# HTDerekLiu/surface_multigrid_code

Measured on AMD Instinct MI355X. Metric: V-cycles/sec + fine-level SpMV GB/s (% HBM peak), 1M-vert mesh fp64, higher is better.
Workload: dtype f64; 1 GPU; C3: bunny_15K_init x3 midpoint subdivision, 1011330 verts, 5 levels, M_bary+0.01(-L), fp64; n_verts=1011330, nnz=7079298, levels=5, smoother=gs, rhs_columns_per_gpu=1, parallelism=single GPU

## Files before the change

include/smg.h:

```cpp
#ifndef SMG_H
#define SMG_H

#ifdef __cplusplus
extern "C" {
#endif

#define SMG_VERSION 507

enum {
    SMG_OK = 0,
    SMG_ERR_INVALID = -1,
    SMG_ERR_NO_DEVICE = -2,
    SMG_ERR_HIP = -3,
    SMG_ERR_NONFINITE = -4,
    SMG_ERR_ALLOC = -5,
    SMG_ERR_IO = -6,
    SMG_ERR_REDUCE = -7
};

enum { SMG_HOST = 0, SMG_DEVICE = 1 };

enum { SMG_DEC_QSLIM = 0, SMG_DEC_MIDPOINT = 1, SMG_DEC_VERTEX_REMOVAL = 2 };

enum { SMG_SMOOTH_GS = 0, SMG_SMOOTH_JACOBI = 1, SMG_SMOOTH_HYBRID = 2, SMG_SMOOTH_CHEBYSHEV = 3, SMG_SMOOTH_HYBRID_CHEBYSHEV = 4 };
// ... 93 lines not shown
int smg_eigs(smg_hierarchy *h, const double *mass_diag, int nev, int block, const double *X0, int ld_x0, int memspace,
             const smg_solve_opts *opts, unsigned long long seed, double *evals, double *X, int ld_x, double *res_his, int *n_iter,
             int *n_converged);

typedef struct smg_geodesics smg_geodesics;
int smg_geodesics_create(const smg_hierarchy *h, const double *V, int nV, const int *F, int nF, double t, int voronoi, smg_geodesics **out);
void smg_geodesics_destroy(smg_geodesics *g);
double smg_geodesics_time(const smg_geodesics *g);
int smg_geodesics_set_solver(smg_geodesics *g, int heat_pcg, int poisson_pcg);
long long smg_geodesics_device_bytes(const smg_geodesics *g);
int smg_geodesics_solve(smg_geodesics *g, int k, const int *src_ptr, const int *src, int memspace, const smg_solve_opts *heat_opts,
                        const smg_solve_opts *poisson_opts, double *D, int ld_d, int *cycles);

typedef struct smg_arap smg_arap;
int smg_arap_create(const smg_hierarchy *h, const double *V, int nV, const int *F, int nF, const int *handles, int n_handles, smg_arap **out);
void smg_arap_destroy(smg_arap *a);
int smg_arap_set_solver(smg_arap *a, int pcg);
long long smg_arap_device_bytes(const smg_arap *a);
int smg_arap_solve(smg_arap *a, const double *handle_pos, int ld_hp, const double *U0, int ld_u0, int memspace, int max_iter, double rel_tol,
                   const smg_solve_opts *opts, double *U, int ld_u, double *energy_his, int *cycles, int *n_iter);

typedef struct {
    double young, poisson, thickness, mass_scale, dt, pressure;
    int newton_iters;
    double ls_c, ls_shrink, ls_min_alpha, eig_floor, eig_value;
} smg_membrane_params;
void smg_membrane_params_default(smg_membrane_params *p);
typedef struct smg_membrane smg_membrane;
int smg_membrane_create(const smg_hierarchy *h, const double *V, int nV, const int *F, int nF, const smg_membrane_params *p, smg_membrane **out);
void smg_membrane_destroy(smg_membrane *m);
long long smg_membrane_device_bytes(const smg_membrane *m);
int smg_membrane_set_state(smg_membrane *m, const double *pos, const double *qdot, int memspace);
int smg_membrane_get_state(smg_membrane *m, double *pos, double *qdot, int memspace);
int smg_membrane_set_solver(smg_membrane *m, int pcg);
int smg_membrane_step(smg_membrane *m, const smg_solve_opts *opts, double *objective_his, double *alpha, int *cycles, int *n_newton);
int smg_membrane_lists(const int *F, int nF, int nV, int *n_blocks, int *n_contrib, int *bptr, int *bcol, int *c_ptr, int *c_src);
int smg_membrane_faces_host(const double *V0, const double *P, int nV, const int *F, int nF, const smg_membrane_params *p, int fix, double *W,
                            double *G, double *H);

int smg_solve_begin(smg_hierarchy *h, const double *RHS, int ld_rhs, const double *known_val, int ld_kv,
                    const double *z0, int ld_z0, int k, int memspace, const smg_solve_opts *opts);
int smg_solve_iter_residual(smg_hierarchy *h, double *d_sumsq);
int smg_solve_iter_cycle(smg_hierarchy *h, const double *d_sumsq);
int smg_solve_iter_cycle_speculative(smg_hierarchy *h);
int smg_solve_iter_commit(smg_hierarchy *h, const double *d_sumsq);
int smg_solve_poll(smg_hierarchy *h, int *done, int *n_his);
int smg_solve_end(smg_hierarchy *h, double *z, int ld_z, int memspace, double *r_his, int *n_his, int *converged);

typedef int (*smg_reduce_fn)(double *d_sumsq, int count, void *hip_stream, void *ctx);
int smg_solve_sharded(smg_hierarchy *h, const double *RHS, int ld_rhs, const double *known_val, int ld_kv, const double *z0,
                      int ld_z0, int k_local, int memspace, const smg_solve_opts *opts, smg_reduce_fn reduce, void *ctx,
                      double *z, int ld_z, double *r_his, int *n_his, int *converged);

int smg_level_rows(const smg_hierarchy *h, int lv);
int smg_vcycle(smg_hierarchy *h, const double *B, int pre, int post, int lv, double *u, int k);
int smg_apply_A(smg_hierarchy *h, int lv, const double *u, int k, double *Au);
int smg_restrict(smg_hierarchy *h, int lv, const double *x, int k, double *Rx);
int smg_prolong(smg_hierarchy *h, int lv, const double *x, int k, double *Px);
int smg_relax(smg_hierarchy *h, int lv, const double *B, int k, int iters, double *u);
int smg_coarse_solve(smg_hierarchy *h, const double *B, int k, double *u);
int smg_residual_norm(smg_hierarchy *h, int lv, const double *B, const double *u, int k, double *norm);

int smg_raw_spmv(smg_hierarchy *h, int lv, int mode, const double *x, const double *b, double *y, int k);
int smg_raw_relax(smg_hierarchy *h, int lv, const double *b, double *u, int k, int iters);
int smg_raw_spmv_f32(smg_hierarchy *h, int lv, const float *x, float *y, int k);
int smg_raw_outer_iteration(smg_hierarchy *h, int n_iter);
int smg_synchronize(smg_hierarchy *h);
int smg_bench_vcycle(smg_hierarchy *h, int lv, int k, int pre, int post, int reps, double *us_per_cycle);
int smg_bench_relax(smg_hierarchy *h, int lv, int k, int sweeps, int reps, double *us_per_call);

int smg_level_get_matrix(const smg_hierarchy *h, int lv, int which, int internal, int *n_rows, int *n_cols, int *nnz,
                         int *rowptr, int *col, double *val);
int smg_level_get_perm(const smg_hierarchy *h, int lv, int *perm);
int smg_level_get_colors(const smg_hierarchy *h, int lv, int *n_colors, int *color_ptr );
int smg_level_get_Adiag(const smg_hierarchy *h, int lv, double *diag);
int smg_get_unknown(const smg_hierarchy *h, int *n_unknown, int *unknown );
int smg_level_sell_stats(const smg_hierarchy *h, int lv, int which, long *stored, long *padded, int *n_slices);
int smg_level_first_colour_rows(const smg_hierarchy *h, int lv);
long smg_level_spmv_bytes(const smg_hierarchy *h, int lv, int k);
long smg_vcycle_bytes(const smg_hierarchy *h, int k, int pre, int post);

int smg_debug_check_tiling_plan(smg_hierarchy *h, int lv, int sweeps, int tile_rows, int *n_tiles, int *max_ext_rows, double *redundancy,
                                double *max_abs_diff);
int smg_debug_check_block_gs_plan(smg_hierarchy *h, int lv, int block_rows, int *n_blocks, int *n_colors, double *rim, double *fill, double *max_abs_diff);
int smg_debug_check_wave_gs_plan(smg_hierarchy *h, int lv, int piece_rows, int pieces_mode, int *n_pieces, int *n_colors, double *stats, double *max_abs_diff);
int smg_debug_raise_coarse_stall(smg_hierarchy *h);
int smg_debug_schur_solve_host(int n, const int *ptr, const int *col, const double *val, const double *b, double *x, int *n_blocks, int *n_sep);
int smg_debug_check_sparse_cholesky(int n, const int *rowptr, const int *col, const double *val, long *factor_entries, int *dependency_depth,
                                    double *rel_residual);

int smg_debug_dense_geneig_host(int n, const double *A, const double *B, double *evals, double *V);

int smg_debug_eig_gram(int n, int m, int nb_a, const double *Sa, int nb_b, const double *Sb, const double *w, int sym, int done, double *G,
                       int *groups, int *guard_bad);
int smg_debug_eig_combine(int n, int m, int nb, const double *S, const double *AS, const double *C, int make_p, int done, double *X, double *AX,
                          double *P, double *AP, int *guard_bad);
int smg_debug_eig_residual(int n, int m, const double *X, const double *AX, const double *mass, const double *lam, int f32, int done, double *b0,
                           double *u0, float *b32, float *u32, double *res, int *groups, int *guard_bad);
enum { SMG_KRY_DOTS_ZR_ZQ = 0, SMG_KRY_DIRECTION = 1, SMG_KRY_DOTS_PQ = 2, SMG_KRY_STEP_DECIDE = 3, SMG_KRY_PRECOND_IN = 4, SMG_KRY_WIDEN = 5 };
int smg_debug_krylov(int op, int n, int k, double *v0, double *v1, double *v2, double *v3, float *e, double *s, int *restart, double tol, int done,
                     double *ctrl_d, int *ctrl_i, int *groups, int *guard_bad);
enum { SMG_GEO_BASIS = 0, SMG_GEO_SCATTER = 1, SMG_GEO_DIVERGENCE = 2, SMG_GEO_SHIFT = 3 };
int smg_debug_geodesics(int op, int n, int nF, int k, const int *F, const int *m_ptr, const int *m_idx, const int *src_ptr, const int *src,
                        const double *in, double *W, double *Af, double *out, int ld_out, int *guard_bad);
enum { SMG_ARAP_COVARIANCE = 0, SMG_ARAP_ROTATIONS = 1, SMG_ARAP_RHS = 2, SMG_ARAP_VERTEX_ENERGY = 3, SMG_ARAP_ENERGY = 4 };
int smg_debug_arap(int op, int n, const int *rowptr, const int *col, const double *w, const double *P0, const double *P, const double *R_in,
                   double *out, int *guard_hits);

enum { SMG_MEM_REST = 0, SMG_MEM_FACES_RAW = 1, SMG_MEM_FACES = 2, SMG_MEM_ENERGY = 3, SMG_MEM_PRESSURE = 4, SMG_MEM_MATRIX = 5,
       SMG_MEM_GRADIENT = 6, SMG_MEM_OBJECTIVE = 7 };
int smg_debug_membrane(int op, int nV, int nF, const int *F, const double *V0, const double *P, const double *in, const smg_membrane_params *p,
                       double *out, int *guard_hits);

int smg_prof_enable(smg_hierarchy *h, int on);
int smg_prof_reset(smg_hierarchy *h);
int smg_prof_count(smg_hierarchy *h);
int smg_prof_get(smg_hierarchy *h, int idx, char *name, int name_cap, long *count, double *total_ms);

int smg_mesh_read(const char *path, double **V, int *nV, int **F, int *nF);
void smg_free(void *p);
int smg_mesh_normalize_unit_area(double *V, int nV, const int *F, int nF);
int smg_mesh_cotmatrix(const double *V, int nV, const int *F, int nF, int *nnz, int *rowptr, int *col, double *val);
int smg_mesh_massmatrix(const double *V, int nV, const int *F, int nF, int voronoi, double *diag);
int smg_mesh_boundary_loop(const int *F, int nF, int nV, int *loop, int *n_loop);
int smg_mesh_midpoint_upsample(int nV, const int *F, int nF, int *nE, int *S_rowptr, int *S_col, double *S_val,
                               int *NF);
int smg_mesh_torus(int nu, int nv, double R, double r, double *V, int *F);

#ifdef __cplusplus
}
#endif
#endif
```

surface_multigrid_code_amd/_lib.py:

```python
import ctypes as C
import os

HERE = os.path.dirname(os.path.abspath(__file__))
LIB_PATH = os.environ.get("SMG_LIB") or os.path.join(HERE, "lib", "libsmg.so")

SMG_HOST, SMG_DEVICE = 0, 1


class SolveOptsC(C.Structure):
    _fields_ = [("tol", C.c_double), ("max_iter", C.c_int), ("pre", C.c_int), ("post", C.c_int),
                ("verbosity", C.c_int), ("check_every", C.c_int), ("use_graph", C.c_int), ("precision", C.c_int),
                ("smoother", C.c_int), ("omega", C.c_double), ("jacobi_max_rows", C.c_int), ("cheby_fraction", C.c_double)]


class MembraneParamsC(C.Structure):
    _fields_ = [("young", C.c_double), ("poisson", C.c_double), ("thickness", C.c_double), ("mass_scale", C.c_double), ("dt", C.c_double),
                ("pressure", C.c_double), ("newton_iters", C.c_int), ("ls_c", C.c_double), ("ls_shrink", C.c_double),
                ("ls_min_alpha", C.c_double), ("eig_floor", C.c_double), ("eig_value", C.c_double)]


_lib = None


REDUCE_FN = C.CFUNCTYPE(C.c_int, C.c_void_p, C.c_int, C.c_void_p, C.c_void_p)
# ... 24 lines not shown
        "smg_level_spectral_bound": (d, [vp, i]),
        "smg_level_set_prolong": (i, [vp, i, i, i, ip, ip, dp]),
        "smg_level_set_prolong_csc": (i, [vp, i, i, i, ip, ip, dp]),
        "smg_level_set_mesh": (i, [vp, i, dp, i, ip, i]),
        "smg_level_get_mesh": (i, [vp, i, ip, ip, dp, ip]),
        "smg_mg_precompute": (i, [dp, i, ip, i, f, i, i, C.POINTER(vp)]),
        "smg_mg_precompute_capped": (i, [dp, i, ip, i, f, i, i, f, C.POINTER(vp)]),
        "smg_mg_precompute_logged": (i, [dp, i, ip, i, f, i, i, f, i, C.POINTER(vp)]),
        "smg_query_coarse_to_fine": (i, [vp, i, i, ip, dp, ip, dp]),
        "smg_query_fine_to_coarse": (i, [vp, i, i, ip, dp, ip, dp]),
        "smg_mg_precompute_block": (i, [dp, i, ip, i, f, i, i, C.POINTER(vp)]),
        "smg_hierarchy_save": (i, [vp, C.c_char_p]),
        "smg_hierarchy_load": (i, [C.c_char_p, C.POINTER(vp)]),
        "smg_mg_precompute_subdiv": (i, [dp, i, ip, i, i, f, i, i, C.POINTER(vp), dp, ip]),
        "smg_precompute": (i, [vp, i, ip, ip, dp, ip, i]),
        "smg_precompute_values_device": (i, [vp, vp]),
        "smg_assembler_create": (i, [ip, i, i, C.POINTER(vp)]),
        "smg_assembler_destroy": (None, [vp]),
        "smg_assembler_pattern": (i, [vp, ip, ip, ip]),
        "smg_assemble": (i, [vp, vp, i, d, d, vp, vp, vp, vp]),
        "smg_solve": (i, [vp, vp, i, vp, i, vp, i, i, i, C.POINTER(SolveOptsC), vp, i, dp, ip, ip]),
        "smg_solve_pcg": (i, [vp, vp, i, vp, i, vp, i, i, i, C.POINTER(SolveOptsC), vp, i, dp, ip, ip]),
        "smg_eigs": (i, [vp, vp, i, i, vp, i, i, C.POINTER(SolveOptsC), C.c_ulonglong, dp, vp, i, dp, ip, ip]),
        "smg_debug_dense_geneig_host": (i, [i, dp, dp, dp, dp]),
        "smg_debug_eig_gram": (i, [i, i, i, dp, i, dp, dp, i, i, dp, ip, ip]),
        "smg_debug_eig_combine": (i, [i, i, i, dp, dp, dp, i, i, dp, dp, dp, dp, ip]),
        "smg_debug_eig_residual": (i, [i, i, dp, dp, dp, dp, i, i, dp, dp, fp, fp, dp, ip, ip]),
        "smg_debug_krylov": (i, [i, i, i, dp, dp, dp, dp, fp, dp, ip, d, i, dp, ip, ip, ip]),
        "smg_debug_geodesics": (i, [i, i, i, i, ip, ip, ip, ip, ip, dp, dp, dp, dp, i, ip]),
        "smg_geodesics_create": (i, [vp, dp, i, ip, i, d, i, C.POINTER(vp)]),
        "smg_geodesics_destroy": (None, [vp]),
        "smg_geodesics_time": (d, [vp]),
        "smg_geodesics_set_solver": (i, [vp, i, i]),
        "smg_geodesics_device_bytes": (C.c_longlong, [vp]),
        "smg_geodesics_solve": (i, [vp, i, ip, ip, i, C.POINTER(SolveOptsC), C.POINTER(SolveOptsC), vp, i, ip]),
        "smg_debug_arap": (i, [i, i, ip, ip, dp, dp, dp, dp, dp, ip]),
        "smg_arap_create": (i, [vp, dp, i, ip, i, ip, i, C.POINTER(vp)]),
        "smg_arap_destroy": (None, [vp]),
        "smg_arap_set_solver": (i, [vp, i]),
        "smg_arap_device_bytes": (C.c_longlong, [vp]),
        "smg_arap_solve": (i, [vp, vp, i, vp, i, i, i, d, C.POINTER(SolveOptsC), vp, i, dp, ip, ip]),
        "smg_debug_membrane": (i, [i, i, i, ip, dp, dp, dp, C.POINTER(MembraneParamsC), dp, ip]),
        "smg_membrane_params_default": (None, [C.POINTER(MembraneParamsC)]),
        "smg_membrane_create": (i, [vp, dp, i, ip, i, C.POINTER(MembraneParamsC), C.POINTER(vp)]),
        "smg_membrane_destroy": (None, [vp]),
        "smg_membrane_device_bytes": (C.c_longlong, [vp]),
        "smg_membrane_set_state": (i, [vp, vp, vp, i]),
        "smg_membrane_get_state": (i, [vp, vp, vp, i]),
        "smg_membrane_set_solver": (i, [vp, i]),
        "smg_membrane_step": (i, [vp, C.POINTER(SolveOptsC), dp, dp, ip, ip]),
        "smg_membrane_lists": (i, [ip, i, i, ip, ip, ip, ip, ip, ip]),
        "smg_membrane_faces_host": (i, [dp, dp, i, ip, i, C.POINTER(MembraneParamsC), i, dp, dp, dp]),
        "smg_solve_sharded": (i, [vp, vp, i, vp, i, vp, i, i, i, C.POINTER(SolveOptsC), REDUCE_FN, vp, vp, i, dp, ip, ip]),
        "smg_solve_begin": (i, [vp, vp, i, vp, i, vp, i, i, i, C.POINTER(SolveOptsC)]),
        "smg_solve_iter_residual": (i, [vp, vp]),
        "smg_solve_iter_cycle": (i, [vp, vp]),
        "smg_solve_iter_cycle_speculative": (i, [vp]),
        "smg_solve_iter_commit": (i, [vp, vp]),
        "smg_solve_poll": (i, [vp, ip, ip]),
        "smg_solve_end": (i, [vp, vp, i, i, dp, ip, ip]),
        "smg_level_rows": (i, [vp, i]),
        "smg_vcycle": (i, [vp, dp, i, i, i, dp, i]),
        "smg_apply_A": (i, [vp, i, dp, i, dp]),
        "smg_restrict": (i, [vp, i, dp, i, dp]),
        "smg_prolong": (i, [vp, i, dp, i, dp]),
        "smg_relax": (i, [vp, i, dp, i, i, dp]),
        "smg_coarse_solve": (i, [vp, dp, i, dp]),
        "smg_residual_norm": (i, [vp, i, dp, dp, i, dp]),
        "smg_raw_spmv": (i, [vp, i, i, vp, vp, vp, i]),
        "smg_raw_relax": (i, [vp, i, vp, vp, i, i]),
        "smg_raw_spmv_f32": (i, [vp, i, vp, vp, i]),
        "smg_raw_outer_iteration": (i, [vp, i]),
        "smg_synchronize": (i, [vp]),
        "smg_bench_vcycle": (i, [vp, i, i, i, i, i, dp]),
        "smg_bench_relax": (i, [vp, i, i, i, i, dp]),
        "smg_level_get_matrix": (i, [vp, i, i, i, ip, ip, ip, ip, ip, dp]),
        "smg_level_get_perm": (i, [vp, i, ip]),
        "smg_level_get_colors": (i, [vp, i, ip, ip]),
        "smg_level_get_Adiag": (i, [vp, i, dp]),
        "smg_get_unknown": (i, [vp, ip, ip]),
        "smg_level_sell_stats": (i, [vp, i, i, lp, lp, ip]),
        "smg_level_first_colour_rows": (i, [vp, i]),
        "smg_debug_check_tiling_plan": (i, [vp, i, i, i, ip, ip, dp, dp]),
        "smg_debug_check_sparse_cholesky": (i, [i, ip, ip, dp, lp, ip, dp]),
        "smg_hierarchy_set_coarse_dense_max": (i, [vp, i]),
        "smg_hierarchy_set_coarse_schur": (i, [vp, i, i]),
        "smg_debug_schur_solve_host": (i, [i, ip, ip, dp, dp, dp, ip, ip]),
        "smg_hierarchy_set_block_gs": (i, [vp, i]),
        "smg_hierarchy_set_wave_gs": (i, [vp, i]),
        "smg_hierarchy_set_memory_lean": (i, [vp, i]),
        "smg_hierarchy_create_union": (i, [C.POINTER(vp), i, C.POINTER(vp)]),
        "smg_union_members": (i, [vp]),
        "smg_union_member_rows": (i, [vp, i, ip, ip]),
        "smg_union_get_history": (i, [vp, i, dp, i, ip, ip]),
        "smg_debug_device_bytes": (i, [vp, C.c_char_p, i]),
        "smg_level_get_wave_gs_order": (i, [vp, i, i, ip, ip, ip, ip, ip, dp]),
        "smg_debug_check_wave_gs_plan": (i, [vp, i, i, i, ip, ip, dp, dp]),
        "smg_debug_raise_coarse_stall": (i, [vp]),
        "smg_debug_check_block_gs_plan": (i, [vp, i, i, ip, ip, dp, dp, dp]),
        "smg_level_get_block_gs_order": (i, [vp, i, i, ip, ip, ip, ip, ip, dp]),
        "smg_hierarchy_coarse_solver": (i, [vp, lp]),
        "smg_hierarchy_set_block_mode": (i, [vp, i]),
        "smg_hierarchy_block_size": (i, [vp]),
        "smg_level_block_stats": (i, [vp, i, lp, lp, ip]),
        "smg_level_get_block_image": (i, [vp, i, ip, ip, ip, ip, ip, ip, dp]),
        "smg_level_spmv_bytes": (C.c_long, [vp, i, i]),
        "smg_vcycle_bytes": (C.c_long, [vp, i, i, i]),
        "smg_prof_enable": (i, [vp, i]),
        "smg_prof_reset": (i, [vp]),
        "smg_prof_count": (i, [vp]),
        "smg_prof_get": (i, [vp, i, C.c_char_p, i, lp, dp]),
        "smg_mesh_read": (i, [C.c_char_p, C.POINTER(dp), ip, C.POINTER(ip), ip]),
        "smg_free": (None, [vp]),
        "smg_mesh_normalize_unit_area": (i, [dp, i, ip, i]),
        "smg_mesh_cotmatrix": (i, [dp, i, ip, i, ip, ip, ip, dp]),
        "smg_mesh_massmatrix": (i, [dp, i, ip, i, i, dp]),
        "smg_mesh_boundary_loop": (i, [ip, i, i, ip, ip]),
        "smg_mesh_midpoint_upsample": (i, [i, ip, i, ip, ip, ip, dp, ip]),
        "smg_mesh_torus": (i, [i, i, d, d, dp, ip]),
    }
    for name, (res, args) in sig.items():
        fn = getattr(L, name)
        fn.restype = res
        fn.argtypes = args
    L._smg_signatures = sig
    _lib = L
    return L


def exported_symbols():
    return sorted(load()._smg_signatures.keys())
```

surface_multigrid_code_amd/api.py:

```python
import ctypes as C

import numpy as np
import scipy.sparse as sp

from . import _lib
from ._lib import SMG_DEVICE, SMG_HOST, SolveOptsC


class SmgError(RuntimeError):
    def __init__(self, code, where):
        msg = _lib.load().smg_last_error()
        super().__init__("%s failed (%d): %s" % (where, code, msg.decode() if msg else ""))
        self.code = code


def _chk(rc, where):
    if rc != 0:
        raise SmgError(rc, where)


def _ip(a):
    return a.ctypes.data_as(C.POINTER(C.c_int))


# ... 216 lines not shown
        y = np.zeros((nout, x.shape[1]), order="F")
        _chk(fn(self.h, lv, _dp(x), x.shape[1], _dp(y)), name)
        return y

    def A(self, lv, u):
        return self._piece(self.L.smg_apply_A, "smg_apply_A", lv, u, self.rows(lv), self.rows(lv))

    def restrict(self, lv, x):
        return self._piece(self.L.smg_restrict, "smg_restrict", lv, x, self.rows(lv + 1), self.rows(lv))

    def prolong(self, lv, x):
        return self._piece(self.L.smg_prolong, "smg_prolong", lv, x, self.rows(lv), self.rows(lv + 1))

    def relax(self, lv, B, u, iters):
        B, u = _colmajor(B), _colmajor(u).copy(order="F")
        self._rows_checked(lv, "smg_relax", B, u)
        _chk(self.L.smg_relax(self.h, lv, _dp(B), B.shape[1], iters, _dp(u)), "smg_relax")
        return u

    def coarse_solve(self, B, u):
        B, u = _colmajor(B), _colmajor(u).copy(order="F")
        self._rows_checked(self.n_levels - 1, "smg_coarse_solve", B, u)
        _chk(self.L.smg_coarse_solve(self.h, _dp(B), B.shape[1], _dp(u)), "smg_coarse_solve")
        return u

    def vcycle(self, B, u, lv=0, pre=2, post=2):
        B, u = _colmajor(B), _colmajor(u).copy(order="F")
        self._rows_checked(lv, "smg_vcycle", B, u)
        _chk(self.L.smg_vcycle(self.h, _dp(B), pre, post, lv, _dp(u), B.shape[1]), "smg_vcycle")
        return u

    def residual_norm(self, lv, B, u):
        B, u = _colmajor(B), _colmajor(u)
        self._rows_checked(lv, "smg_residual_norm", B, u)
        out = C.c_double(0)
        _chk(self.L.smg_residual_norm(self.h, lv, _dp(B), _dp(u), B.shape[1], C.byref(out)), "smg_residual_norm")
        return out.value

    def matrix(self, lv, which="A", internal=False):
        w = {"A": 0, "P": 1, "PT": 2, "P_full": 3, "Auk": 4}[which]
        nr, nc, nnz = C.c_int(), C.c_int(), C.c_int()
        _chk(self.L.smg_level_get_matrix(self.h, lv, w, int(internal), C.byref(nr), C.byref(nc), C.byref(nnz),
                                         None, None, None), "smg_level_get_matrix")
        ptr = np.zeros(nr.value + 1, np.int32)
        col = np.zeros(max(nnz.value, 1), np.int32)
        val = np.zeros(max(nnz.value, 1))
        _chk(self.L.smg_level_get_matrix(self.h, lv, w, int(internal), None, None, None, _ip(ptr), _ip(col), _dp(val)),
             "smg_level_get_matrix")
        return sp.csr_matrix((val[: nnz.value], col[: nnz.value], ptr), shape=(nr.value, nc.value))

    def perm(self, lv):
        p = np.zeros(self.rows(lv), np.int32)
        _chk(self.L.smg_level_get_perm(self.h, lv, _ip(p)), "smg_level_get_perm")
        return p

    def colors(self, lv):
        nc = C.c_int()
        _chk(self.L.smg_level_get_colors(self.h, lv, C.byref(nc), None), "smg_level_get_colors")
        cp = np.zeros(nc.value + 1, np.int32)
        _chk(self.L.smg_level_get_colors(self.h, lv, None, _ip(cp)), "smg_level_get_colors")
        return cp

    def Adiag(self, lv):
        d = np.zeros(self.rows(lv))
        _chk(self.L.smg_level_get_Adiag(self.h, lv, _dp(d)), "smg_level_get_Adiag")
        return d

    def unknown(self):
        n = C.c_int()
        _chk(self.L.smg_get_unknown(self.h, C.byref(n), None), "smg_get_unknown")
        u = np.zeros(n.value, np.int32)
        _chk(self.L.smg_get_unknown(self.h, None, _ip(u)), "smg_get_unknown")
        return u

    def sell_stats(self, lv, which="A"):
        st, pd, ns = C.c_long(), C.c_long(), C.c_int()
        _chk(self.L.smg_level_sell_stats(self.h, lv, {"A": 0, "P": 1, "PT": 2}[which], C.byref(st), C.byref(pd),
                                         C.byref(ns)), "smg_level_sell_stats")
        return {"stored": st.value, "padded": pd.value, "n_slices": ns.value}

    def first_colour_rows(self, lv):
        return self.L.smg_level_first_colour_rows(self.h, lv)

    def set_block_gs(self, min_rows):
        _chk(self.L.smg_hierarchy_set_block_gs(self.h, int(min_rows)), "smg_hierarchy_set_block_gs")

    def block_gs_order(self, lv, k):
        nb, nc = C.c_int(), C.c_int()
        rc = self.L.smg_level_get_block_gs_order(self.h, lv, int(k), C.byref(nb), C.byref(nc), None, None, None, None)
        if rc < 0:
            _chk(rc, "smg_level_get_block_gs_order")
        if rc == 0:
            return None
        cp, bp, rows, st = np.zeros(nc.value + 1, np.int32), np.zeros(nb.value + 1, np.int32), np.zeros(self.rows(lv), np.int32), np.zeros(2)
        _chk(min(self.L.smg_level_get_block_gs_order(self.h, lv, int(k), None, None, _ip(cp), _ip(bp), _ip(rows), _dp(st)), 0), "smg_level_get_block_gs_order")
        return {"rows": rows, "blk_ptr": bp, "color_ptr": cp, "rim": st[0], "fill": st[1]}

    def set_wave_gs(self, mode="auto"):
        _chk(self.L.smg_hierarchy_set_wave_gs(self.h, {"auto": -1, "never": 0, "all": 1}[mode]), "smg_hierarchy_set_wave_gs")

    def wave_gs_order(self, lv, k=1):
        nb, nc = C.c_int(), C.c_int()
        rc = self.L.smg_level_get_wave_gs_order(self.h, lv, int(k), C.byref(nb), C.byref(nc), None, None, None, None)
        if rc < 0:
            _chk(rc, "smg_level_get_wave_gs_order")
        if rc == 0:
            return None
        cp, bp, rows, st = np.zeros(nc.value + 1, np.int32), np.zeros(nb.value + 1, np.int32), np.zeros(self.rows(lv), np.int32), np.zeros(3)
        _chk(min(self.L.smg_level_get_wave_gs_order(self.h, lv, int(k), None, None, _ip(cp), _ip(bp), _ip(rows), _dp(st)), 0), "smg_level_get_wave_gs_order")
        return {"rows": rows, "piece_ptr": bp, "color_ptr": cp, "rim": st[0], "phases_mean": st[1], "phases_max": int(st[2])}

    def gs_order(self, lv, k=1):
        w = self.wave_gs_order(lv, k)
        if w is not None:
            return w["rows"]
        b = self.block_gs_order(lv, k)
        if b is not None:
            return b["rows"]
        return np.arange(self.rows(lv), dtype=np.int32)

    @classmethod
    def union(cls, members):
        L = _lib.load()
        arr = (C.c_void_p * len(members))(*[m.h for m in members])
        out = C.c_void_p()
        _chk(L.smg_hierarchy_create_union(arr, len(members), C.byref(out)), "smg_hierarchy_create_union")
        return cls(handle=out.value)

    def union_members(self):
        return self.L.smg_union_members(self.h)

    def union_member_rows(self, member):
        a, b = C.c_int(), C.c_int()
        _chk(self.L.smg_union_member_rows(self.h, member, C.byref(a), C.byref(b)), "smg_union_member_rows")
        return a.value, b.value

    def union_history(self, member, cap=4096):
        rh, n, cv = np.zeros(cap), C.c_int(), C.c_int()
        _chk(self.L.smg_union_get_history(self.h, member, _dp(rh), cap, C.byref(n), C.byref(cv)), "smg_union_get_history")
        return bool(cv.value), rh[:min(n.value, cap)].copy()

    def set_coarse_dense_max(self, n_max):
        _chk(self.L.smg_hierarchy_set_coarse_dense_max(self.h, int(n_max)), "smg_hierarchy_set_coarse_dense_max")

    def set_coarse_schur(self, when="refactor", n_min=-1):
        _chk(self.L.smg_hierarchy_set_coarse_schur(self.h, {"never": 0, "always": 1, "refactor": 2}[when], int(n_min)), "smg_hierarchy_set_coarse_schur")

    def set_memory_lean(self, on=True):
        _chk(self.L.smg_hierarchy_set_memory_lean(self.h, 1 if on else 0), "smg_hierarchy_set_memory_lean")

    def coarse_solver(self):
        ne = C.c_long()
        kind = self.L.smg_hierarchy_coarse_solver(self.h, C.byref(ne))
        return {"kind": {1: "sparse_cholesky", 2: "schur_complement"}.get(kind, "dense_inverse"), "factor_entries": ne.value}

    def set_block_mode(self, mode="auto"):
        _chk(self.L.smg_hierarchy_set_block_mode(self.h, {"auto": -1, "scalar": 0, "block": 3}.get(mode, mode)), "smg_hierarchy_set_block_mode")

    def block_size(self):
        return self.L.smg_hierarchy_block_size(self.h)

    def block_stats(self, lv=0):
        nb, ns, nc = C.c_long(), C.c_long(), C.c_int()
        _chk(self.L.smg_level_block_stats(self.h, lv, C.byref(nb), C.byref(ns), C.byref(nc)), "smg_level_block_stats")
        return {"blocks": nb.value, "block_slots": ns.value, "vertex_colors": nc.value}

# ... 346 lines not shown
```

surface_multigrid_code_amd/csrc/smg_capi.cpp:

```cpp
#include <hip/hip_runtime.h>

#include <algorithm>
#include <atomic>
#include <chrono>
#include <cmath>
#include <cstdarg>
#include <cstdio>
#include <cstdlib>
#include <cstring>
#include <functional>
#include <memory>
#include <numeric>
#include <string>
#include <thread>
#include <vector>

#include "smg_internal.hpp"

using namespace smg;

static thread_local std::string g_err;
int smg::fail(int code, const char* fmt, ...)
{
    char buf[512];
    va_list ap;
    va_start(ap, fmt);
    std::vsnprintf(buf, sizeof(buf), fmt, ap);
    va_end(ap);
    g_err = buf;
    return code;
}

extern "C" const char* smg_last_error(void) { return g_err.c_str(); }
extern "C" int smg_version(void) { return SMG_VERSION; }
extern "C" long long smg_device_bytes_live(void) { return (long long)smg::devbuf_live_bytes().load(); }
extern "C" int smg_debug_device_bytes(const smg_hierarchy* h, char* buf, int cap)
{
    if (!h || !buf || cap < 1) return SMG_ERR_INVALID;
    std::string out;
    auto B = [](const auto& d) { return (long long)(d.n * sizeof(*d.p)); };
    auto sell = [&](const smg::SellBuf& S) { return B(S.slice_row) + B(S.slice_off) + B(S.slice_w) + B(S.col) + B(S.order) + B(S.val) + B(S.diag_slot) + B(S.long_row) + B(S.long_ptr) + B(S.long_col) + B(S.long_val) + B(S.long_valf); };
    long long tot = 0;
    auto line = [&](const std::string& nm, long long v) { if (v) { out += nm + " " + std::to_string(v) + "\n"; tot += v; } };
    for (int lv = 0; lv < h->n_levels; lv++) {
        const smg::Level& L = h->lv[lv];
        const std::string p = "level" + std::to_string(lv) + ".";
        line(p + "A_sell", sell(L.dA)); line(p + "AT_sell", sell(L.dAT)); line(p + "P_sell", sell(L.dP)); line(p + "PT_sell", sell(L.dPT));
        line(p + "A_block3", B(L.bA.slice_row) + B(L.bA.slice_off) + B(L.bA.slice_w) + B(L.bA.col) + B(L.bA.order) + B(L.bA.val) + B(L.bA.valf) + B(L.bAT.slice_row) + B(L.bAT.slice_off) + B(L.bAT.slice_w) + B(L.bAT.col) + B(L.bAT.order) + B(L.bAT.val) + B(L.bAT.valf) + B(L.mapB) + B(L.mapBT));
        line(p + "values_caller_order", B(L.d_Aval) + B(L.d_Tval));
        line(p + "refresh_maps", B(L.mapA) + B(L.mapAT));
        line(p + "galerkin_recipes", B(L.r1_ptr) + B(L.r1_idx) + B(L.r2_ptr) + B(L.r2_idx) + B(L.r1_coef) + B(L.r2_coef));
        long long t = 0;
        for (const auto& T : L.tiled) t += T.bytes();
        line(p + "tiled_plans", t);
        line(p + "bgs_plan", L.bgs.bytes());
        line(p + "wgs_plan", L.wgs.bytes());
        line(p + "fp32_images", B(L.a32) + B(L.at32) + B(L.p32) + B(L.pt32) + B(L.b32) + B(L.u32) + B(L.r32) + B(L.t32) + B(L.d32));
        line(p + "vectors", B(L.b) + B(L.u) + B(L.r) + B(L.t) + B(L.d));
    }
    line("coarse.dense_inverse", B(h->d_Ainv) + B(h->d_Ainv32));
    line("coarse.sym_partials", B(h->d_sympart));
    line("coarse.sparse_factor", B(h->c_perm) + B(h->c_rptr) + B(h->c_rcol) + B(h->c_cptr) + B(h->c_crow) + B(h->c_err) + B(h->c_rval) + B(h->c_cval) + B(h->c_diag) + B(h->c_work));
    line("coarse.schur", B(h->sch.irow) + B(h->sch.bsize) + B(h->sch.srow) + B(h->sch.sptr) + B(h->sch.sidx) + B(h->sch.aptr) + B(h->sch.ablk) + B(h->sch.acol) + B(h->sch.rptr) + B(h->sch.coff) + B(h->sch.pos) +
                         B(h->sch.pos2) + B(h->sch.ones) + B(h->sch.rdst) + B(h->sch.rdst2) + B(h->sch.rsrc) + B(h->sch.arena) + B(h->sch.g) + B(h->sch.xs) + B(h->sch.sym) + B(h->sch.gj) + B(h->sch.arena32) + B(h->sch.g32) + B(h->sch.xs32));
    line("maps_level0", B(h->d_map0) + B(h->d_perm0) + B(h->d_unknown) + B(h->d_known) + B(h->d_auk_ptr) + B(h->d_auk_col) + B(h->d_auk_val));
    line("reprecompute_bookkeeping", B(h->d_lhs_src) + B(h->d_auk_src) + B(h->d_diag_idx) + B(h->d_dense_pos) + B(h->d_Afull));
    line("early_upload", B(h->early0.ptr) + B(h->early0.col) + B(h->early0.val));
    line("krylov", B(h->kry_x) + B(h->kry_r) + B(h->kry_p) + B(h->kry_q) + B(h->kry_b) + B(h->kry_part) + B(h->kry_s) + B(h->kry_restart));
    line("eigs", B(h->eig_x[0]) + B(h->eig_x[1]) + B(h->eig_ax[0]) + B(h->eig_ax[1]) + B(h->eig_p[0]) + B(h->eig_p[1]) + B(h->eig_ap[0]) + B(h->eig_ap[1]) +
                 B(h->eig_w) + B(h->eig_aw) + B(h->eig_mass) + B(h->eig_part) + B(h->eig_small) + B(h->eig_stage));
    line("solve_state", B(h->d_ctrl) + B(h->d_rhis) + B(h->d_partials) + B(h->d_lam) + B(h->d_stage_rhs) + B(h->d_stage_z) + B(h->d_stage_kv) + B(h->d_tmp_cm) + B(h->d_zsave));
    out += "total " + std::to_string(tot) + "\n";
    std::snprintf(buf, (size_t)cap, "%s", out.c_str());
    return SMG_OK;
}
extern "C" int smg_device_count(void)
{
    int n = 0;
    if (hipGetDeviceCount(&n) != hipSuccess) return 0;
    return n;
}
extern "C" void smg_solve_opts_default(smg_solve_opts* o)
{
    if (!o) return;
    o->tol = 1e-3;
    o->max_iter = 20;
    o->pre = 2;
    o->post = 2;
    o->verbosity = 0;
    o->check_every = 0;
    o->use_graph = 1;
    o->precision = 0;
    o->smoother = SMG_SMOOTH_GS;
    o->omega = 0.8;
    o->jacobi_max_rows = 100000;
    o->cheby_fraction = 0.1;
}

int smg::ensure_device(smg_hierarchy* h)
{
    if (h->device >= 0) return SMG_OK;
    int n = 0;
    if (hipGetDeviceCount(&n) != hipSuccess || n <= 0)
        return fail(SMG_ERR_NO_DEVICE, "no HIP device: libsmg has no CPU fallback (the CPU oracle lives in oracle/)");
    int dev = 0;
    HIPCHK(hipGetDevice(&dev));
    h->device = dev;
    if (!h->stream && !h->user_stream) {
        HIPCHK(hipStreamCreateWithFlags(&h->stream, hipStreamNonBlocking));
        h->own_stream = true;
    }
    HIPCHK(h->d_ctrl.alloc(1));
    HIPCHK(hipMemset(h->d_ctrl.p, 0, sizeof(Ctrl)));
    HIPCHK(h->d_rhis.alloc(1));
    return SMG_OK;
}

void smg::drop_graphs(smg_hierarchy* h) { h->graphs.drop(); }

hipError_t SellBuf::upload(const Sell& S)
{
    hipError_t e;
    if ((e = slice_row.upload(S.slice_row)) != hipSuccess) return e;
    if ((e = slice_off.upload(S.slice_off)) != hipSuccess) return e;
    if ((e = slice_w.upload(S.slice_w)) != hipSuccess) return e;
    const bool layout_only = S.col.empty() && S.padded() > 0;
    if (layout_only) {
        if ((e = col.alloc((size_t)S.padded())) != hipSuccess) return e;
        if ((e = val.alloc((size_t)S.padded())) != hipSuccess) return e;
    } else {
        if ((e = col.upload(S.col)) != hipSuccess) return e;
        if ((e = val.upload(S.val)) != hipSuccess) return e;
    }
    if ((e = order.upload(S.region_order)) != hipSuccess) return e;
    view.n_rows = S.n_rows; view.n_cols = S.n_cols; view.n_slices = S.n_slices; view.C = S.C;
    view.order = S.region_order.empty() ? nullptr : order.p;
// ... 710 lines not shown
```

surface_multigrid_code_amd/csrc/smg_cycle.cpp:

```cpp
#include <hip/hip_runtime.h>

#include <algorithm>
#include <chrono>
#include <cmath>
#include <cstdarg>
#include <cstdio>
#include <cstdlib>
#include <cstring>
#include <functional>
#include <memory>
#include <numeric>
#include <string>
#include <thread>
#include <vector>

#include "smg_internal.hpp"

using namespace smg;


int smg::ensure_work(smg_hierarchy* h, int k)
{
    const int L = h->n_levels;
    if (k > h->kcap) {
// ... 198 lines not shown
    static hipError_t coarse(smg_hierarchy* h, Level& L, int k, const Ctrl* ctrl)
    {
        if (h->union_m > 0) return launch_blockdiag_gemv_add(h->un.view, h->d_Ainv.p, h->nc, L.b.p, L.u.p, k, ctrl, h->stream);
        if (h->coarse_sparse) return launch_sparse_coarse_solve(h->c_view, L.b.p, L.u.p, k, ctrl, h->stream);
        if (h->coarse_schur) return launch_schur_solve(h->sch.view, L.b.p, L.u.p, k, ctrl, h->stream);
        return launch_dense_gemv_add(h->d_Ainv.p, h->nc, h->nc_pad, L.b.p, L.u.p, coarse_cols(h, k), k, ctrl, h->stream, h->d_sympart.p);
    }
    static hipError_t opA(smg_hierarchy* h, Level& L, bool smoother_image, SellMode m, int s0, int s1, const double* x, const double* bb, double* y, int k,
                          const Ctrl* ctrl, const FirstColour* fc = nullptr, double omega = 1.0)
    {
        if (h->bs == 3) {
            const Bsr3Dev& V = (smoother_image && L.gs_on_transpose) ? L.bAT.view : L.bA.view;
            return launch_bsr3(m, V, s0, s1 < 0 ? V.n_slices : s1, x, bb, y, k, ctrl, nullptr, nullptr, h->stream, omega, fc ? fc->c1 : 0.0, fc ? fc->d : nullptr);
        }
        const SellDev& V = smoother_image ? G(L) : A(L);
        return sell(m, V, s0, s1 < 0 ? V.n_slices : s1, x, bb, y, k, ctrl, h->stream, nullptr, fc, omega);
    }
};
template <> struct Prec<float> {
    static float* b(Level& L) { return L.b32.p; }
    static float* u(Level& L) { return L.u32.p; }
    static float* r(Level& L) { return L.r32.p; }
    static float* t(Level& L) { return L.t32.p; }
    static float* d(Level& L) { return L.d32.p; }
    static void set_d(FirstColour& fc, Level& L) { fc.df = L.d32.p; }
    static const SellDev& A(Level& L) { return L.dA32; }
    static const SellDev& G(Level& L) { return L.gs_on_transpose ? L.dAT32 : L.dA32; }
    static const SellDev& P(Level& L) { return L.dP32; }
    static const SellDev& PT(Level& L) { return L.dPT32; }
    static bool has_vals(const SellDev& V) { return V.valf != nullptr; }
    static hipError_t sell(SellMode m, const SellDev& V, int s0, int s1, const float* x, const float* bb, float* y, int k, const Ctrl* ctrl,
                           hipStream_t st, float* zero_rows = nullptr, const FirstColour* first = nullptr, double omega = 1.0)
    { return launch_sell_f32(m, V, s0, s1, x, bb, y, k, ctrl, st, zero_rows, first, omega); }
    static hipError_t coarse(smg_hierarchy* h, Level& L, int k, const Ctrl* ctrl)
    {
        if (h->coarse_schur) return launch_schur_solve_f32(h->sch.view, L.b32.p, L.u32.p, k, ctrl, h->stream);
        return launch_dense_gemv_add_f32(h->d_Ainv32.p, h->nc, h->nc_pad, L.b32.p, L.u32.p, coarse_cols(h, k), k, ctrl, h->stream, (float*)h->d_sympart.p);
    }
    static hipError_t opA(smg_hierarchy* h, Level& L, bool smoother_image, SellMode m, int s0, int s1, const float* x, const float* bb, float* y, int k,
                          const Ctrl* ctrl, const FirstColour* fc = nullptr, double omega = 1.0)
    {
        if (h->bs == 3) {
            const Bsr3Dev& V = (smoother_image && L.gs_on_transpose) ? L.bAT.view : L.bA.view;
            return launch_bsr3_f32(m, V, s0, s1 < 0 ? V.n_slices : s1, x, bb, y, k, ctrl, h->stream, omega, fc ? fc->c1 : 0.0, fc ? fc->df : nullptr);
        }
        const SellDev& V = smoother_image ? G(L) : A(L);
        return sell(m, V, s0, s1 < 0 ? V.n_slices : s1, x, bb, y, k, ctrl, h->stream, nullptr, fc, omega);
    }
};

static const std::vector<int>& colour_slices(const smg_hierarchy* h, const Level& Lv)
{
    if (h->bs == 3) return (Lv.gs_on_transpose ? Lv.bAT : Lv.bA).color_slice_ptr;
    return (Lv.gs_on_transpose ? Lv.dAT : Lv.dA).color_slice_ptr;
}

template <typename T>
static int enqueue_gs(smg_hierarchy* h, int lv, const SweepPlan& sp, const T* b, T* u, int k, int iters, const Ctrl* ctrl, int first = FIRST_NONE, T* t = nullptr)
{
    Level& Lv = h->lv[lv];
    ProfGuard pg(h, "MG: relaxation");
    if (const WgsBuf* W = sp.wave) {
        for (int it = 0; it < iters; it++)
            for (size_t c = 0; c + 1 < W->color_ptr.size(); c++)
                HIPCHK(launch_wgs(W->view, W->color_ptr[c], W->color_ptr[c + 1], (const double*)b, (double*)u, k, ctrl, h->stream));
        return SMG_OK;
    }
    if (const BgsBuf* Q = sp.block) {
        for (int it = 0; it < iters; it++)
            for (size_t c = 0; c + 1 < Q->color_ptr.size(); c++)
                HIPCHK(launch_bgs(Q->view, Q->color_ptr[c], Q->color_ptr[c + 1], (const double*)b, (double*)u, k, ctrl, h->stream));
        return SMG_OK;
    }
    const std::vector<int>& cs = colour_slices(h, Lv);
    for (int it = first == FIRST_SWEEP ? 1 : 0; it < iters; it++)
        for (size_t c = (it == 0 && first == FIRST_LAUNCH) ? 1 : 0; c + 1 < cs.size(); c++) {
            if (it == 1 && first == FIRST_SWEEP) HIPCHK(Prec<T>::sell(SELL_GS_OOP, Prec<T>::G(Lv), cs[c], cs[c + 1], t, b, u, k, ctrl, h->stream));
            else HIPCHK(Prec<T>::opA(h, Lv, true, SELL_GS, cs[c], cs[c + 1], u, b, u, k, ctrl));
        }
    return SMG_OK;
}

template <typename T>
static int enqueue_gs_tiled(smg_hierarchy* h, const TiledDev& plan, const T* b, T* const buf[2], int* cur, int k, const Ctrl* ctrl)
{
    ProfGuard pg(h, "MG: relaxation");
    HIPCHK(launch_tiled_gs(plan, (const double*)buf[*cur], (const double*)b, (double*)buf[1 - *cur], k, ctrl, h->stream));
    *cur ^= 1;
    return SMG_OK;
}

template <typename T>
static int enqueue_jacobi(smg_hierarchy* h, int lv, const T* b, T* const buf[2], int* cur, int k, int iters, const Ctrl* ctrl)
{
    Level& Lv = h->lv[lv];
    ProfGuard pg(h, "MG: relaxation");
    for (int it = 0; it < iters; it++) {
        HIPCHK(Prec<T>::opA(h, Lv, true, SELL_JACOBI, 0, -1, buf[*cur], b, buf[1 - *cur], k, ctrl, nullptr, h->omega));
        *cur ^= 1;
    }
    return SMG_OK;
}

template <typename T>
static int enqueue_cheby(smg_hierarchy* h, int lv, const T* b, T* const buf[2], int* cur, int k, int iters, const Ctrl* ctrl, bool first_done = false)
{
    if (iters <= 0) return SMG_OK;
    Level& Lv = h->lv[lv];
    ProfGuard pg(h, "MG: relaxation");
    std::vector<ChebyCoef> cf;
    cheby_coefs(Lv.lam, h->cheby_fraction, iters + 1, cf);
    for (int s = first_done ? 1 : 0; s <= iters; s++) {
        FirstColour fc;
        Prec<T>::set_d(fc, Lv);
        fc.c1 = cf[s].c1;
        HIPCHK(Prec<T>::opA(h, Lv, true, SELL_CHEBY, 0, -1, buf[*cur], b, buf[1 - *cur], k, ctrl, &fc, cf[s].c2));
        *cur ^= 1;
    }
    return SMG_OK;
}

static bool fuse_first_colour() { static const int on = env_int("SMG_FUSE_FIRST", 1); return on != 0; }

template <typename T>
static int enqueue_vcycle_t(smg_hierarchy* h, int lv, int k, int pre, int post, const Ctrl* ctrl, int first = FIRST_NONE)
{
    const bool first_done = first != FIRST_NONE;
    const int L = h->n_levels;
    Level& Lv = h->lv[lv];
    if (lv == L - 1) {
        ProfGuard pg(h, "MG: coarse solve");
        HIPCHK(Prec<T>::coarse(h, Lv, k, ctrl));
        return SMG_OK;
    }
    Level& Lc = h->lv[lv + 1];
    const int kind = level_kind(h, lv);
    const bool jac = kind != LV_GS;
    T* const buf[2] = {Prec<T>::u(Lv), Prec<T>::t(Lv)};
    int cur = 0;
    const bool fp64 = std::is_same<T, double>::value;
    const SweepPlan sp_pre = sweep_plan(h, lv, k, pre, fp64, first), sp_post = sweep_plan(h, lv, k, post, fp64, FIRST_NONE);
    int rc;
    if (kind == LV_JACOBI) {
        if (first_done) cur = 1;
        rc = enqueue_jacobi<T>(h, lv, Prec<T>::b(Lv), buf, &cur, k, pre - (first_done ? 1 : 0), ctrl);
    } else if (kind == LV_CHEBY) {
        if (first_done) cur = 1;
        rc = enqueue_cheby<T>(h, lv, Prec<T>::b(Lv), buf, &cur, k, pre, ctrl, first_done);
    } else if (sp_pre.tiled) rc = enqueue_gs_tiled<T>(h, *sp_pre.tiled, Prec<T>::b(Lv), buf, &cur, k, ctrl);
    else rc = enqueue_gs<T>(h, lv, sp_pre, Prec<T>::b(Lv), buf[0], k, pre, ctrl, first, buf[1]);
    if (rc) return rc;
    {
        ProfGuard pg(h, "MG: residual");
        HIPCHK(Prec<T>::opA(h, Lv, false, SELL_RESID, 0, -1, buf[cur], Prec<T>::b(Lv), Prec<T>::r(Lv), k, ctrl));
    }
    const SellBuf& Gc = Lc.gs_on_transpose ? Lc.dAT : Lc.dA;
    const int kind_c = level_kind(h, lv + 1);
    const bool jac_c = kind_c != LV_GS;
    const bool fuse = h->bs == 1 && sweep_plan(h, lv + 1, k, pre, fp64, FIRST_NONE).colours() && fuse_first_colour() && lv + 1 < L - 1 && pre > 0 && Prec<T>::has_vals(Prec<T>::G(Lc)) && (jac_c ? Gc.n_all > 0 : Gc.n_first > 0);
    const int kt = k * h->bs;
    {
        ProfGuard pg(h, "MG: restrict");
        FirstColour fc;
        if (fuse) {
            fc.diag_slot = Gc.diag_slot.p; fc.n_first = jac_c ? Gc.n_all : Gc.n_first;
            fc.val = Prec<T>::G(Lc).val; fc.valf = Prec<T>::G(Lc).valf;
            fc.jacobi = kind_c == LV_CHEBY ? 2 : (jac_c ? 1 : 0); fc.omega = h->omega;
            if (kind_c == LV_CHEBY) {
                std::vector<ChebyCoef> cf;
                cheby_coefs(Lc.lam, h->cheby_fraction, 1, cf);
                fc.omega = cf[0].c2;
                Prec<T>::set_d(fc, Lc);
            }
        }
        T* init = (fuse && jac_c) ? Prec<T>::t(Lc) : Prec<T>::u(Lc);
        HIPCHK(Prec<T>::sell(SELL_AX, Prec<T>::PT(Lc), 0, Prec<T>::PT(Lc).n_slices, Prec<T>::r(Lv), nullptr, Prec<T>::b(Lc), kt, ctrl, h->stream, init,
                             fuse ? &fc : nullptr));
    }
    rc = enqueue_vcycle_t<T>(h, lv + 1, k, pre, post, ctrl, fuse ? FIRST_LAUNCH : FIRST_NONE);
    if (rc) return rc;
    {
        ProfGuard pg(h, "MG: prolong");
        int dst = cur;
        const int flips = sp_post.tiled ? 1 : kind == LV_CHEBY ? (post > 0 ? post + 1 : 0) : post;
        if ((jac || sp_post.tiled) && ((cur + flips) & 1)) dst = 1 - cur;
        if (!jac && !sp_post.tiled && cur == 1) dst = 0;
        HIPCHK(Prec<T>::sell(SELL_ADD, Prec<T>::P(Lc), 0, Prec<T>::P(Lc).n_slices, Prec<T>::u(Lc), buf[cur], buf[dst], kt, ctrl, h->stream));
        cur = dst;
    }
    if (kind == LV_CHEBY) return enqueue_cheby<T>(h, lv, Prec<T>::b(Lv), buf, &cur, k, post, ctrl);
    if (jac) return enqueue_jacobi<T>(h, lv, Prec<T>::b(Lv), buf, &cur, k, post, ctrl);
    if (sp_post.tiled) return enqueue_gs_tiled<T>(h, *sp_post.tiled, Prec<T>::b(Lv), buf, &cur, k, ctrl);
    return enqueue_gs<T>(h, lv, sp_post, Prec<T>::b(Lv), buf[0], k, post, ctrl);
}

int smg::enqueue_vcycle(smg_hierarchy* h, int k, const Ctrl* ctrl, int first)
{
    if (h->precision == 1) return enqueue_vcycle_t<float>(h, 0, k, h->pre, h->post, ctrl);
    return enqueue_vcycle_t<double>(h, 0, k, h->pre, h->post, ctrl, first);
}

int smg::apply_A(smg_hierarchy* h, int lv, SellMode mode, const double* x, const double* b, double* y, int k, const Ctrl* ctrl)
{
    HIPCHK(Prec<double>::opA(h, h->lv[lv], false, mode, 0, -1, x, b, y, k, ctrl));
    return SMG_OK;
}


static int enqueue_relax(smg_hierarchy* h, int lv, const double* b, double* u, int k, int iters, const Ctrl* ctrl)
{
    Level& Lv = h->lv[lv];
    const int kind = level_kind(h, lv);
    const SweepPlan sp = sweep_plan(h, lv, k, iters, true, FIRST_NONE);
    if (kind == LV_GS && !sp.tiled) return enqueue_gs<double>(h, lv, sp, b, u, k, iters, ctrl);
    double* const buf[2] = {u, Lv.t.p};
    int cur = 0;
    int rc = kind == LV_GS ? enqueue_gs_tiled<double>(h, *sp.tiled, b, buf, &cur, k, ctrl)
             : kind == LV_CHEBY ? enqueue_cheby<double>(h, lv, b, buf, &cur, k, iters, ctrl) : enqueue_jacobi<double>(h, lv, b, buf, &cur, k, iters, ctrl);
    if (rc) return rc;
    if (cur == 1) HIPCHK(hipMemcpyAsync(u, Lv.t.p, (size_t)Lv.n * k * sizeof(double), hipMemcpyDeviceToDevice, h->stream));
    return SMG_OK;
}

bool smg::head_fusable(smg_hierarchy* h, int k)
{
    static const int on = env_int("SMG_FUSE_HEAD", 1);
    if (!on || h->precision != 0 || h->n_levels < 2 || h->prof_on || h->bs != 1 || h->union_m > 0) return false;
    Level& L0 = h->lv[0];
    if (L0.gs_on_transpose) return false;
    if (!sweep_plan(h, 0, k, h->pre, true, FIRST_NONE).colours()) return false;
    const int kind = level_kind(h, 0);
    return kind == LV_GS ? h->pre >= 2 : h->pre >= 1;
}

int smg::enqueue_residual_ss(smg_hierarchy* h, int k, bool fuse_decide, double* sumsq_out)
// ... 47 lines not shown

int smg::enqueue_cycle_part(smg_hierarchy* h, int k, const double* d_sumsq)
{
    if (d_sumsq) HIPCHK(launch_decide(h->d_ctrl.p, d_sumsq, h->stream));
    {
        ProfGuard pg(h, "MG: total VCycle");
        if (h->precision == 1) {
            Level& L0 = h->lv[0];
            const size_t cnt = (size_t)L0.n * k;
            HIPCHK(launch_residual_to_f32(L0.b32.p, L0.u32.p, L0.r.p, cnt, h->d_ctrl.p, h->stream));
            int rc = enqueue_vcycle(h, k, h->d_ctrl.p, FIRST_NONE);
            if (rc) return rc;
            HIPCHK(launch_add_correction(L0.u.p, L0.u32.p, cnt, h->d_ctrl.p, h->stream));
        } else {
            int rc = enqueue_vcycle(h, k, h->d_ctrl.p, h->head_fuse ? FIRST_SWEEP : FIRST_NONE);
            if (rc) return rc;
            if (h->union_m > 0) HIPCHK(launch_union_restore(h->un.view, h->lv[0].u.p, k, h->d_ctrl.p, h->stream));
        }
    }
    return SMG_OK;
}

int smg::coarse_stall_check(smg_hierarchy* h)
{
    if (!h->coarse_sparse || !h->c_err.p) return SMG_OK;
    int cerr = 0;
    HIPCHK(hipMemcpy(&cerr, h->c_err.p, sizeof(int), hipMemcpyDeviceToHost));
    if (!cerr) return SMG_OK;
    (void)hipMemset(h->c_err.p, 0, sizeof(int));
    return fail(SMG_ERR_HIP, "the triangular solves of the sparse coarse factorisation stalled (results are NaN)");
}

int smg::check_ready(const smg_hierarchy* h, const char* who)
{
    if (!h) return fail(SMG_ERR_INVALID, "%s: null handle", who);
    if (!h->precomputed) return fail(SMG_ERR_INVALID, "%s: call smg_precompute first", who);
    if (h->device < 0) return fail(SMG_ERR_NO_DEVICE, "%s: no HIP device", who);
    return SMG_OK;
}

int smg::internal_cols(const smg_hierarchy* h, int k)
{
    static const int on = env_int("SMG_PAD_COLS", 1);
    if (!on || k <= 4 || k > 64 || h->union_m > 0) return k;
    if (k > 32) return k > 40 ? 64 : k;
    int p = 8;
    while (p < k) p *= 2;
    return p;
}

static int piece_prolog(smg_hierarchy* h, int lv, int k, const char* who, bool need_coarser);

static int time_graph(smg_hierarchy* h, hipGraphExec_t g, int reps, double* us)
{
    hipEvent_t e0, e1;
    HIPCHK(hipEventCreate(&e0));
    HIPCHK(hipEventCreate(&e1));
    for (int i = 0; i < 3; i++) HIPCHK(hipGraphLaunch(g, h->stream));
    HIPCHK(hipEventRecord(e0, h->stream));
    for (int i = 0; i < reps; i++) HIPCHK(hipGraphLaunch(g, h->stream));
    HIPCHK(hipEventRecord(e1, h->stream));
    HIPCHK(hipStreamSynchronize(h->stream));
    float ms = 0.f;
    HIPCHK(hipEventElapsedTime(&ms, e0, e1));
    *us = 1e3 * ms / reps;
    (void)hipEventDestroy(e0); (void)hipEventDestroy(e1); (void)hipGraphExecDestroy(g);
    return SMG_OK;
}

extern "C" int smg_bench_vcycle(smg_hierarchy* h, int lv, int k, int pre, int post, int reps, double* us_per_cycle)
{
    int rc = piece_prolog(h, lv, k, "smg_bench_vcycle", false);
    if (rc) return rc;
    DeviceScope dsc(h->device);
    if (reps < 1 || !us_per_cycle) return fail(SMG_ERR_INVALID, "smg_bench_vcycle: bad arguments");
    if ((rc = prepare_sweep_plans(h, k, pre, post))) return rc;
    hipGraphExec_t g = nullptr;
    rc = capture_graph(h, &g, [&]() { return enqueue_vcycle_t<double>(h, lv, k, pre, post, nullptr); });
    if (rc) return rc;
    if ((rc = time_graph(h, g, reps, us_per_cycle))) return rc;
    return coarse_stall_check(h);
}

extern "C" int smg_bench_relax(smg_hierarchy* h, int lv, int k, int sweeps, int reps, double* us_per_call)
{
    int rc = piece_prolog(h, lv, k, "smg_bench_relax", true);
    if (rc) return rc;
    DeviceScope dsc(h->device);
    if (reps < 1 || sweeps < 1 || !us_per_call) return fail(SMG_ERR_INVALID, "smg_bench_relax: bad arguments");
    if ((rc = prepare_sweep_plans(h, k, sweeps, sweeps))) return rc;
    Level& Lv = h->lv[lv];
    hipGraphExec_t g = nullptr;
    rc = capture_graph(h, &g, [&]() { return enqueue_relax(h, lv, Lv.b.p, Lv.u.p, k, sweeps, nullptr); });
    if (rc) return rc;
    return time_graph(h, g, reps, us_per_call);
}

extern "C" int smg_synchronize(smg_hierarchy* h)
{
    if (!h || h->device < 0) return fail(SMG_ERR_INVALID, "smg_synchronize: no device");
    DeviceScope dsc(h->device);
    HIPCHK(hipStreamSynchronize(h->stream));
    return coarse_stall_check(h);
}

extern "C" int smg_level_rows(const smg_hierarchy* h, int lv)
{
    if (!h || lv < 0 || lv >= h->n_levels) return SMG_ERR_INVALID;
    return h->lv[lv].n;
}

static int put_block(smg_hierarchy* h, int lv, const double* src, int k, double* dst)
{
    const Level& Lv = h->lv[lv];
    std::vector<double> tmp((size_t)Lv.n * k);
    for (int i = 0; i < Lv.n; i++)
        for (int c = 0; c < k; c++) tmp[(size_t)i * k + c] = src[(size_t)Lv.ord.perm[i] + (size_t)c * Lv.n];
    HIPCHK(hipMemcpyAsync(dst, tmp.data(), tmp.size() * sizeof(double), hipMemcpyHostToDevice, h->stream));
    HIPCHK(hipStreamSynchronize(h->stream));
    return SMG_OK;
}
static int get_block(smg_hierarchy* h, int lv, const double* src, int k, double* dst)
{
    const Level& Lv = h->lv[lv];
    std::vector<double> tmp((size_t)Lv.n * k);
    HIPCHK(hipMemcpyAsync(tmp.data(), src, tmp.size() * sizeof(double), hipMemcpyDeviceToHost, h->stream));
    HIPCHK(hipStreamSynchronize(h->stream));
    for (int i = 0; i < Lv.n; i++)
        for (int c = 0; c < k; c++) dst[(size_t)Lv.ord.perm[i] + (size_t)c * Lv.n] = tmp[(size_t)i * k + c];
    return coarse_stall_check(h);
}

static int piece_prolog(smg_hierarchy* h, int lv, int k, const char* who, bool need_coarser)
{
    int rc = check_ready(h, who);
    if (rc) return rc;
    if (h->in_solve) return fail(SMG_ERR_INVALID, "%s: a split-phase solve is in progress", who);
    if (lv < 0 || lv >= h->n_levels || (need_coarser && lv >= h->n_levels - 1) || k < 1)
        return fail(SMG_ERR_INVALID, "%s: bad level %d or k %d", who, lv, k);
    DeviceScope dsc(h->device);
    return ensure_work(h, k);
}

extern "C" int smg_apply_A(smg_hierarchy* h, int lv, const double* u, int k, double* Au)
{
    int rc = piece_prolog(h, lv, k, "smg_apply_A", true);
    if (rc) return rc;
    DeviceScope dsc(h->device);
    Level& Lv = h->lv[lv];
    if ((rc = put_block(h, lv, u, k, Lv.u.p))) return rc;
    HIPCHK(Prec<double>::opA(h, Lv, false, SELL_AX, 0, -1, Lv.u.p, nullptr, Lv.r.p, k, nullptr));
    return get_block(h, lv, Lv.r.p, k, Au);
}

extern "C" int smg_restrict(smg_hierarchy* h, int lv, const double* x, int k, double* Rx)
{
    int rc = piece_prolog(h, lv, k, "smg_restrict", true);
    if (rc) return rc;
    DeviceScope dsc(h->device);
    Level &Lv = h->lv[lv], &Lc = h->lv[lv + 1];
    if ((rc = put_block(h, lv, x, k, Lv.r.p))) return rc;
    HIPCHK(launch_sell(SELL_AX, Lc.dPT.view, 0, Lc.dPT.view.n_slices, Lv.r.p, nullptr, Lc.b.p, k * h->bs, nullptr, nullptr, nullptr, h->stream));
    return get_block(h, lv + 1, Lc.b.p, k, Rx);
}

extern "C" int smg_prolong(smg_hierarchy* h, int lv, const double* x, int k, double* Px)
// ... 139 lines not shown
```

surface_multigrid_code_amd/csrc/smg_device.hip:

```cpp
#include <hip/hip_runtime.h>

#include <cstdlib>
#include <type_traits>

#include "smg_device.hpp"
#include "smg_device_inl.hpp"
#include "smg_gj_inl.hpp"

namespace smg {


__device__ int g_never_done = 0;
const int* never_done()
{
    static const int* p = nullptr;
    if (!p) { void* q = nullptr; if (hipGetSymbolAddress(&q, HIP_SYMBOL(g_never_done)) == hipSuccess) p = (const int*)q; }
    return p;
}


template <typename T> struct CoarseInit { T* u; const T* gs_val; const int* diag_slot; int n_first; int jacobi; T omega; T* d; T c1; int codes; T tab[4]; };
template <typename T> __device__ __forceinline__ T code_val(const CoarseInit<T>& z, int cw)
{
    const T lo = (cw & 1) ? z.tab[1] : z.tab[0], hi = (cw & 1) ? z.tab[3] : z.tab[2];
// ... 982 lines not shown
        for (int t = 0; t < DEPTH; t++) { av[t] = an[t]; bv[t] = bn[t]; }
    }
    __shared__ double red[4][4][64];
#pragma unroll
    for (int r = 0; r < 4; r++) red[w][r][lane] = acc[r];
    __syncthreads();
    if (w == 0 && !stop) {
#pragma unroll
        for (int r = 0; r < 4; r++) {
            const int row = row0 + lr + 4 * r;
            if (row < n && colok) {
                const size_t o = (size_t)row * ld + col0 + lc;
                u[o] = u[o] + ((red[0][r][lane] + red[1][r][lane]) + (red[2][r][lane] + red[3][r][lane]));
            }
        }
    }
}

template <int KC, int CPW>
__global__ __launch_bounds__(256) void k_dense_gemm_mfma_multi(const double* __restrict__ Ainv, int n, int lda, const double* __restrict__ b,
                                                               double* u, int ld, const int* done, int kvalid)
{
    const int stop = load_flag(done);
    constexpr int CB = KC / 16 / CPW, DEPTH = 6;
    const int lane = threadIdx.x & 63, w = threadIdx.x >> 6;
    const int rb = blockIdx.x / CB, cb = blockIdx.x % CB;
    const int row0 = rb * 16, col0 = cb * 16 * CPW;
    const int lc = lane & 15, lr = lane >> 4;
    const int per = lda / 16;
    const int s0 = per * w;
    const double* pa = Ainv + (size_t)(4 * s0 + lr) * lda + row0 + lc;
    const double* pb = b + (size_t)(4 * s0 + lr) * ld + col0 + lc;
    const size_t sa = (size_t)4 * lda, sb = (size_t)4 * ld;
    v4f64_t acc[CPW];
#pragma unroll
    for (int c = 0; c < CPW; c++) acc[c] = (v4f64_t){0.0, 0.0, 0.0, 0.0};
    double av[DEPTH], bv[CPW][DEPTH];
#pragma unroll
    for (int t = 0; t < DEPTH; t++) {
        av[t] = t < per ? pa[t * sa] : 0.0;
#pragma unroll
        for (int c = 0; c < CPW; c++) bv[c][t] = (t < per && col0 + 16 * c + lc < kvalid) ? pb[t * sb + 16 * c] : 0.0;
    }
    for (int s = 0; s < per; s += DEPTH) {
        double an[DEPTH], bn[CPW][DEPTH];
#pragma unroll
        for (int t = 0; t < DEPTH; t++) {
            const int q = s + DEPTH + t;
            an[t] = q < per ? pa[q * sa] : 0.0;
#pragma unroll
            for (int c = 0; c < CPW; c++) bn[c][t] = (q < per && col0 + 16 * c + lc < kvalid) ? pb[q * sb + 16 * c] : 0.0;
        }
#pragma unroll
        for (int t = 0; t < DEPTH; t++)
#pragma unroll
            for (int c = 0; c < CPW; c++) acc[c] = __builtin_amdgcn_mfma_f64_16x16x4f64(av[t], bv[c][t], acc[c], 0, 0, 0);
#pragma unroll
        for (int t = 0; t < DEPTH; t++) {
            av[t] = an[t];
#pragma unroll
            for (int c = 0; c < CPW; c++) bv[c][t] = bn[c][t];
        }
    }
    __shared__ double red[CPW][4][4][64];
#pragma unroll
    for (int c = 0; c < CPW; c++)
#pragma unroll
        for (int r = 0; r < 4; r++) red[c][w][r][lane] = acc[c][r];
    __syncthreads();
    if (!stop) {
        for (int c = w; c < CPW; c += 4) {
#pragma unroll
            for (int r = 0; r < 4; r++) {
                const int row = row0 + lr + 4 * r;
                if (row < n && col0 + 16 * c + lc < kvalid) {
                    const size_t o = (size_t)row * ld + col0 + 16 * c + lc;
                    u[o] = u[o] + ((red[c][0][r][lane] + red[c][1][r][lane]) + (red[c][2][r][lane] + red[c][3][r][lane]));
                }
            }
        }
    }
}

template <typename T>
__global__ __launch_bounds__(256) void k_sym_gemv_tiles(const T* __restrict__ Ainv, int lda, const T* __restrict__ b, T* __restrict__ part, int nb)
{
    const int idx = blockIdx.x;
    int I = (int)((sqrtf(8.0f * (float)idx + 1.0f) - 1.0f) * 0.5f);
    I -= (I * (I + 1) / 2 > idx);
    I += ((I + 1) * (I + 2) / 2 <= idx);
    const int J = idx - I * (I + 1) / 2;
    __shared__ T tile[64][65];
    __shared__ T bI[64], bJ[64];
    const int t = threadIdx.x;
#pragma unroll
    for (int e = 0; e < 16; e++) {
        const int idx = e * 256 + t, r = idx >> 6, c = idx & 63;
        tile[r][c] = Ainv[(size_t)(I * 64 + r) * lda + J * 64 + c];
    }
    if (t < 64) bJ[t] = b[J * 64 + t];
    else if (t < 128) bI[t - 64] = b[I * 64 + t - 64];
    __syncthreads();
    __shared__ T red[4][64];
    const int g = t >> 6, l = t & 63, h0 = (g & 1) * 32;
    T s = (T)0;
    if (g < 2) {
#pragma unroll 8
        for (int c = h0; c < h0 + 32; c++) s += tile[l][c] * bJ[c];
    } else {
#pragma unroll 8
        for (int r = h0; r < h0 + 32; r++) s += tile[r][l] * bI[r];
    }
    red[g][l] = s;
    __syncthreads();
    if (t < 64) part[((size_t)I * nb + J) * 64 + t] = red[0][t] + red[1][t];
    else if (t < 128 && I != J) part[((size_t)J * nb + I) * 64 + (t - 64)] = red[2][t - 64] + red[3][t - 64];
}
template <typename T>
__global__ __launch_bounds__(256) void k_sym_gemv_sum(const T* __restrict__ part, int nb, int n, T* u, const int* done)
{
    const int stop = load_flag(done);
    __shared__ T red[4][64];
    const int a = blockIdx.x, g = threadIdx.x >> 6, l = threadIdx.x & 63;
    const int q = (nb + 3) / 4, b0 = g * q, b1 = min(nb, b0 + q);
    T s = (T)0;
#pragma unroll 8
    for (int bidx = b0; bidx < b1; bidx++) s += part[((size_t)a * nb + bidx) * 64 + l];
    red[g][l] = s;
    __syncthreads();
    const int i = a * 64 + l;
    if (g == 0 && i < n && !stop) u[i] = u[i] + ((red[0][l] + red[1][l]) + (red[2][l] + red[3][l]));
}

template <typename T>
static hipError_t launch_dense_T(const T* Ainv, int n, int lda, const T* b, T* u, int k, int ld, const Ctrl* ctrl, hipStream_t st, void* sym_work)
{
    const int* done = ctrl ? &ctrl->done : never_done();
    const int nb = (n + 3) / 4;
    if (n <= 0) return hipSuccess;
    if (k == 1 && ld == 1 && sym_work && lda % 64 == 0 && lda >= 512) {
        const int nt = lda / 64;
        hipLaunchKernelGGL((k_sym_gemv_tiles<T>), dim3(nt * (nt + 1) / 2), dim3(256), 0, st, Ainv, lda, b, (T*)sym_work, nt);
        hipLaunchKernelGGL((k_sym_gemv_sum<T>), dim3(nt), dim3(256), 0, st, (const T*)sym_work, nt, n, u, done);
        return hipGetLastError();
    }
    int c0 = 0;
    static const int use_mfma8 = getenv("SMG_COARSE_MFMA") ? atoi(getenv("SMG_COARSE_MFMA")) : 1;
    const int mfma_min = (std::is_same<T, double>::value && use_mfma8 && lda % 64 == 0) ? 8 : 16;
    while (k - c0 >= mfma_min) {
        int kc = 64;
        while (kc > k - c0 && kc > 16) kc >>= 1;
        const int kv = kc < k - c0 ? kc : k - c0;
        const int tb = (n + 15) / 16;
        static const int use_mfma = getenv("SMG_COARSE_MFMA") ? atoi(getenv("SMG_COARSE_MFMA")) : 1;
        if constexpr (std::is_same<T, double>::value) {
            if (use_mfma && lda % 64 == 0) {
                static const int cpw = getenv("SMG_COARSE_CPW") ? atoi(getenv("SMG_COARSE_CPW")) : 2;
                if (kc == 64 && cpw == 2) { hipLaunchKernelGGL((k_dense_gemm_mfma_multi<64, 2>), dim3(tb * 2), dim3(256), 0, st, Ainv, n, lda, b + c0, u + c0, ld, done, kv); c0 += kv; continue; }
                switch (kc) {
                    case 64: hipLaunchKernelGGL((k_dense_gemm_mfma<64>), dim3(tb * 4), dim3(256), 0, st, Ainv, n, lda, b + c0, u + c0, ld, done, kv); break;
                    case 32: hipLaunchKernelGGL((k_dense_gemm_mfma<32>), dim3(tb * 2), dim3(256), 0, st, Ainv, n, lda, b + c0, u + c0, ld, done, kv); break;
                    default: hipLaunchKernelGGL((k_dense_gemm_mfma<16>), dim3(tb), dim3(256), 0, st, Ainv, n, lda, b + c0, u + c0, ld, done, kv); break;
                }
                c0 += kv;
                continue;
            }
        }
        switch (kc) {
            case 64: hipLaunchKernelGGL((k_dense_gemm_tile<64, T>), dim3(tb), dim3(256), 0, st, Ainv, n, lda, b + c0, u + c0, ld, done); break;
            case 32: hipLaunchKernelGGL((k_dense_gemm_tile<32, T>), dim3(tb), dim3(256), 0, st, Ainv, n, lda, b + c0, u + c0, ld, done); break;
            default: hipLaunchKernelGGL((k_dense_gemm_tile<16, T>), dim3(tb), dim3(256), 0, st, Ainv, n, lda, b + c0, u + c0, ld, done); break;
        }
        c0 += kc;
    }
    for (; c0 < k; c0 += 4) {
        const int kb = (k - c0) < 4 ? (k - c0) : 4;
        switch (kb) {
            case 1: hipLaunchKernelGGL((k_dense_gemv_add<1, T>), dim3(nb), dim3(256), 0, st, Ainv, n, lda, b + c0, u + c0, ld, done); break;
            case 2: hipLaunchKernelGGL((k_dense_gemv_add<2, T>), dim3(nb), dim3(256), 0, st, Ainv, n, lda, b + c0, u + c0, ld, done); break;
            case 3: hipLaunchKernelGGL((k_dense_gemv_add<3, T>), dim3(nb), dim3(256), 0, st, Ainv, n, lda, b + c0, u + c0, ld, done); break;
            default: hipLaunchKernelGGL((k_dense_gemv_add<4, T>), dim3(nb), dim3(256), 0, st, Ainv, n, lda, b + c0, u + c0, ld, done); break;
        }
    }
    return hipGetLastError();
}
hipError_t launch_sym_gemv_tiles(const double* Ainv, int lda, const double* b, double* part, hipStream_t st)
{
    if (lda <= 0 || lda % 64) return hipErrorInvalidValue;
    const int nt = lda / 64;
    hipLaunchKernelGGL((k_sym_gemv_tiles<double>), dim3(nt * (nt + 1) / 2), dim3(256), 0, st, Ainv, lda, b, part, nt);
    return hipGetLastError();
}
hipError_t launch_sym_gemv_tiles_f32(const float* Ainv, int lda, const float* b, float* part, hipStream_t st)
{
    if (lda <= 0 || lda % 64) return hipErrorInvalidValue;
    const int nt = lda / 64;
    hipLaunchKernelGGL((k_sym_gemv_tiles<float>), dim3(nt * (nt + 1) / 2), dim3(256), 0, st, Ainv, lda, b, part, nt);
    return hipGetLastError();
}
hipError_t launch_dense_gemv_add(const double* Ainv, int n, int lda, const double* b, double* u, int k, int ld,
                                 const Ctrl* ctrl, hipStream_t st, double* sym_work)
{
    return launch_dense_T<double>(Ainv, n, lda, b, u, k, ld, ctrl, st, sym_work);
}
hipError_t launch_dense_gemv_add_f32(const float* Ainv, int n, int lda, const float* b, float* u, int k, int ld,
                                     const Ctrl* ctrl, hipStream_t st, float* sym_work)
{
    return launch_dense_T<float>(Ainv, n, lda, b, u, k, ld, ctrl, st, sym_work);
}

__global__ void k_cvt_f64_f32(float* dst, const double* src, size_t n)
{
    const size_t i = (size_t)blockIdx.x * blockDim.x + threadIdx.x;
    if (i < n) dst[i] = (float)src[i];
}
__global__ void k_residual_to_f32(float* b32, float* u32, const double* r64, size_t n, const int* done)
{
    if (done && *done) return;
    const size_t i = (size_t)blockIdx.x * blockDim.x + threadIdx.x;
    if (i < n) { b32[i] = (float)r64[i]; u32[i] = 0.0f; }
}
__global__ void k_add_correction(double* z, const float* e, size_t n, const int* done)
{
    if (done && *done) return;
    const size_t i = (size_t)blockIdx.x * blockDim.x + threadIdx.x;
    if (i < n) z[i] = z[i] + (double)e[i];
}
hipError_t launch_cvt_f64_f32(float* dst, const double* src, size_t n, hipStream_t st)
{
    if (n == 0) return hipSuccess;
    hipLaunchKernelGGL(k_cvt_f64_f32, dim3((unsigned)((n + 255) / 256)), dim3(256), 0, st, dst, src, n);
    return hipGetLastError();
}
hipError_t launch_residual_to_f32(float* b32, float* u32, const double* r64, size_t n, const Ctrl* ctrl, hipStream_t st)
{
    if (n == 0) return hipSuccess;
    hipLaunchKernelGGL(k_residual_to_f32, dim3((unsigned)((n + 255) / 256)), dim3(256), 0, st, b32, u32, r64, n, ctrl ? &ctrl->done : nullptr);
    return hipGetLastError();
}
hipError_t launch_add_correction(double* z, const float* e, size_t n, const Ctrl* ctrl, hipStream_t st)
{
    if (n == 0) return hipSuccess;
    hipLaunchKernelGGL(k_add_correction, dim3((unsigned)((n + 255) / 256)), dim3(256), 0, st, z, e, n, ctrl ? &ctrl->done : nullptr);
    return hipGetLastError();
}

constexpr int GJ_H = 32;

__global__ __launch_bounds__(256) void k_gj_diag(const double* M, int n, int kb, double* dinv)
{
    __shared__ double a[GJ_NB][GJ_NB + 1];
    __shared__ double Rb[16][GJ_NB + 1];
    __shared__ double Cb[GJ_NB][17];
    const int K = kb * GJ_NB;
    for (int e = threadIdx.x; e < GJ_NB * GJ_NB; e += 256) a[e / GJ_NB][e % GJ_NB] = M[(size_t)(K + e / GJ_NB) * n + K + e % GJ_NB];
    __syncthreads();
    gj_invert64(a, Rb, Cb);
    for (int e = threadIdx.x; e < GJ_NB * GJ_NB; e += 256) dinv[e] = a[e / GJ_NB][e % GJ_NB];
}

__global__ __launch_bounds__(256) void k_gj_panels(const double* M, int n, int kb, const double* dinv, double* rowp,
                                                   double* colp)
{
    __shared__ double m_s[GJ_NB][GJ_H + 1];
    const int K = kb * GJ_NB;
    const int j0 = blockIdx.x * GJ_H;
    const int J = j0 / GJ_NB;
    const int t = threadIdx.x;
    if (J == kb) {
        for (int e = t; e < GJ_NB * GJ_H; e += 256) {
            const int r = e / GJ_H, c = e % GJ_H;
            rowp[(size_t)r * n + j0 + c] = dinv[r * GJ_NB + j0 + c - K];
        }
        return;
    }
    const int lane = t & 63, w = t >> 6, lr = lane >> 4, lc = lane & 15;
    double av[GJ_NB / 4], mr[8];
#pragma unroll
    for (int q = 0; q < GJ_NB / 4; q++) av[q] = dinv[(16 * w + lc) * GJ_NB + 4 * q + lr];
    if (J < kb) {
// ... 618 lines not shown
```

surface_multigrid_code_amd/csrc/smg_device.hpp:

```cpp
#pragma once
#include <hip/hip_runtime_api.h>

#include <cstdint>

namespace smg {

struct Ctrl {
    int done;
    int n_his;
    int status;
    int just_done;
    double sumsq;
    double tol;
    double* r_his;
    int his_cap;
    int pad_;
    double r_last, r_prev;
};

struct SellDev {
    int n_rows = 0, n_cols = 0, n_slices = 0;
    int C = 64;
    const int* slice_row = nullptr;
    const int* slice_off = nullptr;
// ... 40 lines not shown
struct FirstColour {
    const int* diag_slot = nullptr;
    int n_first = 0;
    const double* val = nullptr;
    const float* valf = nullptr;
    int jacobi = 0;
    double omega = 1.0;
    double* d = nullptr;
    float* df = nullptr;
    double c1 = 0.0;
};
hipError_t launch_sell(SellMode mode, const SellDev& A, int s_begin, int s_end, const double* x, const double* b,
                       double* y, int k, const Ctrl* ctrl, double* partials, int* n_blocks, hipStream_t st,
                       double* zero_rows = nullptr, const FirstColour* first = nullptr, double omega = 1.0);
hipError_t launch_sell_f32(SellMode mode, const SellDev& A, int s_begin, int s_end, const float* x, const float* b,
                           float* y, int k, const Ctrl* ctrl, hipStream_t st, float* zero_rows = nullptr,
                           const FirstColour* first = nullptr, double omega = 1.0);
hipError_t launch_gershgorin(const SellDev& A, double* out, hipStream_t st);
struct Bsr3Dev {
    int n_vert = 0, n_slices = 0, w_max = 0;
    const int* slice_row = nullptr;
    const int* slice_off = nullptr;
    const int* slice_w = nullptr;
    const int* order = nullptr;
    const int* col = nullptr;
    const double* val = nullptr;
    const float* valf = nullptr;
};
hipError_t launch_bsr3(SellMode mode, const Bsr3Dev& A, int s_begin, int s_end, const double* x, const double* b, double* y, int k, const Ctrl* ctrl,
                       double* partials, int* n_blocks, hipStream_t st, double omega = 1.0, double c1 = 0.0, double* dvec = nullptr);
hipError_t launch_bsr3_f32(SellMode mode, const Bsr3Dev& A, int s_begin, int s_end, const float* x, const float* b, float* y, int k, const Ctrl* ctrl, hipStream_t st,
                           double omega = 1.0, double c1 = 0.0, float* dvec = nullptr);
hipError_t launch_bsr3_gershgorin(const Bsr3Dev& A, double* out, hipStream_t st);
int bsr3_blocks(int n_slices);
hipError_t launch_bsr3_fill(const int* ptr, const int* col, const double* val, const int* gptr, const int* gcol, const int* perm, const int* iperm, const Bsr3Dev& B,
                            size_t panel_cols, bool transposed, hipStream_t st);

struct BgsDev {
    int n_blocks = 0, n_colors = 0, xrows = 0;
    const int* hdr = nullptr;
    const int* xrow = nullptr;
    const int* ugrow = nullptr;
    const int* ulrow = nullptr;
    const double* udiag = nullptr;
    const int* eidx = nullptr;
    const double* eval = nullptr;
};
hipError_t launch_bgs(const BgsDev& P, int b_begin, int b_end, const double* b, double* u, int k, const Ctrl* ctrl, hipStream_t st);

struct WgsDev {
    int n_pieces = 0, n_colors = 0, rim_pitch = 0, nb_max = 0;
    const int* hdr = nullptr;
    const int* grow = nullptr;
    const int* meta = nullptr;
    const double* diag = nullptr;
    const int* rim = nullptr;
    const unsigned* eoff = nullptr;
    const double* eval = nullptr;
};
hipError_t launch_wgs(const WgsDev& P, int q_begin, int q_end, const double* b, double* u, int k, const Ctrl* ctrl, hipStream_t st);

struct UnionDev {
    int m = 0, his_cap = 0, max_rows = 0;
    const int* rows = nullptr;
    const int* rptr = nullptr;
    const int* crow_member = nullptr;
    const long long* moff = nullptr;
    const int* mlda = nullptr;
    const int* mrow0 = nullptr;
    double* ss = nullptr;
    double* his = nullptr;
    int* nhis = nullptr;
    int* done = nullptr;
    double* zsave = nullptr;
};
hipError_t launch_blockdiag_gemv_add(const UnionDev& U, const double* Ainv, int n, const double* b, double* u, int k, const Ctrl* ctrl, hipStream_t st);
hipError_t launch_union_sumsq_decide(const UnionDev& U, const double* r, const double* u, int k, Ctrl* ctrl, hipStream_t st);
hipError_t launch_union_restore(const UnionDev& U, double* u, int k, const Ctrl* ctrl, hipStream_t st);
hipError_t launch_scatter_dense(double* dense, const double* src, const long long* pos, int nnz, hipStream_t st);
hipError_t launch_dense_identity(double* dense, int np, int n, hipStream_t st);

struct TiledDev {
    int n_tiles = 0, nc = 0, P = 0, sweeps = 0, max_ext = 0, w_max = 0, threads = 512;
    const int* hdr = nullptr;
    const int* ext_rows = nullptr;
    const int* pcol = nullptr;
    const double* pval = nullptr;
    const int* prow = nullptr;
    const double* pdiag = nullptr;
};
hipError_t launch_tiled_gs(const TiledDev& T, const double* x, const double* b, double* y, int k, const Ctrl* ctrl, hipStream_t st);
hipError_t tiled_gs_prepare(int max_ext);

struct SparseCholDev {
    int n = 0;
    const int* perm = nullptr;
    const int *rptr = nullptr, *rcol = nullptr;
    const int *cptr = nullptr, *crow = nullptr;
    const double *rval = nullptr, *cval = nullptr, *diag = nullptr;
    double* work = nullptr;
    int* err = nullptr;
};
hipError_t launch_sparse_coarse_solve(const SparseCholDev& F, const double* b, double* u, int k, const Ctrl* ctrl, hipStream_t st);
int sparse_coarse_work_cols(int k);

constexpr int SCHUR_M_MAX_DEV = 128;
struct SchurDev {
    int n = 0, nb = 0, ns = 0, ns_pad = 0;
    const int *irow = nullptr, *bsize = nullptr, *srow = nullptr, *sptr = nullptr, *sidx = nullptr, *aptr = nullptr, *ablk = nullptr, *apan = nullptr;
    double* arena = nullptr;
    float* arena32 = nullptr;
    long long off_D = 0, off_P = 0, off_W = 0, off_S = 0, off_C = 0;
    const long long *coff = nullptr, *pos = nullptr, *pos2 = nullptr, *ones = nullptr, *rdst = nullptr, *rdst2 = nullptr, *rsrc = nullptr;
    const int* rptr = nullptr;
    int nnz = 0, n_ones = 0, n_red = 0;
    double *g = nullptr, *xs = nullptr;
    float *g32 = nullptr, *xs32 = nullptr;
    double* sym_work = nullptr;
    double* gj_work = nullptr;
};
hipError_t launch_schur_factor(const SchurDev& F, const double* vals, hipStream_t st);
hipError_t launch_schur_check(const SchurDev& F, int* d_flag, hipStream_t st);
hipError_t launch_schur_solve(const SchurDev& F, const double* b, double* u, int k, const Ctrl* ctrl, hipStream_t st);
hipError_t launch_schur_solve_f32(const SchurDev& F, const float* b, float* u, int k, const Ctrl* ctrl, hipStream_t st);

int sell_blocks(int n_slices);
int sell_wide_blocks(int n_slices, int k);

int ss_partials_room();
hipError_t launch_ss_finalize(const double* partials, int n, Ctrl* ctrl, hipStream_t st, double* out = nullptr);
hipError_t launch_decide(Ctrl* ctrl, const double* sumsq, hipStream_t st);
hipError_t launch_decide_spec(Ctrl* ctrl, const double* sumsq, hipStream_t st);
hipError_t launch_copy_unless_done(double* dst, const double* src, size_t n, const Ctrl* ctrl, hipStream_t st);
hipError_t launch_restore_if_just_done(double* dst, const double* src, size_t n, const Ctrl* ctrl, hipStream_t st);
hipError_t launch_ss_finalize_decide(const double* partials, int n, Ctrl* ctrl, hipStream_t st);

enum { KS_RZ = 0, KS_RZ_PREV = 1, KS_ALPHA = 2, KS_BETA = 3, KS_SLOTS = 4 };
constexpr int KRY_MAX_GROUPS = 512;
struct KryDev {
    int n = 0, k = 0;
    int groups = 0;
    double* part = nullptr;
    double* s = nullptr;
    int* restart = nullptr;
};
int kry_groups(int n, int k);
hipError_t launch_kry_dots_zr_zq(const KryDev& K, const double* z, const double* r, const double* q, const Ctrl* ctrl, hipStream_t st);
hipError_t launch_kry_direction(const KryDev& K, const double* z, double* p, const Ctrl* ctrl, hipStream_t st);
hipError_t launch_kry_dots_pq(const KryDev& K, const double* p, const double* q, const Ctrl* ctrl, hipStream_t st);
hipError_t launch_kry_step_decide(const KryDev& K, double* x, double* r, const double* p, const double* q, Ctrl* ctrl, hipStream_t st);
hipError_t launch_kry_precond_in(const double* r, double* b0, double* u0, size_t cnt, const Ctrl* ctrl, hipStream_t st);
hipError_t launch_kry_widen(const float* e, double* z, size_t cnt, const Ctrl* ctrl, hipStream_t st);
hipError_t launch_kry_arm(const KryDev& K, Ctrl* ctrl, bool reopen, hipStream_t st);

struct EigBlocks {
    const double* p[3] = {nullptr, nullptr, nullptr};
    int nb = 0;
};
constexpr int EIG_TILE = 64;
constexpr int EIG_MAX_GROUPS = 256;
int eig_groups(int n);
size_t eig_gram_part_size(int a, int b, int groups);
hipError_t launch_eig_gram(const EigBlocks& Sa, const EigBlocks& Sb, int n, int m, const double* w, bool sym, double* part, int groups,
                           double* G, const Ctrl* ctrl, hipStream_t st);
hipError_t launch_eig_combine(const EigBlocks& S, const EigBlocks& AS, int n, int m, const double* C, double* X, double* AX, double* P,
                              double* AP, const Ctrl* ctrl, hipStream_t st);
hipError_t launch_eig_residual(const double* X, const double* AX, const double* mass, const double* lam, int n, int m, double* b0, double* u0,
                               float* b32, float* u32, double* part, int groups, double* res, const Ctrl* ctrl, hipStream_t st);

hipError_t launch_dense_gemv_add(const double* Ainv, int n, int lda, const double* b, double* u, int k, int ld,
                                 const Ctrl* ctrl, hipStream_t st, double* sym_work = nullptr);
hipError_t launch_dense_gemv_add_f32(const float* Ainv, int n, int lda, const float* b, float* u, int k, int ld,
                                     const Ctrl* ctrl, hipStream_t st, float* sym_work = nullptr);
hipError_t launch_sym_gemv_tiles(const double* Ainv, int lda, const double* b, double* part, hipStream_t st);
hipError_t launch_sym_gemv_tiles_f32(const float* Ainv, int lda, const float* b, float* part, hipStream_t st);
hipError_t launch_cvt_f64_f32(float* dst, const double* src, size_t n, hipStream_t st);
hipError_t launch_residual_to_f32(float* b32, float* u32, const double* r64, size_t n, const Ctrl* ctrl, hipStream_t st);
hipError_t launch_add_correction(double* z, const float* e, size_t n, const Ctrl* ctrl, hipStream_t st);
hipError_t launch_spd_inverse(double* M, int n, double* work, hipStream_t st);

hipError_t launch_recipe(int n_out, const int* ptr, const int* idx, const double* coef, const double* src, double* out, hipStream_t st);
hipError_t launch_sell_fill(const int* ptr, const int* col, const double* val, const int* perm, const int* iperm, const SellDev& S, size_t padded, hipStream_t st,
                            bool transposed = false);
hipError_t launch_sell_encode(const SellDev& S, size_t padded, const double* tab, int n_tab, int* out_col, int* bad, hipStream_t st);
hipError_t launch_sell_diag_slots(const SellDev& S, int* slot, int* first_missing, hipStream_t st);
hipError_t warm_device_code(hipStream_t st);
hipError_t launch_sell_fill_map(const int* ptr, const int* col, const int* perm, const int* iperm, const SellDev& S, size_t padded, bool transposed, int* map, hipStream_t st);
hipError_t launch_bit_symmetric(int n, const int* ptr, const int* col, const double* val, int* differs, hipStream_t st);
hipError_t launch_gather_vals(double* dst, const double* src, const int* map, size_t n, hipStream_t st);
hipError_t launch_dense_from_csr(double* dense, int np, int n, const double* src, const long long* pos, int nnz, hipStream_t st);
hipError_t launch_add_at(double* v, const int* where, int n, double c, hipStream_t st);

hipError_t launch_assemble(int nV, int nF, int nnz, const double* V, const int* F, int voronoi, const int* l_ptr, const int* l_idx,
                           const signed char* l_sgn, const int* m_ptr, const int* m_idx, const int* diag_of, double* Qc, double* Qm,
                           double* Md, double mass_coef, double lap_coef, double* val, double* Lval, hipStream_t st);

hipError_t launch_gather_in(double* dst, const double* src, const int* map, int n, int k, int kin, int ld_src,
                            hipStream_t st);
hipError_t launch_scatter_out(double* dst, const double* src, const int* map, int n, int k, int kin, int ld_dst,
                              hipStream_t st);
hipError_t launch_scatter_cm(double* dst, const double* src, const int* idx, int n, int k, int ld_src, int ld_dst,
                             hipStream_t st);
hipError_t launch_gather_cm(double* dst, const double* src, const int* idx, int n, int k, int ld_src, int ld_dst,
                            hipStream_t st);
hipError_t launch_csr_sub(int n_rows, const int* ptr, const int* col, const double* val, const double* x, int ldx,
                          double* y, int ld, int k, hipStream_t st);

hipError_t launch_geo_basis(const double* V, const int* F, int nF, double* W, double* Af, hipStream_t st);
hipError_t launch_geo_scatter(int n, int k, const int* src_ptr, const int* src, double* B, int ldb, hipStream_t st);
hipError_t launch_geo_divergence(int n, int k, const int* F, const double* W, const double* Af, const int* m_ptr, const int* m_idx,
                                 const double* U, int ldu, double* out, int ldo, hipStream_t st);
hipError_t launch_geo_shift(int n, int k, const int* src_ptr, const int* src, const double* phi, int ldp, double* mean, double* D, int ldd,
                            hipStream_t st);

hipError_t launch_arap_covariance(int n, const int* rowptr, const int* col, const double* w, const double* P0, const double* P, double* S, hipStream_t st);
hipError_t launch_arap_rotations(int n, const int* rowptr, const int* col, const double* w, const double* P0, const double* P, double* R, double* eterm,
                                 hipStream_t st);
hipError_t launch_arap_vertex_energy(int n, const int* rowptr, const int* col, const double* w, const double* P0, const double* P, const double* R,
                                     double* eterm, hipStream_t st);
hipError_t launch_arap_rhs(int n, const int* rowptr, const int* col, const double* w, const double* P0, const double* R, double* B, int ldb, hipStream_t st);
int arap_groups(int n);
hipError_t launch_arap_energy(const double* eterm, int n, double* part, double* E, hipStream_t st);
hipError_t launch_arap_rows(int n, const double* U, int ldu, double* P, hipStream_t st);
hipError_t launch_arap_columns(int n, const double* P, double* U, int ldu, hipStream_t st);
hipError_t launch_arap_set_handles(int nh, const int* handles, const double* hp, int ldh, double* U, int ldu, hipStream_t st);

hipError_t launch_membrane_rest(int nF, const int* F, const double* V0, double thickness, double* rest, hipStream_t st);
hipError_t launch_membrane_faces(int mode, int nF, const int* F, const double* P, const double* rest, double alpha, double beta, double floor,
                                 double value, double* W, double* G, double* H, hipStream_t st);
hipError_t launch_membrane_matrix(int nB, const int* brow, const int* bcol, const int* bptr, const int* c_ptr, const int* c_src, const double* H,
                                  int nF, double dt2, const double* mass0, double mass_scale, double* val, hipStream_t st);
hipError_t launch_membrane_pressure(int nV, int nF, const int* F, const double* P, const int* m_ptr, const int* m_idx, double pressure, double* Qn,
                                    double* mass, double* fext, hipStream_t st);
hipError_t launch_membrane_gradient(int nV, const int* m_ptr, const int* m_idx, const double* G, int nF, const double* mass0, double mass_scale,
                                    double dt, const double* qdot, const double* qdot0, const double* fext, double* g, double* b, hipStream_t st);
hipError_t launch_membrane_trial(int nV, const double* qdot, const double* dx, double step, const double* qdot0, const double* pos0,
                                 const double* fext, const double* mass0, double mass_scale, double dt, double* t_out, double* p_out, double* term,
                                 hipStream_t st);
hipError_t launch_membrane_dot3(int nV, const double* a, const double* b, double* term, hipStream_t st);

}
```

surface_multigrid_code_amd/csrc/smg_hier.hpp:

```cpp
#pragma once
#include <memory>
#include <hip/hip_runtime_api.h>

#include <atomic>
#include <cstdint>
#include <string>
#include <vector>

#include "smg_bsr3.hpp"
#include "smg_coarse.hpp"
#include "smg_device.hpp"
#include "smg_mesh.hpp"
#include "smg_order.hpp"
#include "smg_sparse.hpp"
#include "smg_tiled.hpp"
#include "smg_bgs.hpp"
#include "smg_wgs.hpp"
#include "smg_schur.hpp"

namespace smg {

inline std::atomic<long long>& devbuf_live_bytes() { static std::atomic<long long> v{0}; return v; }

template <typename T>
// ... 7 lines not shown
    void release() { if (p) (void)hipHostFree(p); p = nullptr; n = 0; }
    hipError_t ensure(size_t count)
    {
        if (count <= n) return hipSuccess;
        release();
        hipError_t e = hipHostMalloc((void**)&p, count * sizeof(T), hipHostMallocDefault);
        if (e == hipSuccess) n = count; else p = nullptr;
        return e;
    }
};

template <typename T>
struct DevBuf {
    T* p = nullptr;
    size_t n = 0;
    DevBuf() = default;
    DevBuf(const DevBuf&) = delete;
    DevBuf& operator=(const DevBuf&) = delete;
    DevBuf(DevBuf&& o) noexcept : p(o.p), n(o.n) { o.p = nullptr; o.n = 0; }
    DevBuf& operator=(DevBuf&& o) noexcept { if (this != &o) { release(); p = o.p; n = o.n; o.p = nullptr; o.n = 0; } return *this; }
    ~DevBuf() { release(); }
    void release() { if (p) { (void)hipFree(p); devbuf_live_bytes() -= (long long)(n * sizeof(T)); } p = nullptr; n = 0; }
    hipError_t alloc(size_t count)
    {
        release();
        if (count == 0) return hipSuccess;
        hipError_t e = hipMalloc((void**)&p, count * sizeof(T));
        if (e == hipSuccess) { n = count; devbuf_live_bytes() += (long long)(count * sizeof(T)); } else p = nullptr;
        return e;
    }
    hipError_t ensure(size_t count) { return count <= n ? hipSuccess : alloc(count); }
    long long bytes() const { return (long long)(n * sizeof(T)); }
    template <class Alloc>
    hipError_t upload(const std::vector<T, Alloc>& v)
    {
        hipError_t e = alloc(v.size());
        if (e != hipSuccess || v.empty()) return e;
        return hipMemcpy(p, v.data(), v.size() * sizeof(T), hipMemcpyHostToDevice);
    }
    template <class Alloc>
    hipError_t upload_in_place(const std::vector<T, Alloc>& v, bool* moved)
    {
        if (p && v.size() == n) return v.empty() ? hipSuccess : hipMemcpy(p, v.data(), v.size() * sizeof(T), hipMemcpyHostToDevice);
        *moved = true;
        return upload(v);
    }
};

struct SellBuf {
    DevBuf<int> slice_row, slice_off, slice_w, col, order;
    DevBuf<double> val;
    SellDev view;
    std::vector<int> color_slice_ptr;
    DevBuf<int> diag_slot;
    int n_first = 0;
    int n_all = 0;
    long stored = 0, padded = 0, used = 0;
    hipError_t upload(const Sell& S);
    DevBuf<int> long_row, long_ptr, long_col;
    DevBuf<double> long_val;
    DevBuf<float> long_valf;
    hipError_t upload_long(const std::vector<int>& rows, const std::vector<int>& ptr, const std::vector<int>& col, const std::vector<double>& val);
    hipError_t encode_codes(const double* vals, size_t n_vals, hipStream_t st);
};

struct Bsr3Buf {
    DevBuf<int> slice_row, slice_off, slice_w, col, order;
    DevBuf<double> val;
    DevBuf<float> valf;
    Bsr3Dev view;
    std::vector<int> color_slice_ptr;
    long stored = 0, blocks = 0, padded = 0;
    hipError_t upload(const Bsr3Sell& S);
};

struct PlanValues {
    DevBuf<double> val, diag;
    DevBuf<int> map, mapd;
    std::vector<int> host_map, host_mapd;
    long long bytes() const { return val.bytes() + diag.bytes() + map.bytes() + mapd.bytes(); }
};

struct TiledBuf {
    DevBuf<int> hdr, ext_rows, pcol, prow;
    PlanValues v;
    TiledDev view;
    bool tried = false;
    long long bytes() const { return hdr.bytes() + ext_rows.bytes() + pcol.bytes() + prow.bytes() + v.bytes(); }
};

struct BgsBuf {
    DevBuf<int> hdr, xrow, ugrow, ulrow, eidx;
    PlanValues v;
    BgsDev view;
    std::vector<int> color_ptr;
    std::vector<int> host_rows, host_blk_ptr;
    double rim = 0.0, fill = 0.0;
    bool tried = false;
    long long bytes() const { return hdr.bytes() + xrow.bytes() + ugrow.bytes() + ulrow.bytes() + eidx.bytes() + v.bytes(); }
};

struct WgsBuf {
    DevBuf<int> hdr, grow, meta, rim;
    DevBuf<unsigned> eoff;
    PlanValues v;
    WgsDev view;
    std::vector<int> color_ptr;
    std::vector<int> host_rows, host_piece_ptr;
    double rim_ratio = 0.0, phases_mean = 0.0;
    int phases_max = 0;
    bool tried = false;
    long long bytes() const { return hdr.bytes() + grow.bytes() + meta.bytes() + rim.bytes() + eoff.bytes() + v.bytes(); }
};

struct Level {
    std::vector<double> V;
    std::vector<int> F;
    Csr P_full;
    std::shared_ptr<DecimationLog> dec_log;
    Csr A;
    std::vector<double> A_diag;
    Csr P, PT;
    Ordering ord;
    uint64_t ord_key = 0;
    Csr A_int, P_int, PT_int;
    Ordering vord;
    Csr Pv, PTv;
    Bsr3Buf bA, bAT;
    DevBuf<int> mapB, mapBT;
    SellBuf dA, dP, dPT;
    SellBuf dAT;
    bool gs_on_transpose = false;
    bool P_device_filled = false, PT_device_filled = false;
    bool device_filled = false;
    Csr vpat;
    bool A_bit_symmetric = false;
    TiledBuf tiled[4];
    WgsBuf wgs;
    BgsBuf bgs;
    std::vector<int> A_int_src;
    DevBuf<double> d_Aval;
    DevBuf<double> d_Tval;
    DevBuf<int> mapA, mapAT;
    DevBuf<int> r1_ptr, r1_idx, r2_ptr, r2_idx;
    DevBuf<double> r1_coef, r2_coef;
    int nnzT = 0;
    DevBuf<float> a32, at32, p32, pt32;
    SellDev dA32, dAT32, dP32, dPT32;
    DevBuf<float> b32, u32, r32;
    DevBuf<double> b, u, r;
    DevBuf<double> t;
    DevBuf<float> t32;
    DevBuf<double> d;
    DevBuf<float> d32;
    double lam = 0.0;
    int n = 0;
};

struct GraphKey {
    int k = 0, k_user = 0, pre = 0, post = 0, precision = 0, smoother = 0, jacobi_max_rows = 0;
    double omega = 0.0, cheby_fraction = 0.0;
    bool head_fuse = false;
    bool operator==(const GraphKey& o) const
    {
        return k == o.k && k_user == o.k_user && pre == o.pre && post == o.post && precision == o.precision && smoother == o.smoother &&
               jacobi_max_rows == o.jacobi_max_rows && omega == o.omega && cheby_fraction == o.cheby_fraction && head_fuse == o.head_fuse;
    }
    bool operator!=(const GraphKey& o) const { return !(*this == o); }
};

enum Step { STEP_ITER,
            STEP_ITER_N,
            STEP_HEAD,
            STEP_TAIL,
            STEP_SPLIT_RESID,
            STEP_SPLIT_CYCLE,
            STEP_SPEC,
            STEP_PCG,
            STEP_PCG_N,
            STEP_COUNT };

struct GraphCache {
    hipGraphExec_t exec[STEP_COUNT] = {};
    GraphKey mg_key, pcg_key;
    double* sumsq = nullptr;
    void drop(int s0 = 0, int s1 = STEP_COUNT)
    {
        for (int s = s0; s < s1; s++) if (exec[s]) { (void)hipGraphExecDestroy(exec[s]); exec[s] = nullptr; }
        if (s0 <= STEP_ITER && s1 > STEP_ITER) mg_key = GraphKey();
        if (s0 <= STEP_PCG && s1 > STEP_PCG) pcg_key = GraphKey();
    }
};

struct ProfScope { std::string name; long count = 0; double ms = 0.0; };
struct ProfRec { int scope; hipEvent_t e0, e1; };

}

struct smg_hierarchy {
    int n_levels = 0;
    std::vector<smg::Level> lv;
    int n_full = 0;
    bool has_known = false, precomputed = false;
    std::vector<int> known, unknown;
    smg::Csr LHS_unused;
    smg::Csr Auk;
    smg::DevBuf<int> d_map0;
    smg::DevBuf<int> d_perm0;
    smg::DevBuf<int> d_unknown, d_known;
    smg::DevBuf<int> d_auk_ptr, d_auk_col;
    smg::DevBuf<double> d_auk_val;
    uint64_t pre_key = 0;
    int p_version = 0;
    bool input_canonical = false;
    bool recipes_built = false, host_stale = false;
    int nnz_input = 0;
    std::vector<int> lhs_src, auk_src;
    smg::DevBuf<int> d_lhs_src, d_auk_src, d_diag_idx;
    smg::DevBuf<long long> d_dense_pos;
    smg::DevBuf<double> d_Afull;
// ... 92 lines not shown
```

surface_multigrid_code_amd/csrc/smg_internal.hpp:

```cpp
#pragma once
#include <hip/hip_runtime_api.h>

#include <chrono>
#include <cstdio>
#include <cstdlib>
#include <exception>
#include <new>
#include <string>

#include "../../include/smg.h"
#include "smg_hier.hpp"
#include "smg_mesh.hpp"

namespace smg {

int fail(int code, const char* fmt, ...) __attribute__((format(printf, 2, 3)));

#define HIPCHK(expr)                                                                                          \
    do {                                                                                                      \
        hipError_t e__ = (expr);                                                                              \
        if (e__ != hipSuccess) return ::smg::fail(SMG_ERR_HIP, "%s failed: %s", #expr, hipGetErrorString(e__)); \
    } while (0)

template <typename Fn>
// ... 51 lines not shown

int prof_scope_id(smg_hierarchy* h, const char* name);
hipEvent_t prof_event(smg_hierarchy* h);
void prof_collect(smg_hierarchy* h);
struct ProfGuard {
    smg_hierarchy* h; int idx = -1;
    ProfGuard(smg_hierarchy* hh, const char* name) : h(hh)
    {
        if (!h->prof_on) return;
        ProfRec r; r.scope = prof_scope_id(h, name); r.e0 = prof_event(h); r.e1 = prof_event(h);
        (void)hipEventRecord(r.e0, h->stream);
        h->recs.push_back(r);
        idx = (int)h->recs.size() - 1;
    }
    ~ProfGuard() { if (idx >= 0) (void)hipEventRecord(h->recs[idx].e1, h->stream); }
};

const char* check_compressed(int n_major, int n_minor, const int* ptr, const int* idx);
int set_prolong(smg_hierarchy* h, int lv, Csr&& P);
Mesh wrap_mesh(const double* V, int nV, const int* F, int nF);

double double_area(const double* V, const int* F, int f);
int components(const int* F, int nF, int nV);
int level0_rows(const smg_hierarchy* h);
long long handle_bytes(const smg_hierarchy* h);
int copy_prolongations(const smg_hierarchy* src, smg_hierarchy* dst);

struct MembraneLists { std::vector<int> bptr, bcol, brow, c_ptr, c_src; };
void membrane_lists(const int* F, int nF, int nV, MembraneLists& L);

int spectral_bounds(smg_hierarchy* h);
int ensure_spectral_bounds(smg_hierarchy* h);
int refresh_host_values(smg_hierarchy* h);
int ensure_P_int(smg_hierarchy* h, int lv);
int ensure_A_int(smg_hierarchy* h, int lv);

int union_coarse_factor(smg_hierarchy* h, const double* d_vals, bool first);
int union_begin_solve(smg_hierarchy* h, int k);

enum { LV_GS = 0, LV_JACOBI = 1, LV_CHEBY = 2 };
int level_kind(const smg_hierarchy* h, int lv);
inline bool level_is_jacobi(const smg_hierarchy* h, int lv) { return level_kind(h, lv) != LV_GS; }

enum { FIRST_NONE = 0,
       FIRST_LAUNCH = 1,
       FIRST_SWEEP = 2 };

int ensure_work(smg_hierarchy* h, int k);
int ensure_fp32(smg_hierarchy* h, int k);
int enqueue_vcycle(smg_hierarchy* h, int k, const Ctrl* ctrl, int first);
int enqueue_residual_ss(smg_hierarchy* h, int k, bool fuse_decide = false, double* sumsq_out = nullptr);
int enqueue_cycle_part(smg_hierarchy* h, int k, const double* d_sumsq);
int apply_A(smg_hierarchy* h, int lv, SellMode mode, const double* x, const double* b, double* y, int k, const Ctrl* ctrl);
bool head_fusable(smg_hierarchy* h, int k);
int internal_cols(const smg_hierarchy* h, int k);
int coarse_stall_check(smg_hierarchy* h);

template <typename Fn>
static int capture_graph(smg_hierarchy* h, hipGraphExec_t* out, Fn&& body)
{
    hipGraph_t g = nullptr;
    HIPCHK(hipStreamBeginCapture(h->stream, hipStreamCaptureModeThreadLocal));
    int rc = body();
    hipError_t e = hipStreamEndCapture(h->stream, &g);
    if (rc) { if (g) (void)hipGraphDestroy(g); return rc; }
    if (e != hipSuccess) return fail(SMG_ERR_HIP, "hipStreamEndCapture: %s", hipGetErrorString(e));
    e = hipGraphInstantiate(out, g, nullptr, nullptr, 0);
    (void)hipGraphDestroy(g);
    if (e != hipSuccess) return fail(SMG_ERR_HIP, "hipGraphInstantiate: %s", hipGetErrorString(e));
    return SMG_OK;
}

int latch_solve_opts(smg_hierarchy* h, const smg_solve_opts& o);
int reset_ctrl(smg_hierarchy* h, int cap);

struct SweepPlan {
    const TiledDev* tiled = nullptr;
    const WgsBuf* wave = nullptr;
    const BgsBuf* block = nullptr;
    bool colours() const { return !tiled && !wave && !block; }
};
SweepPlan sweep_plan(const smg_hierarchy* h, int lv, int k, int sweeps, bool fp64, int first);
int prepare_sweep_plans(smg_hierarchy* h, int k, int sa, int sb);
int prepare_level_plans(smg_hierarchy* h, int lv);
int refresh_plan_values(smg_hierarchy* h);
void drop_sweep_plans(smg_hierarchy* h);

}
```

surface_multigrid_code_amd/csrc/smg_precompute.cpp:

```cpp
#include <hip/hip_runtime.h>

#include <algorithm>
#include <atomic>
#include <chrono>
#include <condition_variable>
#include <mutex>
#include <cmath>
#include <cstdarg>
#include <cstdio>
#include <cstdlib>
#include <cstring>
#include <exception>
#include <functional>
#include <memory>
#include <numeric>
#include <string>
#include <thread>
#include <vector>

#include "smg_internal.hpp"

using namespace smg;

static bool bit_symmetric(const Csr& A)
// ... 609 lines not shown
        Lv.b32.release(); Lv.u32.release(); Lv.r32.release(); Lv.t32.release(); Lv.d32.release();
    }
    h->kcap = 0; h->kcap32 = 0; h->f32_valid = false;
    return SMG_OK;
}

static void run_image_tasks(const char* what, int lv, std::vector<std::function<void()>>& tasks)
{
    static const bool on = env_int("SMG_TIMING", 0) != 0;
    if (!on) { parallel_tasks(tasks); return; }
    std::vector<double> ms(tasks.size(), 0.0);
    std::vector<std::function<void()>> timed;
    for (size_t i = 0; i < tasks.size(); i++)
        timed.push_back([&, i] {
            const auto t0 = std::chrono::steady_clock::now();
            tasks[i]();
            ms[i] = 1e3 * std::chrono::duration<double>(std::chrono::steady_clock::now() - t0).count();
        });
    const auto t0 = std::chrono::steady_clock::now();
    parallel_tasks(timed);
    std::fprintf(stderr, "[smg timing] device:   level %d %s: %.1f ms, tasks", lv, what, 1e3 * std::chrono::duration<double>(std::chrono::steady_clock::now() - t0).count());
    for (double v : ms) std::fprintf(stderr, " %.1f", v);
    std::fprintf(stderr, "\n");
}

static int coarse_images(smg_hierarchy* h)
{
    const int L = h->n_levels;
    Level& Lc = h->lv[L - 1];
    Lc.device_filled = false;
    Lc.A_int = Lc.A;
    Lc.A_int_src.resize((size_t)Lc.A.nnz());
    std::iota(Lc.A_int_src.begin(), Lc.A_int_src.end(), 0);
    if (L == 1) {
        Sell S = build_sell(Lc.A_int, nullptr, SELL_C, false, h->mem_lean ? 0 : -1);
        HIPCHK(Lc.dA.upload(S));
    }
    const int nc = Lc.n;
    const int np = ((nc + 63) / 64) * 64;
    h->coarse_schur = false;
    h->schur_declined = false;
    if (h->union_m > 0) {
        if (h->bs != 1) return fail(SMG_ERR_INVALID, "a union handle needs scalar hierarchies (no 3-DOF block structure)");
        h->sch.release(); h->schur = SchurPlan();
        DevBuf<double> d_val;
        HIPCHK(d_val.upload(Lc.A.val));
        return union_coarse_factor(h, d_val.p, true);
    }
    if (schur_wanted(h, nc, 1)) {
        bool planned = false;
        const int rc = coarse_plan_schur(h, Lc.A, &planned);
        if (rc) return rc;
        if (planned) {
            DevBuf<double> d_val;
            HIPCHK(d_val.upload(Lc.A.val));
            HIPCHK(launch_schur_factor(h->sch.view, d_val.p, h->stream));
            { int rc2 = schur_check_spd(h, nc); if (rc2) return rc2; }
            h->nc = nc; h->nc_pad = np;
            h->coarse_schur = true;
            if (h->coarse_sparse) {
                h->coarse_sparse = false;
                h->c_perm.release(); h->c_rptr.release(); h->c_rcol.release(); h->c_cptr.release(); h->c_crow.release(); h->c_rval.release(); h->c_cval.release(); h->c_diag.release(); h->c_work.release();
            }
            h->d_Ainv.release(); h->d_Ainv32.release(); h->d_sympart.release();
            return SMG_OK;
        }
    }
    h->sch.release(); h->schur = SchurPlan();
    if (Lc.n > h->coarse_dense_max) {
        h->nc = Lc.n; h->nc_pad = Lc.n;
        return coarse_factor_sparse(h, Lc.A, false);
    }
    h->coarse_sparse = false;
    h->nc = nc; h->nc_pad = np;
    std::vector<long long> pos((size_t)Lc.A.nnz());
    for (int i = 0; i < nc; i++)
        for (int p = Lc.A.ptr[i]; p < Lc.A.ptr[i + 1]; p++) pos[(size_t)p] = (long long)i * np + Lc.A.col[p];
    DevBuf<long long> d_pos;
    DevBuf<double> d_val;
    HIPCHK(d_pos.upload(pos));
    HIPCHK(d_val.upload(Lc.A.val));
    HIPCHK(h->d_Ainv.ensure((size_t)np * np));
    HIPCHK(launch_dense_from_csr(h->d_Ainv.p, np, nc, d_val.p, d_pos.p, (int)Lc.A.nnz(), h->stream));
    if (env_int("SMG_SYM_COARSE", 1)) HIPCHK(h->d_sympart.ensure((size_t)(np / 64) * (np / 64) * 64)); else h->d_sympart.release();
    DevBuf<double> work;
    HIPCHK(work.alloc((size_t)2 * np * 64 + 2 * 64 * 64));
    HIPCHK(launch_spd_inverse(h->d_Ainv.p, np, work.p, h->stream));
    HIPCHK(hipStreamSynchronize(h->stream));
    return SMG_OK;
}

static int level_images(smg_hierarchy* h, int lv, int sym0)
{
    const int L = h->n_levels;
    const int sellC = SELL_C;
    const bool region = env_int("SMG_REGION_ORDER", 1) != 0;
    const bool blk = h->bs == 3;
    const int lp = lv + 1;
    Level& Lw = h->lv[lv];
    Level& Lp = h->lv[lp];
    {
        std::vector<std::function<void()>> tasks;
        tasks.push_back([h, lv, &Lw] {
            Lw.device_filled = false;
            if (device_fill_candidate(h, lv)) {
                Lw.A_int = Csr(); Lw.A_int_src.clear();
                Lw.device_filled = true;
            } else Lw.A_int = permute(Lw.A, Lw.ord.perm, Lw.ord.perm, &Lw.A_int_src);
        });
        tasks.push_back([h, &Lw, &Lp] {
            Lp.P_device_filled = device_fill_rows(h, Lp.P.nr);
            if (Lp.P_device_filled) Lp.P_int = Csr(); else Lp.P_int = permute(Lp.P, Lw.ord.perm, Lp.ord.perm);
        });
        tasks.push_back([h, &Lw, &Lp] {
            static const int long_min = env_int("SMG_LONG_ROW_MIN", 65);
            bool ok = device_fill_rows(h, Lp.PT.nr);
            if (ok && long_min > 0) for (int r = 0; r < Lp.PT.nr && ok; r++) if (Lp.PT.ptr[(size_t)r + 1] - Lp.PT.ptr[(size_t)r] >= long_min) ok = false;
            Lp.PT_device_filled = ok;
            if (ok) Lp.PT_int = Csr(); else Lp.PT_int = permute(Lp.PT, Lp.ord.perm, Lw.ord.perm);
        });
        run_image_tasks("operators in the device numbering", lv, tasks);
    }
    int bad = 0;
    hipError_t eA = hipSuccess, eT = hipSuccess, eP = hipSuccess, eQ = hipSuccess;
    std::vector<std::function<void()>> tasks;
    tasks.push_back([&] {
        DeviceScope ds(h->device);
        if (blk && Lw.device_filled) {
            Lw.dA = SellBuf();
            DeviceCsr D;
            eA = D.put(Lw.A, lv == 0 && !h->has_known ? &h->early0 : nullptr);
            int differs = sym0 == 1 ? 0 : -1;
            DevBuf<int> d_differs, d_gptr, d_gcol, d_perm, d_iperm;
            if (eA == hipSuccess && differs < 0) {
                eA = d_differs.alloc(1);
                if (eA == hipSuccess) eA = launch_bit_symmetric(Lw.A.nr, D.ptr, D.col, D.val, d_differs.p, h->aux[0]);
                if (eA == hipSuccess) eA = hipMemcpyAsync(&differs, d_differs.p, sizeof(int), hipMemcpyDeviceToHost, h->aux[0]);
                if (eA == hipSuccess) eA = hipStreamSynchronize(h->aux[0]);
            }
            if (eA != hipSuccess) return;
            if (Lw.A.nr != Lw.A.nc || (differs & 2)) { bad = 1; return; }
            Lw.A_bit_symmetric = differs == 0;
            Lw.gs_on_transpose = differs != 0;
            Lw.bAT = Bsr3Buf(); Lw.dAT = SellBuf();
            const Csr& G = Lw.vpat;
            const std::vector<int>& vp = Lw.vord.perm;
            std::vector<int> row_len(vp.size());
            parallel_for((long)vp.size(), 1 << 16, [&](long r0, long r1) { for (long r = r0; r < r1; r++) row_len[(size_t)r] = G.ptr[(size_t)vp[(size_t)r] + 1] - G.ptr[(size_t)vp[(size_t)r]]; });
            if (eA == hipSuccess) eA = d_gptr.upload(G.ptr);
            if (eA == hipSuccess) eA = d_gcol.upload(G.col);
            if (eA == hipSuccess) eA = d_perm.upload(vp);
            if (eA == hipSuccess) eA = d_iperm.upload(Lw.vord.iperm);
            const Bsr3Sell S = bsr3_layout(row_len, &Lw.vord.color_ptr, region, Lw.A.nnz(), G.nnz());
            if (eA == hipSuccess) eA = Lw.bA.upload(S);
            if (eA == hipSuccess) eA = launch_bsr3_fill(D.ptr, D.col, D.val, d_gptr.p, d_gcol.p, d_perm.p, d_iperm.p, Lw.bA.view, (size_t)S.slice_off.back(), false, h->aux[0]);
            if (eA == hipSuccess && Lw.gs_on_transpose) {
                const Bsr3Sell ST = bsr3_layout(row_len, &Lw.vord.color_ptr, false, Lw.A.nnz(), G.nnz());
                eT = Lw.bAT.upload(ST);
                if (eT == hipSuccess) eT = launch_bsr3_fill(D.ptr, D.col, D.val, d_gptr.p, d_gcol.p, d_perm.p, d_iperm.p, Lw.bAT.view, (size_t)ST.slice_off.back(), true, h->aux[0]);
            }
            if (eA == hipSuccess) eA = hipStreamSynchronize(h->aux[0]);
            return;
        }
        if (blk) {
            Lw.dA = SellBuf();
            Bsr3Sell S = build_bsr3(Lw.A_int, &Lw.vord.color_ptr, region, false);
            eA = Lw.bA.upload(S);
// ... 538 lines not shown
```

surface_multigrid_code_amd/csrc/smg_sweep_plans.cpp:

```cpp
#include <algorithm>
#include <climits>
#include <cmath>
#include <vector>

#include "smg_internal.hpp"

using namespace smg;

static bool gs_plan_level(const smg_hierarchy* h, int lv)
{
    return h->bs == 1 && lv >= 0 && lv < h->n_levels - 1 && level_kind(h, lv) == LV_GS;
}

static int wgs_mode_now(const smg_hierarchy* h)
{
    static const int env = env_int("SMG_WGS", -1);
    return env >= 0 ? (env == 0 ? 0 : env == 1 ? -1 : 1) : h->wgs_mode;
}
static bool wgs_in_range(const smg_hierarchy* h, int lv)
{
    static const int max_rows = env_int("SMG_WGS_MAX_ROWS", 600000), min_rows = env_int("SMG_WGS_MIN_ROWS", 512);
    return h->precision == 0 && gs_plan_level(h, lv) && h->lv[lv].n >= min_rows && h->lv[lv].n <= max_rows;
}
static bool wgs_forced(const smg_hierarchy* h, int lv) { return wgs_mode_now(h) == 1 && wgs_in_range(h, lv); }
static bool wgs_wanted(const smg_hierarchy* h, int lv, int k)
{
    const int mode = wgs_mode_now(h);
    if (mode == 0 || k < 1 || !wgs_in_range(h, lv)) return false;
    if (mode == 1) return true;
    const Level& Lv = h->lv[lv];
    const SellBuf& Gs = Lv.gs_on_transpose ? Lv.dAT : Lv.dA;
    return Lv.ord.n_colors() > TILED_NCMAX || Gs.view.w_max > TILED_WMAX;
}
static const WgsBuf* wgs_plan(const smg_hierarchy* h, int lv, int k) { return wgs_wanted(h, lv, k) && h->lv[lv].wgs.view.n_pieces > 0 ? &h->lv[lv].wgs : nullptr; }

static bool tiled_wanted(const smg_hierarchy* h, int lv, int k, int sweeps)
{
    static const int on = env_int("SMG_TILED", 1), max_rows = env_int("SMG_TILED_MAX_ROWS", 122880), min_rows = env_int("SMG_TILED_MIN_ROWS", 512);
    if (!on || k < 1 || k > 7 || sweeps < 1 || sweeps > 3 || !gs_plan_level(h, lv) || wgs_forced(h, lv)) return false;
    return h->lv[lv].n >= min_rows && h->lv[lv].n <= max_rows;
}
static const TiledDev* tiled_plan(const smg_hierarchy* h, int lv, int k, int sweeps)
{
    if (!tiled_wanted(h, lv, k, sweeps)) return nullptr;
    const TiledBuf& B = h->lv[lv].tiled[sweeps];
    return B.view.n_tiles > 0 && (size_t)B.view.max_ext * std::min(k, 3) * sizeof(double) + TILED_LDS_STATIC <= 64 * 1024 ? &B.view : nullptr;
}
static bool tiled_either(const smg_hierarchy* h, int lv, int k, int sa, int sb) { return tiled_plan(h, lv, k, sa) || tiled_plan(h, lv, k, sb); }

static bool bgs_wanted(const smg_hierarchy* h, int lv, int k)
{
    static const int on = env_int("SMG_BGS", 1);
    if (!on || h->precision != 0 || k < BGS_COLS || k % BGS_COLS != 0 || h->bgs_min_rows < 0 || !gs_plan_level(h, lv)) return false;
    return h->lv[lv].n >= h->bgs_min_rows;
}
static const BgsBuf* bgs_plan(const smg_hierarchy* h, int lv, int k) { return bgs_wanted(h, lv, k) && h->lv[lv].bgs.view.n_blocks > 0 ? &h->lv[lv].bgs : nullptr; }

SweepPlan smg::sweep_plan(const smg_hierarchy* h, int lv, int k, int sweeps, bool fp64, int first)
{
    SweepPlan s;
    if (!fp64) return s;
    if (first != FIRST_SWEEP) {
        const TiledDev* t = tiled_plan(h, lv, k, sweeps);
        if (t && h->lv[lv].t.p) { s.tiled = t; return s; }
    }
    if (first != FIRST_NONE) return s;
    if ((s.wave = wgs_plan(h, lv, k))) return s;
    s.block = bgs_plan(h, lv, k);
    return s;
}

struct SweepMatrix {
    const Level* Lv = nullptr;
    Csr AT;
    std::vector<int> tsrc;
    const Csr* G = nullptr;
    std::vector<int> to_level_value(const std::vector<int>& entries) const
    {
        std::vector<int> m(entries.size());
        for (size_t i = 0; i < m.size(); i++) m[i] = entries[i] < 0 ? -1 : Lv->A_int_src[(size_t)(Lv->gs_on_transpose ? tsrc[(size_t)entries[i]] : entries[i])];
        return m;
    }
};
static int sweep_matrix(smg_hierarchy* h, int lv, SweepMatrix* M)
{
    int rc = ensure_A_int(h, lv);
    if (rc) return rc;
    M->Lv = &h->lv[lv];
    if (M->Lv->gs_on_transpose) M->AT = transpose(M->Lv->A_int, &M->tsrc);
    M->G = M->Lv->gs_on_transpose ? &M->AT : &M->Lv->A_int;
    return SMG_OK;
}

static int gather_plan_values(smg_hierarchy* h, const Level& Lv, PlanValues& V)
{
    auto ensure_map = [](DevBuf<int>& d, const std::vector<int>& host) { return d.n == host.size() && (d.p || host.empty()) ? hipSuccess : d.upload(host); };
    HIPCHK(ensure_map(V.map, V.host_map)); HIPCHK(ensure_map(V.mapd, V.host_mapd));
    HIPCHK(launch_gather_vals(V.val.p, Lv.d_Aval.p, V.map.p, V.val.n, h->stream));
    HIPCHK(launch_gather_vals(V.diag.p, Lv.d_Aval.p, V.mapd.p, V.diag.n, h->stream));
    return SMG_OK;
}
static int set_plan_values(smg_hierarchy* h, const Level& Lv, const SweepMatrix& M, PlanValues& V, const std::vector<double>& val, const std::vector<int>& entry,
                           const std::vector<double>& diag, const std::vector<int>& dentry)
{
    HIPCHK(V.val.upload(val)); HIPCHK(V.diag.upload(diag));
    V.host_map = M.to_level_value(entry); V.host_mapd = M.to_level_value(dentry);
    return h->host_stale && Lv.d_Aval.p ? gather_plan_values(h, Lv, V) : SMG_OK;
}

static int ensure_tiled(smg_hierarchy* h, int lv, int sweeps)
{
    Level& Lv = h->lv[lv];
    TiledBuf& B = Lv.tiled[sweeps];
    if (B.tried) return SMG_OK;
    B.tried = true;
    static const int rows_env = env_int("SMG_TILED_ROWS", 0), nt_env = env_int("SMG_TILED_NT", 0);
    const int tile_rows0 = rows_env > 0 ? rows_env : std::min(512, std::max(256, (Lv.n + 239) / 240));
    constexpr int max_ext = (64 * 1024 - TILED_LDS_STATIC) / 8;
    SweepMatrix M;
    { int rc = sweep_matrix(h, lv, &M); if (rc) return rc; }
    TiledGs P;
    int threads = 512;
    for (int tile_rows = tile_rows0, tries = 0; tries < 3 && P.empty(); tile_rows = tile_rows * 2 / 3, tries++) {
        threads = nt_env > 0 ? nt_env : 512;
        P = build_tiled_gs(*M.G, Lv.ord.color_ptr, sweeps, tile_rows, max_ext, threads);
    }
    if (P.empty()) return SMG_OK;
    HIPCHK(B.hdr.upload(P.hdr)); HIPCHK(B.ext_rows.upload(P.ext_rows)); HIPCHK(B.pcol.upload(P.pcol)); HIPCHK(B.prow.upload(P.prow));
    { int rc = set_plan_values(h, Lv, M, B.v, P.pval, P.pentry, P.pdiag, P.pdentry); if (rc) return rc; }
    HIPCHK(tiled_gs_prepare(P.max_ext));
    int wmax = 0;
    for (int t = 0; t < P.n_tiles; t++) wmax = std::max(wmax, P.hdr[(size_t)t * TILED_HDR + 2]);
    B.view.threads = threads;
    B.view.n_tiles = P.n_tiles; B.view.nc = P.nc; B.view.P = P.P; B.view.sweeps = sweeps; B.view.max_ext = P.max_ext; B.view.w_max = wmax;
    B.view.hdr = B.hdr.p; B.view.ext_rows = B.ext_rows.p; B.view.pcol = B.pcol.p; B.view.pval = B.v.val.p; B.view.prow = B.prow.p; B.view.pdiag = B.v.diag.p;
    if (env_int("SMG_DEBUG_TILED", 0))
        std::fprintf(stderr, "tiled relax(%d) level %d: %d rows, %d tiles x %d threads, %d phases, extended tile <= %d rows, %.2fx row updates, entries per row <= %d\n", sweeps, lv, Lv.n,
                     P.n_tiles, threads, P.P, P.max_ext, (double)P.updates / ((double)sweeps * Lv.n), wmax);
    return SMG_OK;
}

static int ensure_bgs(smg_hierarchy* h, int lv)
{
    Level& Lv = h->lv[lv];
    BgsBuf& B = Lv.bgs;
    if (B.tried) return SMG_OK;
    B.tried = true;
    static const int rows_env = env_int("SMG_BGS_ROWS", 64);
    SweepMatrix M;
    { int rc = sweep_matrix(h, lv, &M); if (rc) return rc; }
    const auto t_plan0 = std::chrono::steady_clock::now();
    BgsPlan P = build_bgs(*M.G, Lv.ord.color_ptr, std::min(std::max(rows_env, 8), (int)BGS_ROWS));
    const double plan_ms = 1e3 * std::chrono::duration<double>(std::chrono::steady_clock::now() - t_plan0).count();
    if (P.empty()) return SMG_OK;
    HIPCHK(B.hdr.upload(P.hdr)); HIPCHK(B.xrow.upload(P.xrow)); HIPCHK(B.ugrow.upload(P.ugrow)); HIPCHK(B.ulrow.upload(P.ulrow)); HIPCHK(B.eidx.upload(P.eidx));
    { int rc = set_plan_values(h, Lv, M, B.v, P.eval, P.eentry, P.udiag, P.dentry); if (rc) return rc; }
    B.view.n_blocks = P.n_blocks; B.view.n_colors = P.n_colors; B.view.xrows = P.xrows;
    B.view.hdr = B.hdr.p; B.view.xrow = B.xrow.p; B.view.ugrow = B.ugrow.p; B.view.ulrow = B.ulrow.p; B.view.udiag = B.v.diag.p; B.view.eidx = B.eidx.p; B.view.eval = B.v.val.p;
    B.color_ptr = P.color_ptr; B.host_rows = P.rows; B.host_blk_ptr = P.blk_ptr; B.rim = P.rim; B.fill = P.fill;
    if (env_int("SMG_DEBUG_BGS", 0))
        std::fprintf(stderr, "block Gauss-Seidel level %d: %d rows, %d blocks in %d colours, %.0f %% of the units' row slots hold a row of their own, rim %.3f rows read per row beyond the iterate, LDS image of %d rows; plan built in %.0f ms\n",
                     lv, Lv.n, P.n_blocks, P.n_colors, 100.0 * P.fill, P.rim, P.xrows, plan_ms);
    return SMG_OK;
}

static int ensure_wgs(smg_hierarchy* h, int lv)
{
    Level& Lv = h->lv[lv];
    WgsBuf& B = Lv.wgs;
    if (B.tried) return SMG_OK;
    B.tried = true;
    static const int rows_env = env_int("SMG_WGS_ROWS", WGS_ROWS), mode_env = env_int("SMG_WGS_PIECES", 1);
    SweepMatrix M;
    { int rc = sweep_matrix(h, lv, &M); if (rc) return rc; }
    const auto t_plan0 = std::chrono::steady_clock::now();
    WgsPlan P = build_wgs(*M.G, std::min(std::max(rows_env, 8), (int)WGS_ROWS), mode_env);
    const double plan_ms = 1e3 * std::chrono::duration<double>(std::chrono::steady_clock::now() - t_plan0).count();
    if (P.empty()) return SMG_OK;
    HIPCHK(B.hdr.upload(P.hdr)); HIPCHK(B.grow.upload(P.grow)); HIPCHK(B.meta.upload(P.meta)); HIPCHK(B.rim.upload(P.rim)); HIPCHK(B.eoff.upload(P.eoff));
    { int rc = set_plan_values(h, Lv, M, B.v, P.eval, P.eentry, P.diag, P.dentry); if (rc) return rc; }
    B.view.n_pieces = P.n_pieces; B.view.n_colors = P.n_colors; B.view.rim_pitch = P.rim_pitch; B.view.nb_max = P.nb_max;
    B.view.hdr = B.hdr.p; B.view.grow = B.grow.p; B.view.meta = B.meta.p; B.view.diag = B.v.diag.p; B.view.rim = B.rim.p; B.view.eoff = B.eoff.p; B.view.eval = B.v.val.p;
    B.color_ptr = P.color_ptr; B.host_rows = P.rows; B.host_piece_ptr = P.piece_ptr; B.rim_ratio = P.rim_ratio; B.phases_mean = P.phases_mean; B.phases_max = P.phases_max;
    if (env_int("SMG_DEBUG_WGS", 0))
        std::fprintf(stderr, "wave Gauss-Seidel level %d: %d rows, %d pieces in %d colours, phases per piece %.1f (max %d), rim %.2f rows read per row beyond the iterate, rim pitch %d; plan built in %.0f ms\n",
                     lv, Lv.n, P.n_pieces, P.n_colors, P.phases_mean, P.phases_max, P.rim_ratio, P.rim_pitch, plan_ms);
    return SMG_OK;
}

static int ensure_level_plans(smg_hierarchy* h, int lv, int k, int sa, int sb, bool drop)
{
    Level& Lv = h->lv[lv];
    int rc;
    for (int sw : {sa, sb}) if (tiled_wanted(h, lv, k, sw) && (rc = ensure_tiled(h, lv, sw))) return rc;
    if (bgs_wanted(h, lv, k) && !Lv.bgs.tried) { if (drop) drop_graphs(h); if ((rc = ensure_bgs(h, lv))) return rc; }
    if (wgs_wanted(h, lv, k) && !Lv.wgs.tried && !tiled_either(h, lv, k, sa, sb)) { if (drop) drop_graphs(h); if ((rc = ensure_wgs(h, lv))) return rc; }
    return SMG_OK;
}

int smg::prepare_level_plans(smg_hierarchy* h, int lv)
{
    static const int on = env_int("SMG_EARLY_PLANS", 1), max_rows = env_int("SMG_EARLY_PLANS_MAX_ROWS", 70000);
    if (!on || lv <= 0 || lv >= h->n_levels - 1 || h->precision != 0 || h->lv[lv].n > max_rows) return SMG_OK;
    return ensure_level_plans(h, lv, 1, h->pre, h->post, false);
}

int smg::prepare_sweep_plans(smg_hierarchy* h, int k, int sa, int sb)
{
    for (int lv = 0; lv < h->n_levels - 1; lv++) {
        Level& Lv = h->lv[lv];
        int rc = ensure_level_plans(h, lv, k, sa, sb, true);
        if (rc) return rc;
        if (tiled_either(h, lv, k, sa, sb) && Lv.t.n < (size_t)Lv.n * std::max(h->kcap, 1)) {
            drop_graphs(h);
            HIPCHK(Lv.t.alloc((size_t)Lv.n * std::max(h->kcap, 1)));
            HIPCHK(hipMemsetAsync(Lv.t.p, 0, Lv.t.n * sizeof(double), h->stream));
        }
    }
    return SMG_OK;
}

int smg::refresh_plan_values(smg_hierarchy* h)
{
    for (int lv = 0; lv < h->n_levels - 1; lv++) {
        Level& Lv = h->lv[lv];
        int rc;
        for (int s = 1; s <= 3; s++) if (Lv.tiled[s].view.n_tiles > 0 && (rc = gather_plan_values(h, Lv, Lv.tiled[s].v))) return rc;
        if (Lv.wgs.view.n_pieces > 0 && (rc = gather_plan_values(h, Lv, Lv.wgs.v))) return rc;
        if (Lv.bgs.view.n_blocks > 0 && (rc = gather_plan_values(h, Lv, Lv.bgs.v))) return rc;
    }
    return SMG_OK;
}
void smg::drop_sweep_plans(smg_hierarchy* h)
{
    for (auto& Lv : h->lv) { for (auto& B : Lv.tiled) B = TiledBuf(); Lv.bgs = BgsBuf(); Lv.wgs = WgsBuf(); }
}

extern "C" int smg_hierarchy_set_block_gs(smg_hierarchy* h, int min_rows)
{
    if (!h) return fail(SMG_ERR_INVALID, "smg_hierarchy_set_block_gs: null handle");
    if (h->in_solve) return fail(SMG_ERR_INVALID, "smg_hierarchy_set_block_gs called during a split-phase solve");
    if (min_rows != h->bgs_min_rows) { h->bgs_min_rows = min_rows; if (h->stream) drop_graphs(h); }
    return SMG_OK;
}
extern "C" int smg_level_get_block_gs_order(smg_hierarchy* h, int lv, int k, int* n_blocks, int* n_colors, int* color_ptr, int* blk_ptr, int* rows, double* stats)
{
    int rc = check_ready(h, "smg_level_get_block_gs_order");
    if (rc) return rc;
    if (lv < 0 || lv >= h->n_levels || k < 1) return fail(SMG_ERR_INVALID, "smg_level_get_block_gs_order: bad level / k");
    if (!bgs_wanted(h, lv, k)) return 0;
    if (!h->lv[lv].bgs.tried) { drop_graphs(h); if ((rc = ensure_bgs(h, lv))) return rc; }
    const BgsBuf* Q = bgs_plan(h, lv, k);
    if (!Q) return 0;
    if (n_blocks) *n_blocks = Q->view.n_blocks;
    if (n_colors) *n_colors = Q->view.n_colors;
    if (color_ptr) std::copy(Q->color_ptr.begin(), Q->color_ptr.end(), color_ptr);
    if (blk_ptr) std::copy(Q->host_blk_ptr.begin(), Q->host_blk_ptr.end(), blk_ptr);
    if (rows) std::copy(Q->host_rows.begin(), Q->host_rows.end(), rows);
    if (stats) { stats[0] = Q->rim; stats[1] = Q->fill; }
    return 1;
}

extern "C" int smg_hierarchy_set_wave_gs(smg_hierarchy* h, int mode)
{
    if (!h) return fail(SMG_ERR_INVALID, "smg_hierarchy_set_wave_gs: null handle");
    if (h->in_solve) return fail(SMG_ERR_INVALID, "smg_hierarchy_set_wave_gs called during a split-phase solve");
    if (mode < -1 || mode > 1) return fail(SMG_ERR_INVALID, "smg_hierarchy_set_wave_gs: mode must be -1 (automatic), 0 (never) or 1 (every Gauss-Seidel level in range)");
    if (mode != h->wgs_mode) { h->wgs_mode = mode; if (h->stream) drop_graphs(h); }
    return SMG_OK;
}
extern "C" int smg_level_get_wave_gs_order(smg_hierarchy* h, int lv, int k, int* n_pieces, int* n_colors, int* color_ptr, int* piece_ptr, int* rows, double* stats)
{
    int rc = check_ready(h, "smg_level_get_wave_gs_order");
    if (rc) return rc;
    if (lv < 0 || lv >= h->n_levels || k < 1) return fail(SMG_ERR_INVALID, "smg_level_get_wave_gs_order: bad level / k");
    if (!wgs_wanted(h, lv, k)) return 0;
    DeviceScope dsc(h->device);
    if ((rc = prepare_sweep_plans(h, k, h->pre, h->post))) return rc;
    const WgsBuf* Q = wgs_plan(h, lv, k);
    if (!Q || tiled_either(h, lv, k, h->pre, h->post)) return 0;
    if (n_pieces) *n_pieces = Q->view.n_pieces;
    if (n_colors) *n_colors = Q->view.n_colors;
    if (color_ptr) std::copy(Q->color_ptr.begin(), Q->color_ptr.end(), color_ptr);
    if (piece_ptr) std::copy(Q->host_piece_ptr.begin(), Q->host_piece_ptr.end(), piece_ptr);
    if (rows) std::copy(Q->host_rows.begin(), Q->host_rows.end(), rows);
    if (stats) { stats[0] = Q->rim_ratio; stats[1] = Q->phases_mean; stats[2] = (double)Q->phases_max; }
    return 1;
}


static int check_level(smg_hierarchy* h, int lv, bool args_ok, const char* who, const Csr** G)
{
    if (!h || lv < 0 || lv >= h->n_levels - 1 || !args_ok) return fail(SMG_ERR_INVALID, "%s: bad arguments", who);
    int rc = ensure_A_int(h, lv);
    if (rc) return rc;
    const Level& Lv = h->lv[lv];
    if (Lv.A_int.nr != Lv.n || Lv.n == 0 || h->bs != 1) return fail(SMG_ERR_INVALID, "%s: the host half of smg_precompute has not run (scalar hierarchies only)", who);
    *G = &Lv.A_int;
    return SMG_OK;
}
static std::vector<double> check_vector(int n, bool rhs)
{
    std::vector<double> v((size_t)n);
    for (int i = 0; i < n; i++) v[(size_t)i] = rhs ? std::cos(0.11 * i) - 0.5 * std::sin(2.1 * i) : std::sin(0.37 * i) + 0.25 * std::cos(1.3 * i);
    return v;
}
static double max_diff(const std::vector<double>& y, const std::vector<double>& ref)
{
    double d = 0.0;
    for (size_t i = 0; i < y.size(); i++) d = std::max(d, std::fabs(y[i] - ref[i]));
    return d;
}
static int check_partition(const Csr& G, const char* plan, const char* part, const char* parts, int n_parts, int n_colors, const std::vector<int>& color_ptr,
                           const std::vector<int>& part_ptr, const std::vector<int>& rows, int max_rows)
{
    const int n = G.nr;
    std::vector<int> part_of((size_t)n, -1), col_of_part((size_t)n_parts, -1);
    for (int c = 0; c < n_colors; c++) for (int q = color_ptr[(size_t)c]; q < color_ptr[(size_t)c + 1]; q++) col_of_part[(size_t)q] = c;
    for (int q = 0; q < n_parts; q++) {
        if (part_ptr[(size_t)q + 1] - part_ptr[(size_t)q] > max_rows) return fail(SMG_ERR_INVALID, "%s: %s %d has more than %d rows", plan, part, q, max_rows);
        for (int t = part_ptr[(size_t)q]; t < part_ptr[(size_t)q + 1]; t++) {
            const int i = rows[(size_t)t];
            if (i < 0 || i >= n || part_of[(size_t)i] >= 0) return fail(SMG_ERR_INVALID, "%s: row %d is not in exactly one %s", plan, i, part);
            part_of[(size_t)i] = q;
        }
    }
    for (int i = 0; i < n; i++) {
        if (part_of[(size_t)i] < 0) return fail(SMG_ERR_INVALID, "%s: row %d is in no %s", plan, i, part);
        for (int p = G.ptr[(size_t)i]; p < G.ptr[(size_t)i + 1]; p++) {
            const int j = G.col[(size_t)p];
            if (part_of[(size_t)j] != part_of[(size_t)i] && col_of_part[(size_t)part_of[(size_t)j]] == col_of_part[(size_t)part_of[(size_t)i]])
                return fail(SMG_ERR_INVALID, "%s: %s %d and %d share an entry and a colour", plan, parts, part_of[(size_t)i], part_of[(size_t)j]);
        }
    }
    return SMG_OK;
}
static void ordered_sweep(const Csr& G, const std::vector<int>& rows, const std::vector<double>& b, std::vector<double>& x)
{
    const int n = G.nr;
    std::vector<int> pos((size_t)n);
    for (int t = 0; t < n; t++) pos[(size_t)rows[(size_t)t]] = t;
    std::vector<std::pair<int, int>> ent;
    for (int t = 0; t < n; t++) {
        const int i = rows[(size_t)t];
        ent.clear();
        double diag = 1.0;
        for (int p = G.ptr[(size_t)i]; p < G.ptr[(size_t)i + 1]; p++) {
            if (G.col[(size_t)p] == i) diag = G.val[(size_t)p]; else ent.emplace_back(pos[(size_t)G.col[(size_t)p]], p);
        }
        std::sort(ent.begin(), ent.end());
        double acc = 0.0;
        for (const auto& e : ent) acc += G.val[(size_t)e.second] * x[(size_t)G.col[(size_t)e.second]];
        x[(size_t)i] = (b[(size_t)i] - acc) / diag;
    }
}

extern "C" int smg_debug_check_tiling_plan(smg_hierarchy* h, int lv, int sweeps, int tile_rows, int* n_tiles, int* max_ext_rows, double* redundancy,
                                           double* max_abs_diff)
{
    return guarded("smg_debug_check_tiling_plan", [&]() -> int {
        const Csr* G = nullptr;
        int rc = check_level(h, lv, !(sweeps < 1 || tile_rows < 8), "smg_debug_check_tiling_plan", &G);
        if (rc) return rc;
        const int n = G->nr;
        const TiledGs P = build_tiled_gs(*G, h->lv[lv].ord.color_ptr, sweeps, tile_rows, 1 << 20, 1 << 20);
        if (n_tiles) *n_tiles = P.n_tiles;
        if (max_ext_rows) *max_ext_rows = P.max_ext;
        if (redundancy) *redundancy = P.n_tiles ? (double)P.updates / ((double)sweeps * n) : 0.0;
        if (max_abs_diff) *max_abs_diff = 0.0;
        if (P.empty()) return SMG_OK;
        const std::vector<double> x = check_vector(n, false), b = check_vector(n, true);
        std::vector<double> ref = x, y((size_t)n, 0.0);
        const std::vector<int>& cp = h->lv[lv].ord.color_ptr;
        for (int s = 0; s < sweeps; s++)
            for (size_t c = 0; c + 1 < cp.size(); c++)
                for (int i = cp[c]; i < cp[c + 1]; i++) {
                    double acc = 0.0, diag = 1.0;
                    for (int p = G->ptr[(size_t)i]; p < G->ptr[(size_t)i + 1]; p++) {
                        if (G->col[(size_t)p] == i) diag = G->val[(size_t)p];
                        else acc += G->val[(size_t)p] * ref[(size_t)G->col[(size_t)p]];
                    }
                    ref[(size_t)i] = (b[(size_t)i] - acc) / diag;
                }
        const int bad = tiled_sweep_host(P, b.data(), x.data(), y.data());
        if (bad >= 0) return fail(SMG_ERR_INVALID, "tiling plan: tile %d holds a column outside its image", bad);
        if (max_abs_diff) *max_abs_diff = max_diff(y, ref);
        return SMG_OK;
    });
}

extern "C" int smg_debug_check_wave_gs_plan(smg_hierarchy* h, int lv, int piece_rows, int pieces_mode, int* n_pieces, int* n_colors, double* stats, double* max_abs_diff)
{
    return guarded("smg_debug_check_wave_gs_plan", [&]() -> int {
        const Csr* G = nullptr;
        int rc = check_level(h, lv, !(piece_rows < 8), "smg_debug_check_wave_gs_plan", &G);
        if (rc) return rc;
        const WgsPlan P = build_wgs(*G, std::min(piece_rows, (int)WGS_ROWS), pieces_mode);
        if (n_pieces) *n_pieces = P.n_pieces;
        if (n_colors) *n_colors = P.n_colors;
        if (stats) { stats[0] = P.rim_ratio; stats[1] = P.phases_mean; stats[2] = (double)P.phases_max; }
        if (max_abs_diff) *max_abs_diff = 0.0;
        if (P.empty()) return SMG_OK;
        if ((rc = check_partition(*G, "wave plan", "piece", "pieces", P.n_pieces, P.n_colors, P.color_ptr, P.piece_ptr, P.rows, WGS_ROWS))) return rc;
        const std::vector<double> x = check_vector(G->nr, false), b = check_vector(G->nr, true);
        std::vector<double> ref = x, y = x;
        ordered_sweep(*G, P.rows, b, ref);
        wgs_sweep_host(P, b.data(), y.data());
        if (max_abs_diff) *max_abs_diff = max_diff(y, ref);
        return SMG_OK;
    });
}

extern "C" int smg_debug_check_block_gs_plan(smg_hierarchy* h, int lv, int block_rows, int* n_blocks, int* n_colors, double* rim, double* fill, double* max_abs_diff)
{
    return guarded("smg_debug_check_block_gs_plan", [&]() -> int {
        const Csr* G = nullptr;
        int rc = check_level(h, lv, !(block_rows < 8), "smg_debug_check_block_gs_plan", &G);
        if (rc) return rc;
        const BgsPlan P = build_bgs(*G, h->lv[lv].ord.color_ptr, std::min(block_rows, (int)BGS_ROWS));
        if (n_blocks) *n_blocks = P.n_blocks;
        if (n_colors) *n_colors = P.n_colors;
        if (rim) *rim = P.rim;
        if (fill) *fill = P.fill;
        if (max_abs_diff) *max_abs_diff = 0.0;
        if (P.empty()) return SMG_OK;
        if ((rc = check_partition(*G, "block plan", "block", "blocks", P.n_blocks, P.n_colors, P.color_ptr, P.blk_ptr, P.rows, INT_MAX))) return rc;
        const std::vector<double> x = check_vector(G->nr, false), b = check_vector(G->nr, true);
        std::vector<double> ref = x, y = x;
        ordered_sweep(*G, P.rows, b, ref);
        const long bad = bgs_sweep_host(P, b.data(), y.data());
        if (bad >= 0) return fail(SMG_ERR_INVALID, "block plan: local index %d outside the image of %d rows", P.eidx[(size_t)bad], P.xrows);
        if (max_abs_diff) *max_abs_diff = max_diff(y, ref);
        return SMG_OK;
    });
}
```

surface_multigrid_code_amd/csrc/smg_tiled.cpp:

```cpp
#include "smg_tiled.hpp"
#include "smg_bgs.hpp"

#include <algorithm>
#include <array>

namespace smg {

namespace {
struct TileData {
    std::vector<int> ext;
    std::array<int, TILED_NCMAX> n_loc{}, m{};
    std::array<std::array<int, TILED_PMAX + 1>, TILED_NCMAX> cnt{};
    int W = 0;
    std::array<std::vector<int>, TILED_NCMAX> pcol, pentry, prow, pdentry;
    std::array<std::vector<double>, TILED_NCMAX> pval, pdiag;
    long updates = 0;
    bool ok = true;
};
}

std::vector<int> partition_tiles(const Csr& G, int tile_rows, int* n_tiles)
{
    const int n = G.nr;
    std::vector<int> part((size_t)n, 0), order((size_t)n), dist((size_t)n, -1);
    for (int i = 0; i < n; i++) order[(size_t)i] = i;
    struct Seg { int b, e; };
    std::vector<Seg> cur{{0, n}}, done;
    std::vector<int> stamp((size_t)n, -1);
    int id_base = 0;
    while (!cur.empty()) {
        std::vector<Seg> left(cur.size()), right(cur.size());
        std::vector<char> split(cur.size(), 0);
        parallel_for((long)cur.size(), 1, [&](long s0, long s1) {
            std::vector<int> queue;
            for (long s = s0; s < s1; s++) {
                const Seg sg = cur[(size_t)s];
                if (sg.e - sg.b <= tile_rows) continue;
                const int id = id_base + (int)s;
                for (int i = sg.b; i < sg.e; i++) { __atomic_store_n(&stamp[(size_t)order[(size_t)i]], id, __ATOMIC_RELAXED); dist[(size_t)order[(size_t)i]] = -1; }
                auto bfs = [&](int root) {
                    queue.clear();
                    for (int i = sg.b; i < sg.e; i++) dist[(size_t)order[(size_t)i]] = -1;
                    size_t head = 0;
                    int scan = sg.b;
                    int cur_root = root;
                    while ((int)queue.size() < sg.e - sg.b) {
                        if (head == queue.size()) {
                            while (cur_root < 0 || dist[(size_t)cur_root] >= 0) { cur_root = order[(size_t)scan]; scan++; }
                            dist[(size_t)cur_root] = queue.empty() ? 0 : dist[(size_t)queue.back()] + 1;
                            queue.push_back(cur_root);
                            cur_root = -1;
                        }
                        const int v = queue[head++];
                        for (int p = G.ptr[(size_t)v]; p < G.ptr[(size_t)v + 1]; p++) {
                            const int q = G.col[(size_t)p];
                            if (__atomic_load_n(&stamp[(size_t)q], __ATOMIC_RELAXED) == id && dist[(size_t)q] < 0) { dist[(size_t)q] = dist[(size_t)v] + 1; queue.push_back(q); }
                        }
                    }
                    return queue.back();
                };
                const int far1 = bfs(order[(size_t)sg.b]);
                bfs(far1);
                for (int i = 0; i < sg.e - sg.b; i++) order[(size_t)sg.b + i] = queue[(size_t)i];
                const int mid = sg.b + (sg.e - sg.b) / 2;
                left[(size_t)s] = {sg.b, mid};
                right[(size_t)s] = {mid, sg.e};
                split[(size_t)s] = 1;
            }
        });
        id_base += (int)cur.size();
        std::vector<Seg> nxt;
        for (size_t s = 0; s < cur.size(); s++) {
            if (split[s]) { nxt.push_back(left[s]); nxt.push_back(right[s]); }
            else done.push_back(cur[s]);
        }
        cur.swap(nxt);
    }
    std::sort(done.begin(), done.end(), [](const Seg& a, const Seg& c) { return a.b < c.b; });
    *n_tiles = (int)done.size();
    for (size_t t = 0; t < done.size(); t++)
        for (int i = done[t].b; i < done[t].e; i++) part[(size_t)order[(size_t)i]] = (int)t;
    return part;
}

TiledGs build_tiled_gs(const Csr& G, const std::vector<int>& cp, int sweeps, int tile_rows, int max_ext, int max_panel_rows)
{
    TiledGs R;
    const int nc = (int)cp.size() - 1, n = G.nr, P = sweeps * nc;
    if (nc < 2 || nc > TILED_NCMAX || sweeps < 1 || P > TILED_PMAX || n == 0 || tile_rows < nc) return R;
    for (int r = 0; r < n; r++) if (G.ptr[(size_t)r + 1] - G.ptr[(size_t)r] > TILED_WMAX) return R;
    std::vector<signed char> color_of((size_t)n);
    for (int c = 0; c < nc; c++) for (int r = cp[(size_t)c]; r < cp[(size_t)c + 1]; r++) color_of[(size_t)r] = (signed char)c;
    int T = 0;
    const std::vector<int> part = partition_tiles(G, tile_rows, &T);
    std::vector<int> tile_ptr((size_t)T + 1, 0), tile_rows_list((size_t)n);
    for (int r = 0; r < n; r++) tile_ptr[(size_t)part[(size_t)r] + 1]++;
    for (int t = 0; t < T; t++) tile_ptr[(size_t)t + 1] += tile_ptr[(size_t)t];
    {
        std::vector<int> fill(tile_ptr.begin(), tile_ptr.end() - 1);
        for (int r = 0; r < n; r++) tile_rows_list[(size_t)fill[(size_t)part[(size_t)r]]++] = r;
    }
    std::vector<TileData> tiles((size_t)T);
    parallel_for(T, 1, [&](long t0, long t1) {
        std::vector<int> dist((size_t)n, -1), loc((size_t)n, -1), frontier, next, touched;
        for (long t = t0; t < t1; t++) {
            TileData& D = tiles[(size_t)t];
            frontier.clear(); touched.clear();
            for (int i = tile_ptr[(size_t)t]; i < tile_ptr[(size_t)t + 1]; i++) {
                const int r = tile_rows_list[(size_t)i];
                dist[(size_t)r] = 0; frontier.push_back(r); touched.push_back(r);
            }
            std::array<std::array<std::vector<int>, TILED_PMAX + 1>, TILED_NCMAX> bucket;
            for (int r : frontier) bucket[(size_t)color_of[(size_t)r]][0].push_back(r);
            for (int d = 1; d <= P; d++) {
                next.clear();
                for (int r : frontier)
                    for (int p = G.ptr[(size_t)r]; p < G.ptr[(size_t)r + 1]; p++) {
                        const int q = G.col[(size_t)p];
                        if (dist[(size_t)q] < 0) { dist[(size_t)q] = d; next.push_back(q); touched.push_back(q); bucket[(size_t)color_of[(size_t)q]][(size_t)d].push_back(q); }
                    }
                frontier.swap(next);
            }
            if ((int)touched.size() > max_ext) D.ok = false;
            if (D.ok) {
                D.ext.reserve(touched.size());
                for (int c = 0; c < nc; c++) {
                    int run = 0;
                    for (int d = 0; d <= P; d++) {
                        std::vector<int>& bk = bucket[(size_t)c][(size_t)d];
                        std::sort(bk.begin(), bk.end());
                        for (int r : bk) { loc[(size_t)r] = (int)D.ext.size(); D.ext.push_back(r); }
                        run += (int)bk.size();
                        D.cnt[(size_t)c][(size_t)d] = run;
                    }
                    for (int d = P + 1; d <= TILED_PMAX; d++) D.cnt[(size_t)c][(size_t)d] = run;
                    D.n_loc[(size_t)c] = run;
                    D.m[(size_t)c] = D.cnt[(size_t)c][(size_t)(P - c - 1)];
                }
                for (int c = 0; c < nc; c++) if (D.m[(size_t)c] > max_panel_rows) D.ok = false;
            }
            if (D.ok) {
                int W = 0, base = 0;
                for (int c = 0; c < nc; c++) {
                    for (int i = 0; i < D.m[(size_t)c]; i++) { const int r = D.ext[(size_t)base + i]; W = std::max(W, G.ptr[(size_t)r + 1] - G.ptr[(size_t)r]); }
                    base += D.n_loc[(size_t)c];
                }
                D.W = W;
                base = 0;
                for (int c = 0; c < nc; c++) {
                    const int m = D.m[(size_t)c];
                    D.pcol[(size_t)c].assign((size_t)W * m, 0);
                    D.pentry[(size_t)c].assign((size_t)W * m, -1);
                    D.pval[(size_t)c].assign((size_t)W * m, 0.0);
                    D.prow[(size_t)c].resize((size_t)m);
                    D.pdiag[(size_t)c].assign((size_t)m, 1.0);
                    D.pdentry[(size_t)c].assign((size_t)m, -1);
                    for (int i = 0; i < m; i++) {
                        const int r = D.ext[(size_t)base + i];
                        D.prow[(size_t)c][(size_t)i] = r;
                        for (int j = 0; j < W; j++) D.pcol[(size_t)c][(size_t)j * m + i] = base + i;
                        int j = 0;
                        for (int p = G.ptr[(size_t)r]; p < G.ptr[(size_t)r + 1]; p++, j++) {
                            if (G.col[(size_t)p] == r) { D.pdiag[(size_t)c][(size_t)i] = G.val[(size_t)p]; D.pdentry[(size_t)c][(size_t)i] = p; continue; }
                            D.pcol[(size_t)c][(size_t)j * m + i] = loc[(size_t)G.col[(size_t)p]];
                            D.pval[(size_t)c][(size_t)j * m + i] = G.val[(size_t)p];
                            D.pentry[(size_t)c][(size_t)j * m + i] = p;
                        }
                    }
                    base += D.n_loc[(size_t)c];
                }
                for (int p = 1; p <= P; p++) D.updates += D.cnt[(size_t)((p - 1) % nc)][(size_t)(P - p)];
            }
            for (int r : touched) { dist[(size_t)r] = -1; loc[(size_t)r] = -1; }
        }
    });
    for (const TileData& D : tiles) if (!D.ok) return R;
    R.n_tiles = T; R.nc = nc; R.sweeps = sweeps; R.P = P;
    R.hdr.assign((size_t)T * TILED_HDR, 0);
    for (int t = 0; t < T; t++) {
        const TileData& D = tiles[(size_t)t];
        int* H = R.hdr.data() + (size_t)t * TILED_HDR;
        H[0] = (int)R.ext_rows.size(); H[1] = (int)D.ext.size(); H[2] = D.W; H[3] = 0;
        R.max_ext = std::max(R.max_ext, (int)D.ext.size());
        R.updates += D.updates;
        R.ext_rows.insert(R.ext_rows.end(), D.ext.begin(), D.ext.end());
        int lbase = 0;
        for (int c = 0; c < nc; c++) {
            int* C = H + 4 + c * TILED_CSTRIDE;
            C[0] = (int)R.pcol.size(); C[1] = D.m[(size_t)c]; C[2] = (int)R.prow.size(); C[3] = lbase;
            for (int d = 0; d <= TILED_PMAX; d++) C[4 + d] = D.cnt[(size_t)c][(size_t)d];
            R.pcol.insert(R.pcol.end(), D.pcol[(size_t)c].begin(), D.pcol[(size_t)c].end());
            R.pval.insert(R.pval.end(), D.pval[(size_t)c].begin(), D.pval[(size_t)c].end());
            R.pentry.insert(R.pentry.end(), D.pentry[(size_t)c].begin(), D.pentry[(size_t)c].end());
            R.prow.insert(R.prow.end(), D.prow[(size_t)c].begin(), D.prow[(size_t)c].end());
            R.pdiag.insert(R.pdiag.end(), D.pdiag[(size_t)c].begin(), D.pdiag[(size_t)c].end());
            R.pdentry.insert(R.pdentry.end(), D.pdentry[(size_t)c].begin(), D.pdentry[(size_t)c].end());
            lbase += D.n_loc[(size_t)c];
        }
    }
    return R;
}

int tiled_sweep_host(const TiledGs& P, const double* b, const double* x, double* y)
{
    const int nc = P.nc, PP = P.P;
    std::vector<double> xs;
    for (int t = 0; t < P.n_tiles; t++) {
        const int* H = P.hdr.data() + (size_t)t * TILED_HDR;
        const int ext_off = H[0], n_ext = H[1], w = H[2];
        xs.assign((size_t)n_ext, 0.0);
        for (int i = 0; i < n_ext; i++) xs[(size_t)i] = x[(size_t)P.ext_rows[(size_t)ext_off + i]];
        for (int p = 1; p <= PP; p++) {
            const int* C = H + 4 + ((p - 1) % nc) * TILED_CSTRIDE;
            const int pan = C[0], m = C[1], ro = C[2], lbase = C[3], cnt = C[4 + (PP - p)];
            for (int i = 0; i < cnt; i++) {
                double acc = 0.0;
                for (int j = 0; j < w; j++) {
                    const int cl = P.pcol[(size_t)pan + (size_t)j * m + i];
                    if (cl < 0 || cl >= n_ext) return t;
                    acc += P.pval[(size_t)pan + (size_t)j * m + i] * xs[(size_t)cl];
                }
                xs[(size_t)lbase + i] = (b[(size_t)P.prow[(size_t)ro + i]] - acc) / P.pdiag[(size_t)ro + i];
            }
        }
        for (int c = 0; c < nc; c++) {
            const int* C = H + 4 + c * TILED_CSTRIDE;
            for (int i = 0; i < C[4]; i++) y[(size_t)P.prow[(size_t)C[2] + i]] = xs[(size_t)C[3] + i];
        }
    }
    return -1;
}

}
```

surface_multigrid_code_amd/csrc/smg_tiled.hpp:

```cpp
#pragma once
#include <vector>

#include "smg_sparse.hpp"

namespace smg {

constexpr int TILED_NCMAX = 5;
constexpr int TILED_PMAX = 15;
constexpr int TILED_WMAX = 12;
constexpr int TILED_THREADS = 512;
constexpr int TILED_CSTRIDE = 4 + TILED_PMAX + 1;
constexpr int TILED_HDR = 4 + TILED_NCMAX * TILED_CSTRIDE;
constexpr int TILED_LDS_STATIC = 512;

struct TiledGs {
    int n_tiles = 0, nc = 0, sweeps = 0, P = 0, max_ext = 0;
    long updates = 0;
    std::vector<int> hdr;
    std::vector<int> ext_rows;
    std::vector<int> pcol;
    std::vector<double> pval;
    std::vector<int> pentry;
    std::vector<int> prow;
    std::vector<double> pdiag;
    std::vector<int> pdentry;
    bool empty() const { return n_tiles == 0; }
};

TiledGs build_tiled_gs(const Csr& G, const std::vector<int>& color_ptr, int sweeps, int tile_rows, int max_ext, int max_panel_rows = TILED_THREADS);

int tiled_sweep_host(const TiledGs& P, const double* b, const double* x, double* y);

}
```

surface_multigrid_code_amd/csrc/smg_tiled_device.hip:

```cpp
#include <hip/hip_runtime.h>

#include <cstdlib>

#include "smg_device.hpp"
#include "smg_device_inl.hpp"
#include "smg_tiled.hpp"

namespace smg {

constexpr int TILED_NT = TILED_THREADS;

template <int NC, int W, int KB>
__global__ __launch_bounds__(TILED_NT) void k_tiled_gs(const int* __restrict__ hdr, const int* __restrict__ ext_rows, const int* __restrict__ pcol,
                                                       const double* __restrict__ pval, const int* __restrict__ prow, const double* __restrict__ pdiag, const double* __restrict__ b,
                                                       const double* __restrict__ x, double* __restrict__ y, int ld, int nc, int sweeps, const int* done, int dbg_phases)
{
    extern __shared__ double xs[];
    __shared__ int Hs[TILED_HDR];
    const int tid = threadIdx.x;
    if (tid < TILED_HDR) Hs[tid] = hdr[(size_t)blockIdx.x * TILED_HDR + tid];
    const int stop = load_flag(done);
    __syncthreads();
    const int ext_off = Hs[0], n_ext = Hs[1], w = Hs[2];
    const int P = sweeps * nc;
    constexpr int U = 4;
    const int nt = (int)blockDim.x;
    int er[U];
    auto image_indices = [&](const int i0) {
#pragma unroll
        for (int t = 0; t < U; t++) { const int i = i0 + t * nt; er[t] = ext_rows[ext_off + (i < n_ext ? i : n_ext - 1)]; }
    };
    auto image_gather = [&](const int i0) {
        double g[U][KB];
#pragma unroll
        for (int t = 0; t < U; t++) gather_kb<KB, double>(x + (size_t)er[t] * ld, true, g[t]);
#pragma unroll
        for (int t = 0; t < U; t++) {
            const int i = i0 + t * nt;
            if (i < n_ext) {
#pragma unroll
                for (int q = 0; q < KB; q++) xs[i * KB + q] = g[t][q];
            }
        }
    };
    image_indices(tid);
    int cR[NC][W], gR[NC];
    double vR[NC][W], bR[NC][KB], dR[NC];
#pragma unroll
    for (int c = 0; c < NC; c++) {
        gR[c] = -1; dR[c] = 1.0;
#pragma unroll
        for (int j = 0; j < W; j++) { cR[c][j] = 0; vR[c][j] = 0.0; }
        if (c < nc) {
            const int* C = Hs + 4 + c * TILED_CSTRIDE;
            const int pan = C[0], m = C[1];
            if (tid < m) {
                gR[c] = prow[C[2] + tid];
                dR[c] = pdiag[C[2] + tid];
#pragma unroll
                for (int j = 0; j < W; j++)
                    if (j < w) { cR[c][j] = pcol[(size_t)pan + (size_t)j * m + tid]; vR[c][j] = pval[(size_t)pan + (size_t)j * m + tid]; }
            }
        }
    }
    image_gather(tid);
#pragma unroll
    for (int c = 0; c < NC; c++) gather_kb<KB, double>(b + (size_t)(gR[c] >= 0 ? gR[c] : 0) * ld, gR[c] >= 0, bR[c]);
    for (int i0 = tid + U * nt; i0 < n_ext; i0 += U * nt) { image_indices(i0); image_gather(i0); }
    if constexpr (KB > 1) {
#pragma unroll
        for (int c = 0; c < NC; c++)
#pragma unroll
            for (int j = 0; j < W; j++) { int v = cR[c][j]; asm volatile("" : "+v"(v)); cR[c][j] = v * KB; }
    }
    __syncthreads();
    for (int s = 0; s < sweeps; s++) {
#pragma unroll
        for (int c = 0; c < NC; c++) {
            if (c < nc && s * nc + c < dbg_phases) {
                const int p = s * nc + c + 1;
                const int* C = Hs + 4 + c * TILED_CSTRIDE;
                const int lrow = C[3] + tid, cnt = C[4 + (P - p)];
                if (tid < cnt) {
                    double acc[KB];
#pragma unroll
                    for (int q = 0; q < KB; q++) acc[q] = 0.0;
#pragma unroll
                    for (int j = 0; j < W; j++) {
                        const double v = vR[c][j];
                        const int at = cR[c][j];
#pragma unroll
                        for (int q = 0; q < KB; q++) acc[q] += v * xs[at + q];
                    }
#pragma unroll
                    for (int q = 0; q < KB; q++) xs[lrow * KB + q] = (bR[c][q] - acc[q]) / dR[c];
                }
                __syncthreads();
            }
        }
    }
    if (!stop) {
#pragma unroll
        for (int c = 0; c < NC; c++)
            if (c < nc) {
                const int* C = Hs + 4 + c * TILED_CSTRIDE;
                if (tid < C[4]) {
#pragma unroll
                    for (int q = 0; q < KB; q++) y[(size_t)gR[c] * ld + q] = xs[(C[3] + tid) * KB + q];
                }
            }
    }
}

template <int NC, int W>
static void launch_tiled_one(const TiledDev& Tl, const double* x, const double* b, double* y, int ld, int kb, const int* done, hipStream_t st)
{
    const size_t lds = (size_t)Tl.max_ext * kb * sizeof(double);
    static const int dbg = getenv("SMG_DEBUG_TILED_PHASES") ? atoi(getenv("SMG_DEBUG_TILED_PHASES")) : 1 << 20;
#define SMG_TILED_LAUNCH(KB) hipLaunchKernelGGL((k_tiled_gs<NC, W, KB>), dim3(Tl.n_tiles), dim3(Tl.threads), lds, st, Tl.hdr, Tl.ext_rows, Tl.pcol, Tl.pval, Tl.prow, Tl.pdiag, b, x, y, ld, Tl.nc, Tl.sweeps, done, dbg)
    if (kb == 1) SMG_TILED_LAUNCH(1);
    else if (kb == 2) SMG_TILED_LAUNCH(2);
    else SMG_TILED_LAUNCH(3);
#undef SMG_TILED_LAUNCH
}

hipError_t launch_tiled_gs(const TiledDev& Tl, const double* x, const double* b, double* y, int k, const Ctrl* ctrl, hipStream_t st)
{
    if (Tl.n_tiles <= 0 || k < 1 || (size_t)Tl.max_ext * (k < 3 ? k : 3) * sizeof(double) + TILED_LDS_STATIC > 64 * 1024) return hipErrorInvalidValue;
    const int* done = ctrl ? &ctrl->done : never_done();
    for (int c = 0; c < k; c += 3) {
        const int kb = k - c < 3 ? k - c : 3;
        const bool w8 = Tl.w_max <= 8;
        if (Tl.nc <= 3) { if (w8) launch_tiled_one<3, 8>(Tl, x + c, b + c, y + c, k, kb, done, st); else launch_tiled_one<3, 12>(Tl, x + c, b + c, y + c, k, kb, done, st); }
        else if (Tl.nc == 4) { if (w8) launch_tiled_one<4, 8>(Tl, x + c, b + c, y + c, k, kb, done, st); else launch_tiled_one<4, 12>(Tl, x + c, b + c, y + c, k, kb, done, st); }
        else { if (w8) launch_tiled_one<5, 8>(Tl, x + c, b + c, y + c, k, kb, done, st); else launch_tiled_one<5, 12>(Tl, x + c, b + c, y + c, k, kb, done, st); }
    }
    return hipGetLastError();
}

hipError_t tiled_gs_prepare(int max_ext)
{
    return (size_t)max_ext * sizeof(double) + TILED_LDS_STATIC <= 64 * 1024 ? hipSuccess : hipErrorInvalidValue;
}

}
```

Before: 3417 V-cycles/s.

## Fuse residual into tiled GS pre-smoother and single-launch symmetric coarse gemv

Tiled Gauss-Seidel plans gain one extra halo ring so the kernel can compute the residual b - A x for owned rows directly from the shared-memory iterate. This removes the separate residual SpMV pass after pre-smoothing on levels where the tiled plan is used. Separately, the symmetric dense coarse gemv folds its partial-sum reduction into the tile kernel through atomic counters and a last-block reduction, saving a launch. The costs are extra redundant halo work per tile, higher register pressure, and atomic synchronisation on the coarse level.

```diff
diff --git a/include/smg.h b/include/smg.h
--- a/include/smg.h
+++ b/include/smg.h
@@ -199,6 +199,9 @@
 
 int smg_debug_check_tiling_plan(smg_hierarchy *h, int lv, int sweeps, int tile_rows, int *n_tiles, int *max_ext_rows, double *redundancy,
                                 double *max_abs_diff);
+int smg_debug_check_tiling_resid_plan(smg_hierarchy *h, int lv, int sweeps, int tile_rows, int *n_tiles, double *redundancy, int *iterate_bits_differ,
+                                      int *residual_bits_differ);
+int smg_debug_cycle_shape(smg_hierarchy *h, int k, int *kernel_nodes, int *tiled_resid_levels, int *coarse_one_launch);
 int smg_debug_check_block_gs_plan(smg_hierarchy *h, int lv, int block_rows, int *n_blocks, int *n_colors, double *rim, double *fill, double *max_abs_diff);
 int smg_debug_check_wave_gs_plan(smg_hierarchy *h, int lv, int piece_rows, int pieces_mode, int *n_pieces, int *n_colors, double *stats, double *max_abs_diff);
 int smg_debug_raise_coarse_stall(smg_hierarchy *h);
diff --git a/surface_multigrid_code_amd/_lib.py b/surface_multigrid_code_amd/_lib.py
--- a/surface_multigrid_code_amd/_lib.py
+++ b/surface_multigrid_code_amd/_lib.py
@@ -130,6 +130,8 @@
         "smg_level_sell_stats": (i, [vp, i, i, lp, lp, ip]),
         "smg_level_first_colour_rows": (i, [vp, i]),
         "smg_debug_check_tiling_plan": (i, [vp, i, i, i, ip, ip, dp, dp]),
+        "smg_debug_check_tiling_resid_plan": (i, [vp, i, i, i, ip, dp, ip, ip]),
+        "smg_debug_cycle_shape": (i, [vp, i, ip, ip, ip]),
         "smg_debug_check_sparse_cholesky": (i, [i, ip, ip, dp, lp, ip, dp]),
         "smg_hierarchy_set_coarse_dense_max": (i, [vp, i]),
         "smg_hierarchy_set_coarse_schur": (i, [vp, i, i]),
diff --git a/surface_multigrid_code_amd/api.py b/surface_multigrid_code_amd/api.py
--- a/surface_multigrid_code_amd/api.py
+++ b/surface_multigrid_code_amd/api.py
@@ -322,6 +322,11 @@
     def first_colour_rows(self, lv):
         return self.L.smg_level_first_colour_rows(self.h, lv)
 
+    def cycle_shape(self, k=1):
+        kn, tr, co = C.c_int(), C.c_int(), C.c_int()
+        _chk(self.L.smg_debug_cycle_shape(self.h, int(k), C.byref(kn), C.byref(tr), C.byref(co)), "smg_debug_cycle_shape")
+        return kn.value, tr.value, co.value
+
     def set_block_gs(self, min_rows):
         _chk(self.L.smg_hierarchy_set_block_gs(self.h, int(min_rows)), "smg_hierarchy_set_block_gs")
 
diff --git a/surface_multigrid_code_amd/csrc/smg_capi.cpp b/surface_multigrid_code_amd/csrc/smg_capi.cpp
--- a/surface_multigrid_code_amd/csrc/smg_capi.cpp
+++ b/surface_multigrid_code_amd/csrc/smg_capi.cpp
@@ -52,6 +52,7 @@
         line(p + "galerkin_recipes", B(L.r1_ptr) + B(L.r1_idx) + B(L.r2_ptr) + B(L.r2_idx) + B(L.r1_coef) + B(L.r2_coef));
         long long t = 0;
         for (const auto& T : L.tiled) t += T.bytes();
+        for (const auto& T : L.tiled_r) t += T.bytes();
         line(p + "tiled_plans", t);
         line(p + "bgs_plan", L.bgs.bytes());
         line(p + "wgs_plan", L.wgs.bytes());
diff --git a/surface_multigrid_code_amd/csrc/smg_cycle.cpp b/surface_multigrid_code_amd/csrc/smg_cycle.cpp
--- a/surface_multigrid_code_amd/csrc/smg_cycle.cpp
+++ b/surface_multigrid_code_amd/csrc/smg_cycle.cpp
@@ -304,10 +304,11 @@
 }
 
 template <typename T>
-static int enqueue_gs_tiled(smg_hierarchy* h, const TiledDev& plan, const T* b, T* const buf[2], int* cur, int k, const Ctrl* ctrl)
+static int enqueue_gs_tiled(smg_hierarchy* h, const TiledDev& plan, const T* b, T* const buf[2], int* cur, int k, const Ctrl* ctrl, T* resid = nullptr)
 {
     ProfGuard pg(h, "MG: relaxation");
-    HIPCHK(launch_tiled_gs(plan, (const double*)buf[*cur], (const double*)b, (double*)buf[1 - *cur], k, ctrl, h->stream));
+    if (resid) HIPCHK(launch_tiled_gs_resid(plan, (const double*)buf[*cur], (const double*)b, (double*)buf[1 - *cur], (double*)resid, k, ctrl, h->stream));
+    else HIPCHK(launch_tiled_gs(plan, (const double*)buf[*cur], (const double*)b, (double*)buf[1 - *cur], k, ctrl, h->stream));
     *cur ^= 1;
     return SMG_OK;
 }
@@ -362,6 +363,7 @@
     int cur = 0;
     const bool fp64 = std::is_same<T, double>::value;
     const SweepPlan sp_pre = sweep_plan(h, lv, k, pre, fp64, first), sp_post = sweep_plan(h, lv, k, post, fp64, FIRST_NONE);
+    const TiledDev* pre_resid = (fp64 && kind == LV_GS) ? tiled_resid_plan(h, lv, k, pre, sp_pre.tiled) : nullptr;
     int rc;
     if (kind == LV_JACOBI) {
         if (first_done) cur = 1;
@@ -369,10 +371,11 @@
     } else if (kind == LV_CHEBY) {
         if (first_done) cur = 1;
         rc = enqueue_cheby<T>(h, lv, Prec<T>::b(Lv), buf, &cur, k, pre, ctrl, first_done);
-    } else if (sp_pre.tiled) rc = enqueue_gs_tiled<T>(h, *sp_pre.tiled, Prec<T>::b(Lv), buf, &cur, k, ctrl);
+    } else if (pre_resid) rc = enqueue_gs_tiled<T>(h, *pre_resid, Prec<T>::b(Lv), buf, &cur, k, ctrl, Prec<T>::r(Lv));
+    else if (sp_pre.tiled) rc = enqueue_gs_tiled<T>(h, *sp_pre.tiled, Prec<T>::b(Lv), buf, &cur, k, ctrl);
     else rc = enqueue_gs<T>(h, lv, sp_pre, Prec<T>::b(Lv), buf[0], k, pre, ctrl, first, buf[1]);
     if (rc) return rc;
-    {
+    if (!pre_resid) {
         ProfGuard pg(h, "MG: residual");
         HIPCHK(Prec<T>::opA(h, Lv, false, SELL_RESID, 0, -1, buf[cur], Prec<T>::b(Lv), Prec<T>::r(Lv), k, ctrl));
     }
@@ -586,6 +589,39 @@
     return coarse_stall_check(h);
 }
 
+extern "C" int smg_debug_cycle_shape(smg_hierarchy* h, int k, int* kernel_nodes, int* tiled_resid_levels, int* coarse_one_launch)
+{
+    int rc = piece_prolog(h, 0, k, "smg_debug_cycle_shape", false);
+    if (rc) return rc;
+    DeviceScope dsc(h->device);
+    if (h->precision != 0) return fail(SMG_ERR_INVALID, "smg_debug_cycle_shape: fp64 cycles only");
+    hipGraph_t g = nullptr;
+    HIPCHK(hipStreamBeginCapture(h->stream, hipStreamCaptureModeThreadLocal));
+    rc = enqueue_vcycle_t<double>(h, 0, k, h->pre, h->post, nullptr);
+    hipError_t e = hipStreamEndCapture(h->stream, &g);
+    if (rc) { if (g) (void)hipGraphDestroy(g); return rc; }
+    if (e != hipSuccess) return fail(SMG_ERR_HIP, "hipStreamEndCapture: %s", hipGetErrorString(e));
+    size_t nn = 0;
+    e = hipGraphGetNodes(g, nullptr, &nn);
+    std::vector<hipGraphNode_t> nodes(nn);
+    if (e == hipSuccess && nn) e = hipGraphGetNodes(g, nodes.data(), &nn);
+    int kn = 0;
+    for (size_t i = 0; e == hipSuccess && i < nn; i++) {
+        hipGraphNodeType ty;
+        if ((e = hipGraphNodeGetType(nodes[i], &ty)) == hipSuccess && ty == hipGraphNodeTypeKernel) kn++;
+    }
+    (void)hipGraphDestroy(g);
+    if (e != hipSuccess) return fail(SMG_ERR_HIP, "smg_debug_cycle_shape: %s", hipGetErrorString(e));
+    if (kernel_nodes) *kernel_nodes = kn;
+    int folded = 0;
+    for (int lv = 0; lv < h->n_levels - 1; lv++)
+        if (level_kind(h, lv) == LV_GS && tiled_resid_plan(h, lv, k, h->pre, sweep_plan(h, lv, k, h->pre, true, FIRST_NONE).tiled)) folded++;
+    if (tiled_resid_levels) *tiled_resid_levels = folded;
+    if (coarse_one_launch)
+        *coarse_one_launch = h->union_m == 0 && !h->coarse_sparse && !h->coarse_schur && sym_coarse_one_launch(coarse_cols(h, k), k, h->nc_pad, h->d_sympart.p);
+    return SMG_OK;
+}
+
 extern "C" int smg_bench_relax(smg_hierarchy* h, int lv, int k, int sweeps, int reps, double* us_per_call)
 {
     int rc = piece_prolog(h, lv, k, "smg_bench_relax", true);
diff --git a/surface_multigrid_code_amd/csrc/smg_device.hip b/surface_multigrid_code_amd/csrc/smg_device.hip
--- a/surface_multigrid_code_amd/csrc/smg_device.hip
+++ b/surface_multigrid_code_amd/csrc/smg_device.hip
@@ -1088,9 +1088,12 @@
     }
 }
 
-template <typename T>
-__global__ __launch_bounds__(256) void k_sym_gemv_tiles(const T* __restrict__ Ainv, int lda, const T* __restrict__ b, T* __restrict__ part, int nb)
-{
+template <typename T, bool ONE = false>
+__global__ __launch_bounds__(256) void k_sym_gemv_tiles(const T* __restrict__ Ainv, int lda, const T* __restrict__ b, T* __restrict__ part, int nb,
+                                                        int* cnt, int n, T* u, const int* done)
+{
+    int stop = 0;
+    if (ONE) stop = load_flag(done);
     const int idx = blockIdx.x;
     int I = (int)((sqrtf(8.0f * (float)idx + 1.0f) - 1.0f) * 0.5f);
     I -= (I * (I + 1) / 2 > idx);
@@ -1119,8 +1122,41 @@
     }
     red[g][l] = s;
     __syncthreads();
-    if (t < 64) part[((size_t)I * nb + J) * 64 + t] = red[0][t] + red[1][t];
-    else if (t < 128 && I != J) part[((size_t)J * nb + I) * 64 + (t - 64)] = red[2][t - 64] + red[3][t - 64];
+    if constexpr (!ONE) {
+        if (t < 64) part[((size_t)I * nb + J) * 64 + t] = red[0][t] + red[1][t];
+        else if (t < 128 && I != J) part[((size_t)J * nb + I) * 64 + (t - 64)] = red[2][t - 64] + red[3][t - 64];
+    } else {
+        if (t < 64) __hip_atomic_store(&part[((size_t)I * nb + J) * 64 + t], red[0][t] + red[1][t], __ATOMIC_RELAXED, __HIP_MEMORY_SCOPE_AGENT);
+        else if (t < 128 && I != J) __hip_atomic_store(&part[((size_t)J * nb + I) * 64 + (t - 64)], red[2][t - 64] + red[3][t - 64], __ATOMIC_RELAXED, __HIP_MEMORY_SCOPE_AGENT);
+        asm volatile("s_waitcnt vmcnt(0)" ::: "memory");
+        __shared__ int last[2];
+        __syncthreads();
+        if (t == 0) {
+            __builtin_amdgcn_fence(__ATOMIC_RELEASE, "agent");
+            asm volatile("s_waitcnt vmcnt(0)" ::: "memory");
+            last[0] = __hip_atomic_fetch_add(&cnt[I], 1, __ATOMIC_RELAXED, __HIP_MEMORY_SCOPE_AGENT) == nb - 1;
+            last[1] = I != J && __hip_atomic_fetch_add(&cnt[J], 1, __ATOMIC_RELAXED, __HIP_MEMORY_SCOPE_AGENT) == nb - 1;
+            if (last[0] | last[1]) {
+                __builtin_amdgcn_fence(__ATOMIC_ACQUIRE, "agent");
+                asm volatile("s_waitcnt vmcnt(0)" ::: "memory");
+            }
+        }
+        __syncthreads();
+        const int q = (nb + 3) / 4, b0 = g * q, b1 = min(nb, b0 + q);
+        for (int which = 0; which < 2; which++) {
+            if (!last[which]) continue;
+            const int a = which ? J : I;
+            T sum = (T)0;
+#pragma unroll 8
+            for (int bidx = b0; bidx < b1; bidx++) sum += __hip_atomic_load(&part[((size_t)a * nb + bidx) * 64 + l], __ATOMIC_RELAXED, __HIP_MEMORY_SCOPE_AGENT);
+            red[g][l] = sum;
+            __syncthreads();
+            const int i = a * 64 + l;
+            if (g == 0 && i < n && !stop) u[i] = u[i] + ((red[0][l] + red[1][l]) + (red[2][l] + red[3][l]));
+            if (t == 0) __hip_atomic_store(&cnt[a], 0, __ATOMIC_RELAXED, __HIP_MEMORY_SCOPE_AGENT);
+            __syncthreads();
+        }
+    }
 }
 template <typename T>
 __global__ __launch_bounds__(256) void k_sym_gemv_sum(const T* __restrict__ part, int nb, int n, T* u, const int* done)
@@ -1138,6 +1174,9 @@
     if (g == 0 && i < n && !stop) u[i] = u[i] + ((red[0][l] + red[1][l]) + (red[2][l] + red[3][l]));
 }
 
+static bool sym_one_knob() { static const int one = getenv("SMG_SYM_COARSE_ONE") ? atoi(getenv("SMG_SYM_COARSE_ONE")) : 1; return one != 0; }
+bool sym_coarse_one_launch(int k, int ld, int lda, const void* sym_work) { return k == 1 && ld == 1 && sym_work && lda % 64 == 0 && lda >= 512 && sym_one_knob(); }
+
 template <typename T>
 static hipError_t launch_dense_T(const T* Ainv, int n, int lda, const T* b, T* u, int k, int ld, const Ctrl* ctrl, hipStream_t st, void* sym_work)
 {
@@ -1146,7 +1185,12 @@
     if (n <= 0) return hipSuccess;
     if (k == 1 && ld == 1 && sym_work && lda % 64 == 0 && lda >= 512) {
         const int nt = lda / 64;
-        hipLaunchKernelGGL((k_sym_gemv_tiles<T>), dim3(nt * (nt + 1) / 2), dim3(256), 0, st, Ainv, lda, b, (T*)sym_work, nt);
+        if (sym_one_knob()) {
+            int* cnt = (int*)((double*)sym_work + (size_t)nt * nt * 64);
+            hipLaunchKernelGGL((k_sym_gemv_tiles<T, true>), dim3(nt * (nt + 1) / 2), dim3(256), 0, st, Ainv, lda, b, (T*)sym_work, nt, cnt, n, u, done);
+            return hipGetLastError();
+        }
+        hipLaunchKernelGGL((k_sym_gemv_tiles<T, false>), dim3(nt * (nt + 1) / 2), dim3(256), 0, st, Ainv, lda, b, (T*)sym_work, nt, (int*)nullptr, 0, (T*)nullptr, (const int*)nullptr);
         hipLaunchKernelGGL((k_sym_gemv_sum<T>), dim3(nt), dim3(256), 0, st, (const T*)sym_work, nt, n, u, done);
         return hipGetLastError();
     }
@@ -1194,14 +1238,14 @@
 {
     if (lda <= 0 || lda % 64) return hipErrorInvalidValue;
     const int nt = lda / 64;
-    hipLaunchKernelGGL((k_sym_gemv_tiles<double>), dim3(nt * (nt + 1) / 2), dim3(256), 0, st, Ainv, lda, b, part, nt);
+    hipLaunchKernelGGL((k_sym_gemv_tiles<double, false>), dim3(nt * (nt + 1) / 2), dim3(256), 0, st, Ainv, lda, b, part, nt, (int*)nullptr, 0, (double*)nullptr, (const int*)nullptr);
     return hipGetLastError();
 }
 hipError_t launch_sym_gemv_tiles_f32(const float* Ainv, int lda, const float* b, float* part, hipStream_t st)
 {
     if (lda <= 0 || lda % 64) return hipErrorInvalidValue;
     const int nt = lda / 64;
-    hipLaunchKernelGGL((k_sym_gemv_tiles<float>), dim3(nt * (nt + 1) / 2), dim3(256), 0, st, Ainv, lda, b, part, nt);
+    hipLaunchKernelGGL((k_sym_gemv_tiles<float, false>), dim3(nt * (nt + 1) / 2), dim3(256), 0, st, Ainv, lda, b, part, nt, (int*)nullptr, 0, (float*)nullptr, (const int*)nullptr);
     return hipGetLastError();
 }
 hipError_t launch_dense_gemv_add(const double* Ainv, int n, int lda, const double* b, double* u, int k, int ld,
diff --git a/surface_multigrid_code_amd/csrc/smg_device.hpp b/surface_multigrid_code_amd/csrc/smg_device.hpp
--- a/surface_multigrid_code_amd/csrc/smg_device.hpp
+++ b/surface_multigrid_code_amd/csrc/smg_device.hpp
@@ -146,14 +146,17 @@
 
 struct TiledDev {
     int n_tiles = 0, nc = 0, P = 0, sweeps = 0, max_ext = 0, w_max = 0, threads = 512;
+    int rings = 0;
     const int* hdr = nullptr;
     const int* ext_rows = nullptr;
     const int* pcol = nullptr;
     const double* pval = nullptr;
     const int* prow = nullptr;
     const double* pdiag = nullptr;
+    const int* pdslot = nullptr;
 };
 hipError_t launch_tiled_gs(const TiledDev& T, const double* x, const double* b, double* y, int k, const Ctrl* ctrl, hipStream_t st);
+hipError_t launch_tiled_gs_resid(const TiledDev& T, const double* x, const double* b, double* y, double* r, int k, const Ctrl* ctrl, hipStream_t st);
 hipError_t tiled_gs_prepare(int max_ext);
 
 struct SparseCholDev {
@@ -232,6 +235,8 @@
 hipError_t launch_eig_residual(const double* X, const double* AX, const double* mass, const double* lam, int n, int m, double* b0, double* u0,
                                float* b32, float* u32, double* part, int groups, double* res, const Ctrl* ctrl, hipStream_t st);
 
+bool sym_coarse_one_launch(int k, int ld, int lda, const void* sym_work);
+inline size_t sym_coarse_work_doubles(int lda) { const size_t nt = (size_t)(lda / 64); return nt * nt * 64 + (nt + 1) / 2 + 1; }
 hipError_t launch_dense_gemv_add(const double* Ainv, int n, int lda, const double* b, double* u, int k, int ld,
                                  const Ctrl* ctrl, hipStream_t st, double* sym_work = nullptr);
 hipError_t launch_dense_gemv_add_f32(const float* Ainv, int n, int lda, const float* b, float* u, int k, int ld,
diff --git a/surface_multigrid_code_amd/csrc/smg_hier.hpp b/surface_multigrid_code_amd/csrc/smg_hier.hpp
--- a/surface_multigrid_code_amd/csrc/smg_hier.hpp
+++ b/surface_multigrid_code_amd/csrc/smg_hier.hpp
@@ -113,11 +113,11 @@
 };
 
 struct TiledBuf {
-    DevBuf<int> hdr, ext_rows, pcol, prow;
+    DevBuf<int> hdr, ext_rows, pcol, prow, pdslot;
     PlanValues v;
     TiledDev view;
     bool tried = false;
-    long long bytes() const { return hdr.bytes() + ext_rows.bytes() + pcol.bytes() + prow.bytes() + v.bytes(); }
+    long long bytes() const { return hdr.bytes() + ext_rows.bytes() + pcol.bytes() + prow.bytes() + pdslot.bytes() + v.bytes(); }
 };
 
 struct BgsBuf {
@@ -167,6 +167,7 @@
     Csr vpat;
     bool A_bit_symmetric = false;
     TiledBuf tiled[4];
+    TiledBuf tiled_r[4];
     WgsBuf wgs;
     BgsBuf bgs;
     std::vector<int> A_int_src;
diff --git a/surface_multigrid_code_amd/csrc/smg_internal.hpp b/surface_multigrid_code_amd/csrc/smg_internal.hpp
--- a/surface_multigrid_code_amd/csrc/smg_internal.hpp
+++ b/surface_multigrid_code_amd/csrc/smg_internal.hpp
@@ -157,6 +157,7 @@
 };
 SweepPlan sweep_plan(const smg_hierarchy* h, int lv, int k, int sweeps, bool fp64, int first);
 int prepare_sweep_plans(smg_hierarchy* h, int k, int sa, int sb);
+const TiledDev* tiled_resid_plan(const smg_hierarchy* h, int lv, int k, int sweeps, const TiledDev* tiled);
 int prepare_level_plans(smg_hierarchy* h, int lv);
 int refresh_plan_values(smg_hierarchy* h);
 void drop_sweep_plans(smg_hierarchy* h);
diff --git a/surface_multigrid_code_amd/csrc/smg_precompute.cpp b/surface_multigrid_code_amd/csrc/smg_precompute.cpp
--- a/surface_multigrid_code_amd/csrc/smg_precompute.cpp
+++ b/surface_multigrid_code_amd/csrc/smg_precompute.cpp
@@ -715,7 +715,11 @@
     HIPCHK(d_val.upload(Lc.A.val));
     HIPCHK(h->d_Ainv.ensure((size_t)np * np));
     HIPCHK(launch_dense_from_csr(h->d_Ainv.p, np, nc, d_val.p, d_pos.p, (int)Lc.A.nnz(), h->stream));
-    if (env_int("SMG_SYM_COARSE", 1)) HIPCHK(h->d_sympart.ensure((size_t)(np / 64) * (np / 64) * 64)); else h->d_sympart.release();
+    if (env_int("SMG_SYM_COARSE", 1)) {
+        HIPCHK(h->d_sympart.ensure(sym_coarse_work_doubles(np)));
+        const size_t shares = (size_t)(np / 64) * (np / 64) * 64;
+        HIPCHK(hipMemsetAsync(h->d_sympart.p + shares, 0, (h->d_sympart.n - shares) * sizeof(double), h->stream));
+    } else h->d_sympart.release();
     DevBuf<double> work;
     HIPCHK(work.alloc((size_t)2 * np * 64 + 2 * 64 * 64));
     HIPCHK(launch_spd_inverse(h->d_Ainv.p, np, work.p, h->stream));
diff --git a/surface_multigrid_code_amd/csrc/smg_sweep_plans.cpp b/surface_multigrid_code_amd/csrc/smg_sweep_plans.cpp
--- a/surface_multigrid_code_amd/csrc/smg_sweep_plans.cpp
+++ b/surface_multigrid_code_amd/csrc/smg_sweep_plans.cpp
@@ -1,6 +1,7 @@
 #include <algorithm>
 #include <climits>
 #include <cmath>
+#include <cstring>
 #include <vector>
 
 #include "smg_internal.hpp"
@@ -44,6 +45,19 @@
 {
     if (!tiled_wanted(h, lv, k, sweeps)) return nullptr;
     const TiledBuf& B = h->lv[lv].tiled[sweeps];
+    return B.view.n_tiles > 0 && (size_t)B.view.max_ext * std::min(k, 3) * sizeof(double) + TILED_LDS_STATIC <= 64 * 1024 ? &B.view : nullptr;
+}
+static bool tiled_resid_wanted(const smg_hierarchy* h, int lv, int k, int sweeps)
+{
+    static const int on = env_int("SMG_TILED_RESID", 1);
+    if (!on || !tiled_wanted(h, lv, k, sweeps) || lv >= h->n_levels - 1) return false;
+    const Level& Lv = h->lv[lv];
+    return !Lv.gs_on_transpose && Lv.dA.view.long_n == 0 && !Lv.dA.view.codes;
+}
+const TiledDev* smg::tiled_resid_plan(const smg_hierarchy* h, int lv, int k, int sweeps, const TiledDev* tiled)
+{
+    if (!tiled || h->prof_on || !tiled_resid_wanted(h, lv, k, sweeps)) return nullptr;
+    const TiledBuf& B = h->lv[lv].tiled_r[sweeps];
     return B.view.n_tiles > 0 && (size_t)B.view.max_ext * std::min(k, 3) * sizeof(double) + TILED_LDS_STATIC <= 64 * 1024 ? &B.view : nullptr;
 }
 static bool tiled_either(const smg_hierarchy* h, int lv, int k, int sa, int sb) { return tiled_plan(h, lv, k, sa) || tiled_plan(h, lv, k, sb); }
@@ -108,10 +122,10 @@
     return h->host_stale && Lv.d_Aval.p ? gather_plan_values(h, Lv, V) : SMG_OK;
 }
 
-static int ensure_tiled(smg_hierarchy* h, int lv, int sweeps)
+static int ensure_tiled(smg_hierarchy* h, int lv, int sweeps, bool resid = false)
 {
     Level& Lv = h->lv[lv];
-    TiledBuf& B = Lv.tiled[sweeps];
+    TiledBuf& B = resid ? Lv.tiled_r[sweeps] : Lv.tiled[sweeps];
     if (B.tried) return SMG_OK;
     B.tried = true;
     static const int rows_env = env_int("SMG_TILED_ROWS", 0), nt_env = env_int("SMG_TILED_NT", 0);
@@ -123,19 +137,22 @@
     int threads = 512;
     for (int tile_rows = tile_rows0, tries = 0; tries < 3 && P.empty(); tile_rows = tile_rows * 2 / 3, tries++) {
         threads = nt_env > 0 ? nt_env : 512;
-        P = build_tiled_gs(*M.G, Lv.ord.color_ptr, sweeps, tile_rows, max_ext, threads);
+        P = build_tiled_gs(*M.G, Lv.ord.color_ptr, sweeps, tile_rows, max_ext, threads, resid);
     }
     if (P.empty()) return SMG_OK;
+    int wmax = 0;
+    for (int t = 0; t < P.n_tiles; t++) wmax = std::max(wmax, P.hdr[(size_t)t * TILED_HDR + 2]);
+    if (resid && P.nc == 5 && wmax > 8) return SMG_OK;
     HIPCHK(B.hdr.upload(P.hdr)); HIPCHK(B.ext_rows.upload(P.ext_rows)); HIPCHK(B.pcol.upload(P.pcol)); HIPCHK(B.prow.upload(P.prow));
+    if (resid) { HIPCHK(B.pdslot.upload(P.pdslot)); B.view.pdslot = B.pdslot.p; }
+    B.view.rings = P.rings;
     { int rc = set_plan_values(h, Lv, M, B.v, P.pval, P.pentry, P.pdiag, P.pdentry); if (rc) return rc; }
     HIPCHK(tiled_gs_prepare(P.max_ext));
-    int wmax = 0;
-    for (int t = 0; t < P.n_tiles; t++) wmax = std::max(wmax, P.hdr[(size_t)t * TILED_HDR + 2]);
     B.view.threads = threads;
     B.view.n_tiles = P.n_tiles; B.view.nc = P.nc; B.view.P = P.P; B.view.sweeps = sweeps; B.view.max_ext = P.max_ext; B.view.w_max = wmax;
     B.view.hdr = B.hdr.p; B.view.ext_rows = B.ext_rows.p; B.view.pcol = B.pcol.p; B.view.pval = B.v.val.p; B.view.prow = B.prow.p; B.view.pdiag = B.v.diag.p;
     if (env_int("SMG_DEBUG_TILED", 0))
-        std::fprintf(stderr, "tiled relax(%d) level %d: %d rows, %d tiles x %d threads, %d phases, extended tile <= %d rows, %.2fx row updates, entries per row <= %d\n", sweeps, lv, Lv.n,
+        std::fprintf(stderr, "tiled relax(%d)%s level %d: %d rows, %d tiles x %d threads, %d phases, extended tile <= %d rows, %.2fx row updates, entries per row <= %d\n", sweeps, resid ? " + residual" : "", lv, Lv.n,
                      P.n_tiles, threads, P.P, P.max_ext, (double)P.updates / ((double)sweeps * Lv.n), wmax);
     return SMG_OK;
 }
@@ -193,6 +210,7 @@
     Level& Lv = h->lv[lv];
     int rc;
     for (int sw : {sa, sb}) if (tiled_wanted(h, lv, k, sw) && (rc = ensure_tiled(h, lv, sw))) return rc;
+    if (tiled_resid_wanted(h, lv, k, sa) && !Lv.tiled_r[sa].tried) { if (drop) drop_graphs(h); if ((rc = ensure_tiled(h, lv, sa, true))) return rc; }
     if (bgs_wanted(h, lv, k) && !Lv.bgs.tried) { if (drop) drop_graphs(h); if ((rc = ensure_bgs(h, lv))) return rc; }
     if (wgs_wanted(h, lv, k) && !Lv.wgs.tried && !tiled_either(h, lv, k, sa, sb)) { if (drop) drop_graphs(h); if ((rc = ensure_wgs(h, lv))) return rc; }
     return SMG_OK;
@@ -226,6 +244,7 @@
         Level& Lv = h->lv[lv];
         int rc;
         for (int s = 1; s <= 3; s++) if (Lv.tiled[s].view.n_tiles > 0 && (rc = gather_plan_values(h, Lv, Lv.tiled[s].v))) return rc;
+        for (int s = 1; s <= 3; s++) if (Lv.tiled_r[s].view.n_tiles > 0 && (rc = gather_plan_values(h, Lv, Lv.tiled_r[s].v))) return rc;
         if (Lv.wgs.view.n_pieces > 0 && (rc = gather_plan_values(h, Lv, Lv.wgs.v))) return rc;
         if (Lv.bgs.view.n_blocks > 0 && (rc = gather_plan_values(h, Lv, Lv.bgs.v))) return rc;
     }
@@ -233,7 +252,7 @@
 }
 void smg::drop_sweep_plans(smg_hierarchy* h)
 {
-    for (auto& Lv : h->lv) { for (auto& B : Lv.tiled) B = TiledBuf(); Lv.bgs = BgsBuf(); Lv.wgs = WgsBuf(); }
+    for (auto& Lv : h->lv) { for (auto& B : Lv.tiled) B = TiledBuf(); for (auto& B : Lv.tiled_r) B = TiledBuf(); Lv.bgs = BgsBuf(); Lv.wgs = WgsBuf(); }
 }
 
 extern "C" int smg_hierarchy_set_block_gs(smg_hierarchy* h, int min_rows)
@@ -389,6 +408,48 @@
     });
 }
 
+extern "C" int smg_debug_check_tiling_resid_plan(smg_hierarchy* h, int lv, int sweeps, int tile_rows, int* n_tiles, double* redundancy, int* iterate_bits_differ,
+                                                 int* residual_bits_differ)
+{
+    return guarded("smg_debug_check_tiling_resid_plan", [&]() -> int {
+        const Csr* G = nullptr;
+        int rc = check_level(h, lv, !(sweeps < 1 || tile_rows < 8 || !iterate_bits_differ || !residual_bits_differ), "smg_debug_check_tiling_resid_plan", &G);
+        if (rc) return rc;
+        const int n = G->nr;
+        const TiledGs P = build_tiled_gs(*G, h->lv[lv].ord.color_ptr, sweeps, tile_rows, 1 << 20, 1 << 20, true);
+        if (n_tiles) *n_tiles = P.n_tiles;
+        if (redundancy) *redundancy = P.n_tiles ? (double)P.updates / ((double)sweeps * n) : 0.0;
+        *iterate_bits_differ = 0; *residual_bits_differ = 0;
+        if (P.empty()) return SMG_OK;
+        const std::vector<double> x = check_vector(n, false), b = check_vector(n, true);
+        std::vector<double> ref = x, rref((size_t)n, 0.0), y((size_t)n, 0.0), r((size_t)n, 0.0);
+        const std::vector<int>& cp = h->lv[lv].ord.color_ptr;
+        for (int s = 0; s < sweeps; s++)
+            for (size_t c = 0; c + 1 < cp.size(); c++)
+                for (int i = cp[c]; i < cp[c + 1]; i++) {
+                    double acc = 0.0, diag = 1.0;
+                    for (int p = G->ptr[(size_t)i]; p < G->ptr[(size_t)i + 1]; p++) {
+                        if (G->col[(size_t)p] == i) diag = G->val[(size_t)p];
+                        else acc += G->val[(size_t)p] * ref[(size_t)G->col[(size_t)p]];
+                    }
+                    ref[(size_t)i] = (b[(size_t)i] - acc) / diag;
+                }
+        for (int i = 0; i < n; i++) {
+            double acc = 0.0;
+            for (int p = G->ptr[(size_t)i]; p < G->ptr[(size_t)i + 1]; p++) acc += G->val[(size_t)p] * ref[(size_t)G->col[(size_t)p]];
+            rref[(size_t)i] = b[(size_t)i] - acc;
+        }
+        const int bad = tiled_sweep_resid_host(P, b.data(), x.data(), y.data(), r.data());
+        if (bad >= 0) return fail(SMG_ERR_INVALID, "tiling plan with residual: tile %d holds a column outside its image", bad);
+        if (bad < -1) return fail(SMG_ERR_INVALID, "tiling plan with residual: the builder returned a plan without the extra ring");
+        for (int i = 0; i < n; i++) {
+            *iterate_bits_differ += std::memcmp(&y[(size_t)i], &ref[(size_t)i], sizeof(double)) != 0;
+            *residual_bits_differ += std::memcmp(&r[(size_t)i], &rref[(size_t)i], sizeof(double)) != 0;
+        }
+        return SMG_OK;
+    });
+}
+
 extern "C" int smg_debug_check_wave_gs_plan(smg_hierarchy* h, int lv, int piece_rows, int pieces_mode, int* n_pieces, int* n_colors, double* stats, double* max_abs_diff)
 {
     return guarded("smg_debug_check_wave_gs_plan", [&]() -> int {
diff --git a/surface_multigrid_code_amd/csrc/smg_tiled.cpp b/surface_multigrid_code_amd/csrc/smg_tiled.cpp
--- a/surface_multigrid_code_amd/csrc/smg_tiled.cpp
+++ b/surface_multigrid_code_amd/csrc/smg_tiled.cpp
@@ -12,7 +12,7 @@
     std::array<int, TILED_NCMAX> n_loc{}, m{};
     std::array<std::array<int, TILED_PMAX + 1>, TILED_NCMAX> cnt{};
     int W = 0;
-    std::array<std::vector<int>, TILED_NCMAX> pcol, pentry, prow, pdentry;
+    std::array<std::vector<int>, TILED_NCMAX> pcol, pentry, prow, pdentry, pdslot;
     std::array<std::vector<double>, TILED_NCMAX> pval, pdiag;
     long updates = 0;
     bool ok = true;
@@ -83,11 +83,12 @@
     return part;
 }
 
-TiledGs build_tiled_gs(const Csr& G, const std::vector<int>& cp, int sweeps, int tile_rows, int max_ext, int max_panel_rows)
+TiledGs build_tiled_gs(const Csr& G, const std::vector<int>& cp, int sweeps, int tile_rows, int max_ext, int max_panel_rows, bool with_residual)
 {
     TiledGs R;
     const int nc = (int)cp.size() - 1, n = G.nr, P = sweeps * nc;
-    if (nc < 2 || nc > TILED_NCMAX || sweeps < 1 || P > TILED_PMAX || n == 0 || tile_rows < nc) return R;
+    const int X = with_residual ? 1 : 0;
+    if (nc < 2 || nc > TILED_NCMAX || sweeps < 1 || P + X > TILED_PMAX || n == 0 || tile_rows < nc) return R;
     for (int r = 0; r < n; r++) if (G.ptr[(size_t)r + 1] - G.ptr[(size_t)r] > TILED_WMAX) return R;
     std::vector<signed char> color_of((size_t)n);
     for (int c = 0; c < nc; c++) for (int r = cp[(size_t)c]; r < cp[(size_t)c + 1]; r++) color_of[(size_t)r] = (signed char)c;
@@ -112,7 +113,7 @@
             }
             std::array<std::array<std::vector<int>, TILED_PMAX + 1>, TILED_NCMAX> bucket;
             for (int r : frontier) bucket[(size_t)color_of[(size_t)r]][0].push_back(r);
-            for (int d = 1; d <= P; d++) {
+            for (int d = 1; d <= P + X; d++) {
                 next.clear();
                 for (int r : frontier)
                     for (int p = G.ptr[(size_t)r]; p < G.ptr[(size_t)r + 1]; p++) {
@@ -126,16 +127,16 @@
                 D.ext.reserve(touched.size());
                 for (int c = 0; c < nc; c++) {
                     int run = 0;
-                    for (int d = 0; d <= P; d++) {
+                    for (int d = 0; d <= P + X; d++) {
                         std::vector<int>& bk = bucket[(size_t)c][(size_t)d];
                         std::sort(bk.begin(), bk.end());
                         for (int r : bk) { loc[(size_t)r] = (int)D.ext.size(); D.ext.push_back(r); }
                         run += (int)bk.size();
                         D.cnt[(size_t)c][(size_t)d] = run;
                     }
-                    for (int d = P + 1; d <= TILED_PMAX; d++) D.cnt[(size_t)c][(size_t)d] = run;
+                    for (int d = P + X + 1; d <= TILED_PMAX; d++) D.cnt[(size_t)c][(size_t)d] = run;
                     D.n_loc[(size_t)c] = run;
-                    D.m[(size_t)c] = D.cnt[(size_t)c][(size_t)(P - c - 1)];
+                    D.m[(size_t)c] = D.cnt[(size_t)c][(size_t)(P - c - 1 + X)];
                 }
                 for (int c = 0; c < nc; c++) if (D.m[(size_t)c] > max_panel_rows) D.ok = false;
             }
@@ -155,13 +156,14 @@
                     D.prow[(size_t)c].resize((size_t)m);
                     D.pdiag[(size_t)c].assign((size_t)m, 1.0);
                     D.pdentry[(size_t)c].assign((size_t)m, -1);
+                    D.pdslot[(size_t)c].assign((size_t)m, -1);
                     for (int i = 0; i < m; i++) {
                         const int r = D.ext[(size_t)base + i];
                         D.prow[(size_t)c][(size_t)i] = r;
                         for (int j = 0; j < W; j++) D.pcol[(size_t)c][(size_t)j * m + i] = base + i;
                         int j = 0;
                         for (int p = G.ptr[(size_t)r]; p < G.ptr[(size_t)r + 1]; p++, j++) {
-                            if (G.col[(size_t)p] == r) { D.pdiag[(size_t)c][(size_t)i] = G.val[(size_t)p]; D.pdentry[(size_t)c][(size_t)i] = p; continue; }
+                            if (G.col[(size_t)p] == r) { D.pdiag[(size_t)c][(size_t)i] = G.val[(size_t)p]; D.pdentry[(size_t)c][(size_t)i] = p; D.pdslot[(size_t)c][(size_t)i] = j; continue; }
                             D.pcol[(size_t)c][(size_t)j * m + i] = loc[(size_t)G.col[(size_t)p]];
                             D.pval[(size_t)c][(size_t)j * m + i] = G.val[(size_t)p];
                             D.pentry[(size_t)c][(size_t)j * m + i] = p;
@@ -169,13 +171,13 @@
                     }
                     base += D.n_loc[(size_t)c];
                 }
-                for (int p = 1; p <= P; p++) D.updates += D.cnt[(size_t)((p - 1) % nc)][(size_t)(P - p)];
+                for (int p = 1; p <= P; p++) D.updates += D.cnt[(size_t)((p - 1) % nc)][(size_t)(P - p + X)];
             }
             for (int r : touched) { dist[(size_t)r] = -1; loc[(size_t)r] = -1; }
         }
     });
     for (const TileData& D : tiles) if (!D.ok) return R;
-    R.n_tiles = T; R.nc = nc; R.sweeps = sweeps; R.P = P;
+    R.n_tiles = T; R.nc = nc; R.sweeps = sweeps; R.P = P; R.rings = X;
     R.hdr.assign((size_t)T * TILED_HDR, 0);
     for (int t = 0; t < T; t++) {
         const TileData& D = tiles[(size_t)t];
@@ -195,15 +197,16 @@
             R.prow.insert(R.prow.end(), D.prow[(size_t)c].begin(), D.prow[(size_t)c].end());
             R.pdiag.insert(R.pdiag.end(), D.pdiag[(size_t)c].begin(), D.pdiag[(size_t)c].end());
             R.pdentry.insert(R.pdentry.end(), D.pdentry[(size_t)c].begin(), D.pdentry[(size_t)c].end());
+            R.pdslot.insert(R.pdslot.end(), D.pdslot[(size_t)c].begin(), D.pdslot[(size_t)c].end());
             lbase += D.n_loc[(size_t)c];
         }
     }
     return R;
 }
 
-int tiled_sweep_host(const TiledGs& P, const double* b, const double* x, double* y)
+static int tiled_sweep_host_any(const TiledGs& P, const double* b, const double* x, double* y, double* r)
 {
-    const int nc = P.nc, PP = P.P;
+    const int nc = P.nc, PP = P.P, X = P.rings;
     std::vector<double> xs;
     for (int t = 0; t < P.n_tiles; t++) {
         const int* H = P.hdr.data() + (size_t)t * TILED_HDR;
@@ -212,7 +215,7 @@
         for (int i = 0; i < n_ext; i++) xs[(size_t)i] = x[(size_t)P.ext_rows[(size_t)ext_off + i]];
         for (int p = 1; p <= PP; p++) {
             const int* C = H + 4 + ((p - 1) % nc) * TILED_CSTRIDE;
-            const int pan = C[0], m = C[1], ro = C[2], lbase = C[3], cnt = C[4 + (PP - p)];
+            const int pan = C[0], m = C[1], ro = C[2], lbase = C[3], cnt = C[4 + (PP - p) + X];
             for (int i = 0; i < cnt; i++) {
                 double acc = 0.0;
                 for (int j = 0; j < w; j++) {
@@ -226,9 +229,23 @@
         for (int c = 0; c < nc; c++) {
             const int* C = H + 4 + c * TILED_CSTRIDE;
             for (int i = 0; i < C[4]; i++) y[(size_t)P.prow[(size_t)C[2] + i]] = xs[(size_t)C[3] + i];
+            if (!r) continue;
+            const int pan = C[0], m = C[1], ro = C[2];
+            for (int i = 0; i < C[4]; i++) {
+                const int ds = P.pdslot[(size_t)ro + i];
+                double acc = 0.0;
+                for (int j = 0; j < w; j++) {
+                    const double v = j == ds ? P.pdiag[(size_t)ro + i] : P.pval[(size_t)pan + (size_t)j * m + i];
+                    acc += v * xs[(size_t)P.pcol[(size_t)pan + (size_t)j * m + i]];
+                }
+                r[(size_t)P.prow[(size_t)ro + i]] = b[(size_t)P.prow[(size_t)ro + i]] - acc;
+            }
         }
     }
     return -1;
 }
 
-}
+int tiled_sweep_host(const TiledGs& P, const double* b, const double* x, double* y) { return tiled_sweep_host_any(P, b, x, y, nullptr); }
+int tiled_sweep_resid_host(const TiledGs& P, const double* b, const double* x, double* y, double* r) { return P.rings == 1 ? tiled_sweep_host_any(P, b, x, y, r) : -2; }
+
+}
diff --git a/surface_multigrid_code_amd/csrc/smg_tiled.hpp b/surface_multigrid_code_amd/csrc/smg_tiled.hpp
--- a/surface_multigrid_code_amd/csrc/smg_tiled.hpp
+++ b/surface_multigrid_code_amd/csrc/smg_tiled.hpp
@@ -15,6 +15,7 @@
 
 struct TiledGs {
     int n_tiles = 0, nc = 0, sweeps = 0, P = 0, max_ext = 0;
+    int rings = 0;
     long updates = 0;
     std::vector<int> hdr;
     std::vector<int> ext_rows;
@@ -24,11 +25,13 @@
     std::vector<int> prow;
     std::vector<double> pdiag;
     std::vector<int> pdentry;
+    std::vector<int> pdslot;
     bool empty() const { return n_tiles == 0; }
 };
 
-TiledGs build_tiled_gs(const Csr& G, const std::vector<int>& color_ptr, int sweeps, int tile_rows, int max_ext, int max_panel_rows = TILED_THREADS);
+TiledGs build_tiled_gs(const Csr& G, const std::vector<int>& color_ptr, int sweeps, int tile_rows, int max_ext, int max_panel_rows = TILED_THREADS, bool with_residual = false);
 
 int tiled_sweep_host(const TiledGs& P, const double* b, const double* x, double* y);
+int tiled_sweep_resid_host(const TiledGs& P, const double* b, const double* x, double* y, double* r);
 
 }
diff --git a/surface_multigrid_code_amd/csrc/smg_tiled_device.hip b/surface_multigrid_code_amd/csrc/smg_tiled_device.hip
--- a/surface_multigrid_code_amd/csrc/smg_tiled_device.hip
+++ b/surface_multigrid_code_amd/csrc/smg_tiled_device.hip
@@ -10,10 +10,11 @@
 
 constexpr int TILED_NT = TILED_THREADS;
 
-template <int NC, int W, int KB>
+template <int NC, int W, int KB, bool RESID>
 __global__ __launch_bounds__(TILED_NT) void k_tiled_gs(const int* __restrict__ hdr, const int* __restrict__ ext_rows, const int* __restrict__ pcol,
                                                        const double* __restrict__ pval, const int* __restrict__ prow, const double* __restrict__ pdiag, const double* __restrict__ b,
-                                                       const double* __restrict__ x, double* __restrict__ y, int ld, int nc, int sweeps, const int* done, int dbg_phases)
+                                                       const double* __restrict__ x, double* __restrict__ y, int ld, int nc, int sweeps, const int* done, int dbg_phases,
+                                                       const int* __restrict__ pdslot, double* __restrict__ r)
 {
     extern __shared__ double xs[];
     __shared__ int Hs[TILED_HDR];
@@ -45,10 +46,12 @@
     };
     image_indices(tid);
     int cR[NC][W], gR[NC];
+    int sR[RESID ? NC : 1];
     double vR[NC][W], bR[NC][KB], dR[NC];
 #pragma unroll
     for (int c = 0; c < NC; c++) {
         gR[c] = -1; dR[c] = 1.0;
+        if constexpr (RESID) sR[c] = -1;
 #pragma unroll
         for (int j = 0; j < W; j++) { cR[c][j] = 0; vR[c][j] = 0.0; }
         if (c < nc) {
@@ -57,6 +60,7 @@
             if (tid < m) {
                 gR[c] = prow[C[2] + tid];
                 dR[c] = pdiag[C[2] + tid];
+                if constexpr (RESID) sR[c] = pdslot[C[2] + tid];
 #pragma unroll
                 for (int j = 0; j < W; j++)
                     if (j < w) { cR[c][j] = pcol[(size_t)pan + (size_t)j * m + tid]; vR[c][j] = pval[(size_t)pan + (size_t)j * m + tid]; }
@@ -80,7 +84,7 @@
             if (c < nc && s * nc + c < dbg_phases) {
                 const int p = s * nc + c + 1;
                 const int* C = Hs + 4 + c * TILED_CSTRIDE;
-                const int lrow = C[3] + tid, cnt = C[4 + (P - p)];
+                const int lrow = C[3] + tid, cnt = C[4 + (P - p) + (RESID ? 1 : 0)];
                 if (tid < cnt) {
                     double acc[KB];
 #pragma unroll
@@ -107,35 +111,60 @@
                 if (tid < C[4]) {
 #pragma unroll
                     for (int q = 0; q < KB; q++) y[(size_t)gR[c] * ld + q] = xs[(C[3] + tid) * KB + q];
+                    if constexpr (RESID) {
+                        double acc[KB];
+#pragma unroll
+                        for (int q = 0; q < KB; q++) acc[q] = 0.0;
+#pragma unroll
+                        for (int j = 0; j < W; j++) {
+                            const double v = j == sR[c] ? dR[c] : vR[c][j];
+                            const int at = cR[c][j];
+#pragma unroll
+                            for (int q = 0; q < KB; q++) acc[q] += v * xs[at + q];
+                        }
+#pragma unroll
+                        for (int q = 0; q < KB; q++) r[(size_t)gR[c] * ld + q] = bR[c][q] - acc[q];
+                    }
                 }
             }
     }
 }
 
-template <int NC, int W>
-static void launch_tiled_one(const TiledDev& Tl, const double* x, const double* b, double* y, int ld, int kb, const int* done, hipStream_t st)
+template <int NC, int W, bool RESID>
+static void launch_tiled_one(const TiledDev& Tl, const double* x, const double* b, double* y, double* r, int ld, int kb, const int* done, hipStream_t st)
 {
     const size_t lds = (size_t)Tl.max_ext * kb * sizeof(double);
     static const int dbg = getenv("SMG_DEBUG_TILED_PHASES") ? atoi(getenv("SMG_DEBUG_TILED_PHASES")) : 1 << 20;
-#define SMG_TILED_LAUNCH(KB) hipLaunchKernelGGL((k_tiled_gs<NC, W, KB>), dim3(Tl.n_tiles), dim3(Tl.threads), lds, st, Tl.hdr, Tl.ext_rows, Tl.pcol, Tl.pval, Tl.prow, Tl.pdiag, b, x, y, ld, Tl.nc, Tl.sweeps, done, dbg)
+#define SMG_TILED_LAUNCH(KB) hipLaunchKernelGGL((k_tiled_gs<NC, W, KB, RESID>), dim3(Tl.n_tiles), dim3(Tl.threads), lds, st, Tl.hdr, Tl.ext_rows, Tl.pcol, Tl.pval, Tl.prow, Tl.pdiag, b, x, y, ld, Tl.nc, Tl.sweeps, done, dbg, Tl.pdslot, r)
     if (kb == 1) SMG_TILED_LAUNCH(1);
     else if (kb == 2) SMG_TILED_LAUNCH(2);
     else SMG_TILED_LAUNCH(3);
 #undef SMG_TILED_LAUNCH
 }
 
-hipError_t launch_tiled_gs(const TiledDev& Tl, const double* x, const double* b, double* y, int k, const Ctrl* ctrl, hipStream_t st)
+template <bool RESID>
+static hipError_t launch_tiled_any(const TiledDev& Tl, const double* x, const double* b, double* y, double* r, int k, const Ctrl* ctrl, hipStream_t st)
 {
     if (Tl.n_tiles <= 0 || k < 1 || (size_t)Tl.max_ext * (k < 3 ? k : 3) * sizeof(double) + TILED_LDS_STATIC > 64 * 1024) return hipErrorInvalidValue;
+    if (RESID != (Tl.rings == 1) || (RESID && (!Tl.pdslot || !r))) return hipErrorInvalidValue;
     const int* done = ctrl ? &ctrl->done : never_done();
     for (int c = 0; c < k; c += 3) {
         const int kb = k - c < 3 ? k - c : 3;
         const bool w8 = Tl.w_max <= 8;
-        if (Tl.nc <= 3) { if (w8) launch_tiled_one<3, 8>(Tl, x + c, b + c, y + c, k, kb, done, st); else launch_tiled_one<3, 12>(Tl, x + c, b + c, y + c, k, kb, done, st); }
-        else if (Tl.nc == 4) { if (w8) launch_tiled_one<4, 8>(Tl, x + c, b + c, y + c, k, kb, done, st); else launch_tiled_one<4, 12>(Tl, x + c, b + c, y + c, k, kb, done, st); }
-        else { if (w8) launch_tiled_one<5, 8>(Tl, x + c, b + c, y + c, k, kb, done, st); else launch_tiled_one<5, 12>(Tl, x + c, b + c, y + c, k, kb, done, st); }
+        double* rc = RESID ? r + c : nullptr;
+        if (Tl.nc <= 3) { if (w8) launch_tiled_one<3, 8, RESID>(Tl, x + c, b + c, y + c, rc, k, kb, done, st); else launch_tiled_one<3, 12, RESID>(Tl, x + c, b + c, y + c, rc, k, kb, done, st); }
+        else if (Tl.nc == 4) { if (w8) launch_tiled_one<4, 8, RESID>(Tl, x + c, b + c, y + c, rc, k, kb, done, st); else launch_tiled_one<4, 12, RESID>(Tl, x + c, b + c, y + c, rc, k, kb, done, st); }
+        else { if (w8) launch_tiled_one<5, 8, RESID>(Tl, x + c, b + c, y + c, rc, k, kb, done, st); else launch_tiled_one<5, 12, RESID>(Tl, x + c, b + c, y + c, rc, k, kb, done, st); }
     }
     return hipGetLastError();
+}
+hipError_t launch_tiled_gs(const TiledDev& Tl, const double* x, const double* b, double* y, int k, const Ctrl* ctrl, hipStream_t st)
+{
+    return launch_tiled_any<false>(Tl, x, b, y, nullptr, k, ctrl, st);
+}
+hipError_t launch_tiled_gs_resid(const TiledDev& Tl, const double* x, const double* b, double* y, double* r, int k, const Ctrl* ctrl, hipStream_t st)
+{
+    return launch_tiled_any<true>(Tl, x, b, y, r, k, ctrl, st);
 }
 
 hipError_t tiled_gs_prepare(int max_ext)
```

After: 2960 V-cycles/s. -13.4%, worse.
